# mountaindust/Parasitoids

Measured on AMD Instinct MI355X. Metric: grid-days/sec on 4096^2 fp64 domain, higher is better.
Workload: dtype f64; 1 GPU; C3 synthetic stack: N=4097 (nominal 4096^2), 30 Gaussian day kernels K=2049, reference torus P=5121, FFT size 5184 (fast mode), prob model, one replica stack per GPU; dom_len=4097, ndays=30, P=5121, fft_len=5184, kernels_direct=False, full_column_pipeline=True

## Files before the change

include/parasitoid_hip.h:

```cpp
#ifndef PARASITOID_HIP_H
#define PARASITOID_HIP_H
#include <stdint.h>

#ifdef __cplusplus
extern "C" {
#endif

#define PS_OK 0
#define PS_ERR_NO_DEVICE (-1)
#define PS_ERR_OOM (-2)
#define PS_ERR_BAD_SHAPE (-3)
#define PS_ERR_BAD_ARG (-4)
#define PS_ERR_UNSUPPORTED (-5)
#define PS_ERR_HIP (-6)
#define PS_ERR_HPROB_BOUNDS (-7)
#define PS_ERR_PMF_NEGATIVE (-8)
#define PS_ERR_FLIGHT_PROB (-9)
#define PS_ERR_STATE (-10)
#define PS_ERR_EMPTY (-11)

#define PS_MODE_EXACT 0
#define PS_MODE_FAST 1
#define PS_MODE_FOLD 2
#define PS_MODE_AUTO 3

typedef struct ps_solver ps_solver;
typedef struct ps_model ps_model;

typedef struct ps_day_stats {
  int64_t nnz;
  double sum;
  double delta;
  double padmax;
  int32_t flag;
  int32_t pad_;
} ps_day_stats;

int ps_version(void);
int ps_device_count(void);
const char* ps_last_error(void);
int ps_device_info(int device, char* name, int n, int* cus, int64_t* hbm_bytes);


int ps_solver_create(ps_solver** out, int device, int dom_len, int max_shape, int mode);
int ps_fast_size(int dom_len, int max_shape);
int ps_solver_retarget(ps_solver* s, int max_shape);
int ps_solver_destroy(ps_solver* s);
int ps_solver_info(ps_solver* s, int* dom_len, int* P, int* Pfft, int* H);
int ps_solver_sync(ps_solver* s);
int ps_solver_set_option(ps_solver* s, const char* key, double value);
int ps_solver_get_option(ps_solver* s, const char* key, double* value);
int ps_solver_kernels_direct(ps_solver* s);
int ps_solver_pipeline(ps_solver* s);
int ps_solver_auto_info(ps_solver* s, int* first_fold_day, int* fold_fft);
int ps_solver_auto_route(ps_solver* s, int first, int count, int32_t* owner);

int ps_solver_set_state_coo(ps_solver* s, const int32_t* row, const int32_t* col,
                            const double* val, int64_t nnz);

int ps_solver_fftconv2_coo(ps_solver* s, const int32_t* row, const int32_t* col,
                           const double* val, int64_t nnz, int kshape);

int ps_solver_get_cursol(ps_solver* s, double negval, double stat_scale, int renorm,
                         ps_day_stats* stats);

int ps_solver_back_solve(ps_solver* s, int nfilt, const int64_t* off, const int32_t* row,
                         const int32_t* col, const double* val, double negval,
                         double stat_scale, ps_day_stats* stats);


int ps_chain_set_kernels(ps_solver* s, int nk, const int64_t* off, const int32_t* kshape,
                         const int32_t* row, const int32_t* col, const double* val);
int ps_chain_run(ps_solver* s, int first, int count, double negval, double stat_scale,
                 int renorm);
int ps_chain_stats(ps_solver* s, int first, int count, ps_day_stats* out);

int ps_chain_run_release(ps_solver* s, int first, int count, double negval, int nfilt, int nuse,
                         const double* weights, int* certified);

int ps_chain_block_prefix(ps_solver* s, int first, int count, const void** total_dev, int64_t* total_bytes);
int ps_chain_block_finish(ps_solver* s, int first, int count, int nprev, const void* const* prev_totals,
                          double negval, double stat_scale, int renorm, int* flagged);
int ps_device_copy(void* dst, const void* src, int64_t bytes);

#define PS_REC_CHAIN 0
#define PS_REC_BACK 1
#define PS_REC_STATE 2
#define PS_REC_WSUM 3
int ps_record_stats(ps_solver* s, int kind, int idx, double negval, double stat_scale,
                    int renorm, ps_day_stats* out);
int ps_record_fetch_coo(ps_solver* s, int kind, int idx, double negval, double stat_scale,
                        double delta, double post_scale, int32_t* row, int32_t* col,
                        double* val, int64_t cap, int64_t* nnz_out);
int ps_record_fetch_csr(ps_solver* s, int kind, int idx, double negval, double stat_scale,
                        double delta, double post_scale, int32_t* indptr ,
                        int32_t* indices, double* data, int64_t cap, int64_t* nnz_out);
int ps_record_fetch_dense(ps_solver* s, int kind, int idx, double* out );
int ps_record_gather(ps_solver* s, int kind, int idx, int64_t n, const int32_t* rows,
                     const int32_t* cols, double scale, double negval, double* out);
int ps_record_gather_multi(ps_solver* s, int nrec, const int32_t* kind, const int32_t* idx, int64_t n,
                           const int32_t* rows, const int32_t* cols, double scale, double negval,
                           double* out);
int ps_weighted_sum(ps_solver* s, int n, const int32_t* kind, const int32_t* idx,
                    const double* w);

#define PS_PROF_NCLS 16
int ps_prof_enable(ps_solver* s, int on);
int ps_prof_read(ps_solver* s, int ncls, double* total_ms, int64_t* count);
int ps_prof_read_days(ps_solver* s, int ncls, int64_t* days);
int ps_prof_read_launches(ps_solver* s, int ncls, int64_t* launches);
int ps_prof_read_owner(ps_solver* s, int owner, int ncls, double* total_ms, int64_t* count, int64_t* launches,
                       int64_t* days);
int ps_solver_owner_fft(ps_solver* s, int owner);

int ps_solver_get_spectrum(ps_solver* s, double* out );
int ps_solver_set_spectrum(ps_solver* s, const double* in );

int ps_model_create(ps_model** out, int device);
int ps_model_destroy(ps_model* m);
int ps_model_set_option(ps_model* m, const char* key, double value);
int ps_model_set_wind(ps_model* m, const double* wind, const int32_t* day_keys, int ndays_wind,
                      int T, int test_run);
int ps_model_prob_mass(ps_model* m, int nd, const int32_t* day_idx, const double* start_time,
                       const double* hparams, const double* Dparams, const double* Dlparams,
                       double mu_r, int n_periods, double rad_dist, int rad_res,
                       int32_t* kshape, int64_t* nnz, int32_t* warned, int32_t* status);
int ps_model_fetch_coo(ps_model* m, int i, int32_t* row, int32_t* col, double* val, int64_t cap);
int ps_model_fetch_debug(ps_model* m, int i, double* hprob, int32_t* Hs, double* loss,
                         double* pmfsum);
int ps_model_hflight(ps_model* m, int day_i, const double* hparams, double* out);
int ps_model_mvn_cdf_values(ps_model* m, double cell, double mu_x, double mu_y, double sig_x,
                            double sig_y, double rho, int32_t* H, double* out, int64_t cap);
int ps_chain_set_kernels_from_model(ps_solver* s, ps_model* m, int first, int count);
int ps_solver_set_state_from_model(ps_solver* s, ps_model* m, int i);

int ps_model_export_device(ps_model* m, int first, int count, void* row_dev, void* col_dev, void* val_dev,
                           int64_t cap);
int ps_chain_set_kernels_device(ps_solver* s, int nk, const int64_t* off, const int32_t* kshape,
                                const void* row_dev, const void* col_dev, const void* val_dev);
int ps_solver_set_state_device(ps_solver* s, const void* row_dev, const void* col_dev, const void* val_dev,
                               int64_t nnz, int kshape);

typedef struct ps_summary ps_summary;
int ps_summary_create(int device, int N, int nslot, int nthr, const double* thr, ps_summary** out);
int ps_summary_add(ps_summary* a, ps_solver* s, int nslot, const int32_t* kind, const int32_t* idx,
                   const double* stat_scale, const double* post_scale, const int32_t* use_delta,
                   double negval, uint32_t weight);
int ps_summary_merge(ps_summary* dst, ps_summary* src);
int ps_summary_info(ps_summary* a, double* total_weight, int64_t* members);
int ps_summary_fetch(ps_summary* a, int slot, int what, double* out );
int ps_summary_reset(ps_summary* a);
int ps_summary_prof(ps_summary* a, int enable, double* total_ms, int64_t* launches);
void ps_summary_destroy(ps_summary* a);

typedef struct ps_linspread ps_linspread;
int ps_linspread_create(int device, int N, int nslot, int nparam, int nthr, const double* thr, ps_linspread** out);
int ps_linspread_set_center(ps_linspread* h, ps_solver* s, int nslot, const int32_t* kind, const int32_t* idx,
                            const double* stat_scale, const double* post_scale, const int32_t* use_delta,
                            double negval);
int ps_linspread_add(ps_linspread* h, ps_solver* s, int param, double coef, int nslot, const int32_t* kind,
                     const int32_t* idx, const double* stat_scale, const double* post_scale,
                     const int32_t* use_delta, double negval);
int ps_linspread_finalize(ps_linspread* h, int nparam, int rank, const double* F);
int ps_linspread_fetch(ps_linspread* h, int slot, int what, double* out );
int ps_linspread_info(ps_linspread* h, int* centered, int* finalized, int64_t* adds);
int ps_linspread_reset(ps_linspread* h);
int ps_linspread_prof(ps_linspread* h, int enable, double* add_ms, int64_t* add_launches, double* fin_ms,
                      int64_t* fin_launches);
void ps_linspread_destroy(ps_linspread* h);

typedef struct ps_hist ps_hist;
int ps_hist_create(int device, int N, int nslot, int nedge, const double* edges, ps_hist** out);
int ps_hist_add(ps_hist* h, ps_solver* s, int nslot, const int32_t* kind, const int32_t* idx,
                const double* stat_scale, const double* post_scale, const int32_t* use_delta, double negval,
                uint32_t weight);
int ps_hist_merge(ps_hist* dst, ps_hist* src);
int ps_hist_info(ps_hist* h, double* total_weight, int64_t* members, int* nedge);
int ps_hist_quantile(ps_hist* h, int slot, double p, double* value, double* lower, double* upper);
int ps_hist_exceed(ps_hist* h, int slot, int k, double* out );
int ps_hist_fetch_counts(ps_hist* h, int slot, int b, uint32_t* out );
int ps_hist_reset(ps_hist* h);
int ps_hist_prof(ps_hist* h, int enable, double* add_ms, int64_t* add_launches, double* q_ms,
                 int64_t* q_launches);
void ps_hist_destroy(ps_hist* h);

typedef struct ps_arrival ps_arrival;
int ps_arrival_create(int device, int N, int nslot, int nthr, const double* thr, ps_arrival** out);
int ps_arrival_add(ps_arrival* a, ps_solver* s, int nslot, const int32_t* kind, const int32_t* idx,
                   const double* stat_scale, const double* post_scale, const int32_t* use_delta, double negval,
                   uint32_t weight);
int ps_arrival_merge(ps_arrival* dst, ps_arrival* src);
int ps_arrival_info(ps_arrival* a, double* total_weight, int64_t* members);
int ps_arrival_prob(ps_arrival* a, int k, int slot, double* out );
int ps_arrival_quantile(ps_arrival* a, int k, double p, int32_t* out );
int ps_arrival_fetch_counts(ps_arrival* a, int k, int slot, uint32_t* out );
int ps_arrival_fetch_reached(ps_arrival* a, int64_t first, int64_t count, uint32_t* cells, uint32_t* weights);
int ps_arrival_reset(ps_arrival* a);
int ps_arrival_prof(ps_arrival* a, int enable, double* add_ms, int64_t* adds, double* map_ms, int64_t* maps);
void ps_arrival_destroy(ps_arrival* a);

#ifdef __cplusplus
}
#endif
#endif
```

parasitoids_amd/_lib.py:

```python
import ctypes as C
import os

import numpy as np

_HERE = os.path.dirname(os.path.abspath(__file__))
LIB_PATH = os.path.join(_HERE, 'libparasitoid_hip.so')

PS_OK = 0
PS_ERR_NO_DEVICE = -1
PS_ERR_OOM = -2
PS_ERR_BAD_SHAPE = -3
PS_ERR_BAD_ARG = -4
PS_ERR_UNSUPPORTED = -5
PS_ERR_HIP = -6
PS_ERR_HPROB_BOUNDS = -7
PS_ERR_PMF_NEGATIVE = -8
PS_ERR_FLIGHT_PROB = -9
PS_ERR_STATE = -10
PS_ERR_EMPTY = -11

MODE_EXACT = 0
MODE_FAST = 1
MODE_FOLD = 2
MODE_AUTO = 3

REC_CHAIN, REC_BACK, REC_STATE, REC_WSUM = 0, 1, 2, 3


class DayStats(C.Structure):
    _fields_ = [('nnz', C.c_int64), ('sum', C.c_double), ('delta', C.c_double),
                ('padmax', C.c_double), ('flag', C.c_int32), ('pad_', C.c_int32)]


class HipError(RuntimeError):
    def __init__(self, code, msg):
        super().__init__('libparasitoid_hip error %d: %s' % (code, msg))
        self.code = code


_I32P = C.POINTER(C.c_int32)
_I64P = C.POINTER(C.c_int64)
_F64P = C.POINTER(C.c_double)
_VP = C.c_void_p

SIGNATURES = {
    'ps_version': (C.c_int, []),
    'ps_device_count': (C.c_int, []),
    'ps_last_error': (C.c_char_p, []),
    'ps_device_info': (C.c_int, [C.c_int, C.c_char_p, C.c_int, _I32P, _I64P]),
    'ps_solver_create': (C.c_int, [C.POINTER(_VP), C.c_int, C.c_int, C.c_int, C.c_int]),
    'ps_solver_destroy': (C.c_int, [_VP]),
    'ps_solver_info': (C.c_int, [_VP, _I32P, _I32P, _I32P, _I32P]),
    'ps_solver_sync': (C.c_int, [_VP]),
    'ps_solver_set_option': (C.c_int, [_VP, C.c_char_p, C.c_double]),
    'ps_solver_get_option': (C.c_int, [_VP, C.c_char_p, _F64P]),
    'ps_solver_set_state_coo': (C.c_int, [_VP, _I32P, _I32P, _F64P, C.c_int64]),
    'ps_solver_fftconv2_coo': (C.c_int, [_VP, _I32P, _I32P, _F64P, C.c_int64, C.c_int]),
    'ps_solver_get_cursol': (C.c_int, [_VP, C.c_double, C.c_double, C.c_int, C.POINTER(DayStats)]),
    'ps_solver_back_solve': (C.c_int, [_VP, C.c_int, _I64P, _I32P, _I32P, _F64P, C.c_double,
                                       C.c_double, C.POINTER(DayStats)]),
    'ps_chain_set_kernels': (C.c_int, [_VP, C.c_int, _I64P, _I32P, _I32P, _I32P, _F64P]),
    'ps_chain_run': (C.c_int, [_VP, C.c_int, C.c_int, C.c_double, C.c_double, C.c_int]),
    'ps_chain_stats': (C.c_int, [_VP, C.c_int, C.c_int, C.POINTER(DayStats)]),
    'ps_chain_run_release': (C.c_int, [_VP, C.c_int, C.c_int, C.c_double, C.c_int, C.c_int, _F64P,
                                       C.POINTER(C.c_int)]),
    'ps_record_stats': (C.c_int, [_VP, C.c_int, C.c_int, C.c_double, C.c_double, C.c_int,
                                  C.POINTER(DayStats)]),
    'ps_solver_retarget': (C.c_int, [_VP, C.c_int]),
    'ps_fast_size': (C.c_int, [C.c_int, C.c_int]),
    'ps_solver_kernels_direct': (C.c_int, [_VP]),
    'ps_solver_pipeline': (C.c_int, [_VP]),
    'ps_solver_auto_info': (C.c_int, [_VP, _I32P, _I32P]),
    'ps_solver_auto_route': (C.c_int, [_VP, C.c_int, C.c_int, _I32P]),
    'ps_record_fetch_coo': (C.c_int, [_VP, C.c_int, C.c_int, C.c_double, C.c_double, C.c_double,
                                      C.c_double, _I32P, _I32P, _F64P, C.c_int64, _I64P]),
    'ps_record_fetch_csr': (C.c_int, [_VP, C.c_int, C.c_int, C.c_double, C.c_double, C.c_double,
                                      C.c_double, _I32P, _I32P, _F64P, C.c_int64, _I64P]),
    'ps_record_fetch_dense': (C.c_int, [_VP, C.c_int, C.c_int, _F64P]),
    'ps_record_gather': (C.c_int, [_VP, C.c_int, C.c_int, C.c_int64, _I32P, _I32P, C.c_double,
                                   C.c_double, _F64P]),
    'ps_record_gather_multi': (C.c_int, [_VP, C.c_int, _I32P, _I32P, C.c_int64, _I32P, _I32P, C.c_double,
                                          C.c_double, _F64P]),
    'ps_weighted_sum': (C.c_int, [_VP, C.c_int, _I32P, _I32P, _F64P]),
    'ps_prof_enable': (C.c_int, [_VP, C.c_int]),
    'ps_prof_read': (C.c_int, [_VP, C.c_int, _F64P, _I64P]),
    'ps_prof_read_days': (C.c_int, [_VP, C.c_int, _I64P]),
    'ps_prof_read_launches': (C.c_int, [_VP, C.c_int, _I64P]),
    'ps_chain_block_prefix': (C.c_int, [_VP, C.c_int, C.c_int, C.POINTER(C.c_void_p), C.POINTER(C.c_int64)]),
    'ps_chain_block_finish': (C.c_int, [_VP, C.c_int, C.c_int, C.c_int, C.POINTER(C.c_void_p), C.c_double, C.c_double,
                                        C.c_int, C.POINTER(C.c_int)]),
    'ps_device_copy': (C.c_int, [C.c_void_p, C.c_void_p, C.c_int64]),
    'ps_prof_read_owner': (C.c_int, [_VP, C.c_int, C.c_int, _F64P, _I64P, _I64P, _I64P]),
    'ps_solver_owner_fft': (C.c_int, [_VP, C.c_int]),
    'ps_solver_get_spectrum': (C.c_int, [_VP, _F64P]),
    'ps_solver_set_spectrum': (C.c_int, [_VP, _F64P]),
    'ps_model_create': (C.c_int, [C.POINTER(_VP), C.c_int]),
    'ps_model_destroy': (C.c_int, [_VP]),
    'ps_model_set_option': (C.c_int, [_VP, C.c_char_p, C.c_double]),
    'ps_model_set_wind': (C.c_int, [_VP, _F64P, _I32P, C.c_int, C.c_int, C.c_int]),
    'ps_model_prob_mass': (C.c_int, [_VP, C.c_int, _I32P, _F64P, _F64P, _F64P, _F64P, C.c_double,
                                     C.c_int, C.c_double, C.c_int, _I32P, _I64P, _I32P, _I32P]),
    'ps_model_fetch_coo': (C.c_int, [_VP, C.c_int, _I32P, _I32P, _F64P, C.c_int64]),
    'ps_model_fetch_debug': (C.c_int, [_VP, C.c_int, _F64P, _I32P, _F64P, _F64P]),
    'ps_model_hflight': (C.c_int, [_VP, C.c_int, _F64P, _F64P]),
    'ps_model_mvn_cdf_values': (C.c_int, [_VP, C.c_double, C.c_double, C.c_double, C.c_double,
                                          C.c_double, C.c_double, _I32P, _F64P, C.c_int64]),
    'ps_chain_set_kernels_from_model': (C.c_int, [_VP, _VP, C.c_int, C.c_int]),
    'ps_solver_set_state_from_model': (C.c_int, [_VP, _VP, C.c_int]),
    'ps_model_export_device': (C.c_int, [_VP, C.c_int, C.c_int, _VP, _VP, _VP, C.c_int64]),
    'ps_chain_set_kernels_device': (C.c_int, [_VP, C.c_int, _I64P, _I32P, _VP, _VP, _VP]),
    'ps_solver_set_state_device': (C.c_int, [_VP, _VP, _VP, _VP, C.c_int64, C.c_int]),
    'ps_summary_create': (C.c_int, [C.c_int, C.c_int, C.c_int, C.c_int, _F64P, C.POINTER(_VP)]),
    'ps_summary_add': (C.c_int, [_VP, _VP, C.c_int, _I32P, _I32P, _F64P, _F64P, _I32P, C.c_double,
                                 C.c_uint32]),
    'ps_summary_merge': (C.c_int, [_VP, _VP]),
    'ps_summary_info': (C.c_int, [_VP, _F64P, _I64P]),
    'ps_summary_fetch': (C.c_int, [_VP, C.c_int, C.c_int, _F64P]),
    'ps_summary_reset': (C.c_int, [_VP]),
    'ps_summary_prof': (C.c_int, [_VP, C.c_int, _F64P, _I64P]),
    'ps_summary_destroy': (None, [_VP]),
    'ps_linspread_create': (C.c_int, [C.c_int, C.c_int, C.c_int, C.c_int, C.c_int, _F64P, C.POINTER(_VP)]),
    'ps_linspread_set_center': (C.c_int, [_VP, _VP, C.c_int, _I32P, _I32P, _F64P, _F64P, _I32P, C.c_double]),
    'ps_linspread_add': (C.c_int, [_VP, _VP, C.c_int, C.c_double, C.c_int, _I32P, _I32P, _F64P, _F64P, _I32P,
                                   C.c_double]),
    'ps_linspread_finalize': (C.c_int, [_VP, C.c_int, C.c_int, _F64P]),
    'ps_linspread_fetch': (C.c_int, [_VP, C.c_int, C.c_int, _F64P]),
    'ps_linspread_info': (C.c_int, [_VP, _I32P, _I32P, _I64P]),
    'ps_linspread_reset': (C.c_int, [_VP]),
    'ps_linspread_prof': (C.c_int, [_VP, C.c_int, _F64P, _I64P, _F64P, _I64P]),
    'ps_linspread_destroy': (None, [_VP]),
    'ps_hist_create': (C.c_int, [C.c_int, C.c_int, C.c_int, C.c_int, _F64P, C.POINTER(_VP)]),
    'ps_hist_add': (C.c_int, [_VP, _VP, C.c_int, _I32P, _I32P, _F64P, _F64P, _I32P, C.c_double, C.c_uint32]),
    'ps_hist_merge': (C.c_int, [_VP, _VP]),
    'ps_hist_info': (C.c_int, [_VP, _F64P, _I64P, _I32P]),
    'ps_hist_quantile': (C.c_int, [_VP, C.c_int, C.c_double, _F64P, _F64P, _F64P]),
    'ps_hist_exceed': (C.c_int, [_VP, C.c_int, C.c_int, _F64P]),
    'ps_hist_fetch_counts': (C.c_int, [_VP, C.c_int, C.c_int, C.POINTER(C.c_uint32)]),
    'ps_hist_reset': (C.c_int, [_VP]),
    'ps_hist_prof': (C.c_int, [_VP, C.c_int, _F64P, _I64P, _F64P, _I64P]),
    'ps_hist_destroy': (None, [_VP]),
    'ps_arrival_create': (C.c_int, [C.c_int, C.c_int, C.c_int, C.c_int, _F64P, C.POINTER(_VP)]),
    'ps_arrival_add': (C.c_int, [_VP, _VP, C.c_int, _I32P, _I32P, _F64P, _F64P, _I32P, C.c_double, C.c_uint32]),
    'ps_arrival_merge': (C.c_int, [_VP, _VP]),
    'ps_arrival_info': (C.c_int, [_VP, _F64P, _I64P]),
    'ps_arrival_prob': (C.c_int, [_VP, C.c_int, C.c_int, _F64P]),
    'ps_arrival_quantile': (C.c_int, [_VP, C.c_int, C.c_double, _I32P]),
    'ps_arrival_fetch_counts': (C.c_int, [_VP, C.c_int, C.c_int, C.POINTER(C.c_uint32)]),
    'ps_arrival_fetch_reached': (C.c_int, [_VP, C.c_int64, C.c_int64, C.POINTER(C.c_uint32),
                                           C.POINTER(C.c_uint32)]),
    'ps_arrival_reset': (C.c_int, [_VP]),
    'ps_arrival_prof': (C.c_int, [_VP, C.c_int, _F64P, _I64P, _F64P, _I64P]),
    'ps_arrival_destroy': (None, [_VP]),
}

_lib = None


def load():
    global _lib
    if _lib is not None:
        return _lib
    if not os.path.exists(LIB_PATH):
        raise ImportError(
            'libparasitoid_hip.so not found at %s; build it with '
            '`python -c "import __graft_entry__ as g; g.build()"` or '
            '`make -C parasitoids_amd/csrc`' % LIB_PATH)
    try:
        lib = C.CDLL(LIB_PATH)
    except OSError as e:
        raise ImportError('cannot load %s: %s' % (LIB_PATH, e))
    for name, (res, args) in SIGNATURES.items():
        fn = getattr(lib, name)
        fn.restype = res
        fn.argtypes = args
    _lib = lib
    return lib


def check(rc):
    if rc != PS_OK:
        msg = load().ps_last_error()
        raise HipError(rc, msg.decode() if msg else '')


def require_device():
    lib = load()
    n = lib.ps_device_count()
    if n <= 0:
        msg = lib.ps_last_error()
        raise ImportError('no MI355X/HIP device available: %s' % (msg.decode() if msg else ''))
    return n


def default_device():
    return int(os.environ.get('PARASITOID_DEVICE', os.environ.get('LOCAL_RANK', '0')))


def i32(a):
    return np.ascontiguousarray(a, dtype=np.int32)


def f64(a):
    return np.ascontiguousarray(a, dtype=np.float64)


def p_i32(a):
    return a.ctypes.data_as(_I32P)


def p_i64(a):
    return a.ctypes.data_as(_I64P)


def p_f64(a):
    return a.ctypes.data_as(_F64P)
```

parasitoids_amd/csrc/chain_kernels.h:

```cpp
#pragma once
#include <hip/hip_runtime.h>
#include <stdint.h>

static __global__ void k_scatter_coo(const int* __restrict__ row, const int* __restrict__ col,
                              const double* __restrict__ val, int64_t nnz, double* dst, int ld,
                              int roff, int coff) {
  for (int64_t i = blockIdx.x * (int64_t)blockDim.x + threadIdx.x; i < nnz;
       i += (int64_t)gridDim.x * blockDim.x)
    atomicAdd(&dst[(int64_t)(row[i] + roff) * ld + col[i] + coff], val[i]);
}

static __global__ void k_zero_band(double* dst, int K, int r0, int r1) {
  double* base = dst + (int64_t)blockIdx.y * K * K + (int64_t)r0 * K;
  const int64_t n = (int64_t)(r1 - r0 + 1) * K;
  for (int64_t i = blockIdx.x * (int64_t)blockDim.x + threadIdx.x; i < n; i += (int64_t)gridDim.x * blockDim.x)
    base[i] = 0.0;
}

static __global__ void k_scatter_coo_batch(const int* __restrict__ row, const int* __restrict__ col,
                                           const double* __restrict__ val, const long long* __restrict__ koff,
                                           const int* __restrict__ kshape, int first, double* dst, int K) {
  const int d = first + blockIdx.y;
  const long long lo = koff[d], hi = koff[d + 1];
  const int off = K / 2 - kshape[d] / 2;
  double* out = dst + (int64_t)blockIdx.y * K * K;
  for (long long i = lo + blockIdx.x * (long long)blockDim.x + threadIdx.x; i < hi;
       i += (long long)gridDim.x * blockDim.x)
    atomicAdd(&out[(int64_t)(row[i] + off) * K + col[i] + off], val[i]);
}

struct DayStats {
  long long nnz;
  double sum;
  double delta;
  double padmax;
  int flag;
  int pad_;
};

static __global__ void k_day_finalize(const double* rowsum_, const long long* rowcnt_,
                               const unsigned long long* padmax_, int N, int renorm,
                               DayStats* out_) {
  const double* rowsum = rowsum_ + (int64_t)blockIdx.x * N;
  const long long* rowcnt = rowcnt_ + (int64_t)blockIdx.x * N;
  const unsigned long long* padmax = padmax_ + blockIdx.x;
  DayStats* out = out_ + blockIdx.x;
  __shared__ double ssum[256];
  __shared__ long long scnt[256];
  double s = 0.0;
  long long c = 0;
  for (int r = threadIdx.x; r < N; r += blockDim.x) {
    s += rowsum[r];
    c += rowcnt[r];
  }
  ssum[threadIdx.x] = s;
  scnt[threadIdx.x] = c;
  __syncthreads();
  for (int off = blockDim.x / 2; off > 0; off >>= 1) {
    if ((int)threadIdx.x < off) {
      ssum[threadIdx.x] += ssum[threadIdx.x + off];
      scnt[threadIdx.x] += scnt[threadIdx.x + off];
    }
    __syncthreads();
  }
  if (threadIdx.x == 0) {
    DayStats d;
    d.nnz = scnt[0];
    d.sum = ssum[0];
    d.delta = (renorm && scnt[0] > 0) ? (1.0 - ssum[0]) / (double)scnt[0] : 0.0;
    d.padmax = __longlong_as_double((long long)*padmax);
    d.flag = d.padmax > 1e-8 ? 1 : 0;
    d.pad_ = 0;
    *out = d;
  }
}

static __global__ void k_row_stats(const double* __restrict__ rec, int N, double scale, double negval,
                            double* rowsum, long long* rowcnt) {
  __shared__ double ssum[256];
  __shared__ int scnt[256];
  const int r = blockIdx.x;
  double s = 0.0;
  int c = 0;
  for (int i = threadIdx.x; i < N; i += blockDim.x) {
    const double t = rec[(int64_t)r * N + i] * scale;
    if (t != 0.0 && !(t < negval)) { s += t; ++c; }
  }
  ssum[threadIdx.x] = s;
  scnt[threadIdx.x] = c;
  __syncthreads();
  for (int off = blockDim.x / 2; off > 0; off >>= 1) {
    if ((int)threadIdx.x < off) {
      ssum[threadIdx.x] += ssum[threadIdx.x + off];
      scnt[threadIdx.x] += scnt[threadIdx.x + off];
    }
    __syncthreads();
  }
  if (threadIdx.x == 0) { rowsum[r] = ssum[0]; rowcnt[r] = scnt[0]; }
}

static __global__ void k_fold(const double* __restrict__ lin, int M, int P, int N, int m, double* torus,
                              double* rec, double negval, double stat_scale, double* rowsum,
                              long long* rowcnt, unsigned long long* padmax) {
  const int r = blockIdx.x;
  int yr[3], nr = 0;
  yr[nr++] = r;
  if (r < m) yr[nr++] = r + P;
  if (r >= P - m) yr[nr++] = r - P + M;
  __shared__ double ssum[256];
  __shared__ long long scnt[256];
  __shared__ double smax[256];
  double s = 0.0, pm = 0.0;
  long long cnt = 0;
  for (int c = threadIdx.x; c < P; c += blockDim.x) {
    int yc[3], nc = 0;
    yc[nc++] = c;
    if (c < m) yc[nc++] = c + P;
    if (c >= P - m) yc[nc++] = c - P + M;
    double v = 0.0;
    for (int i = 0; i < nr; ++i)
      for (int j = 0; j < nc; ++j) v += lin[(int64_t)yr[i] * M + yc[j]];
    torus[(int64_t)r * P + c] = v;
    if (r < N && c < N) {
      rec[(int64_t)r * N + c] = v;
      const double t = v * stat_scale;
      if (!(t < negval)) { s += t; ++cnt; }
    } else {
      pm = fmax(pm, v);
    }
  }
  ssum[threadIdx.x] = s;
  scnt[threadIdx.x] = cnt;
  smax[threadIdx.x] = pm;
  __syncthreads();
  for (int off = blockDim.x / 2; off > 0; off >>= 1) {
    if ((int)threadIdx.x < off) {
      ssum[threadIdx.x] += ssum[threadIdx.x + off];
      scnt[threadIdx.x] += scnt[threadIdx.x + off];
      smax[threadIdx.x] = fmax(smax[threadIdx.x], smax[threadIdx.x + off]);
    }
    __syncthreads();
  }
  if (threadIdx.x == 0) {
    if (r < N) { rowsum[r] = ssum[0]; rowcnt[r] = scnt[0]; }
    const double mx = smax[0];
    const unsigned long long bits = (unsigned long long)__double_as_longlong(mx);
    if (mx > 0.0 && bits > __hip_atomic_load(padmax, __ATOMIC_RELAXED, __HIP_MEMORY_SCOPE_AGENT))
      atomicMax(padmax, bits);
  }
}

static __global__ void k_truncate_if_flag(double* torus, int P, int N, const unsigned long long* padmax) {
  if (!(__longlong_as_double((long long)*padmax) > 1e-8)) return;
  const int r = blockIdx.x;
  for (int c = threadIdx.x; c < P; c += blockDim.x)
    if (r >= N || c >= N) torus[(int64_t)r * P + c] = 0.0;
}

static __global__ void k_scan_rows(const long long* rowcnt_, int N, long long* rowoff_) {
  const long long* rowcnt = rowcnt_ + (int64_t)blockIdx.x * N;
  long long* rowoff = rowoff_ + (int64_t)blockIdx.x * N;
  __shared__ long long part[1024];
  const int T = blockDim.x;
  const int per = (N + T - 1) / T;
  const int lo = threadIdx.x * per, hi = min(N, lo + per);
  long long s = 0;
  {
    int r = lo;
    for (; r + 8 <= hi; r += 8) {
      long long v[8];
#pragma unroll
      for (int u = 0; u < 8; ++u) v[u] = rowcnt[r + u];
#pragma unroll
      for (int u = 0; u < 8; ++u) s += v[u];
    }
    for (; r < hi; ++r) s += rowcnt[r];
  }
  part[threadIdx.x] = s;
  __syncthreads();
  for (int off = 1; off < T; off <<= 1) {
    const long long v = (int)threadIdx.x >= off ? part[threadIdx.x - off] : 0;
    __syncthreads();
    part[threadIdx.x] += v;
    __syncthreads();
  }
  long long acc = part[threadIdx.x] - s;
  int r = lo;
  for (; r + 8 <= hi; r += 8) {
    long long v[8];
#pragma unroll
    for (int u = 0; u < 8; ++u) v[u] = rowcnt[r + u];
#pragma unroll
    for (int u = 0; u < 8; ++u) { rowoff[r + u] = acc; acc += v[u]; }
  }
  for (; r < hi; ++r) { rowoff[r] = acc; acc += rowcnt[r]; }
}

static __global__ void k_compact_rows(const double* __restrict__ rec, int N, double scale, double negval,
                               double delta, double post_scale, const long long* rowoff,
                               int* orow, int* ocol, double* oval) {
  const int wave = (blockIdx.x * blockDim.x + threadIdx.x) >> 6;
  const int lane = threadIdx.x & 63;
  if (wave >= N) return;
  long long base = rowoff[wave];
  for (int c0 = 0; c0 < N; c0 += 64) {
    const int c = c0 + lane;
    double t = 0.0;
    bool keep = false;
    if (c < N) {
      t = rec[(int64_t)wave * N + c] * scale;
      keep = (t != 0.0) && !(t < negval);
    }
    const unsigned long long m = __ballot(keep);
    if (keep) {
      const int o = __popcll(m & ((1ull << lane) - 1ull));
      orow[base + o] = wave;
      ocol[base + o] = c;
      oval[base + o] = (t + delta) * post_scale;
    }
    base += __popcll(m);
  }
}

static __global__ void k_weighted_sum(const double* const* recs, const double* w, int nrec, int64_t n,
                               double* out) {
  for (int64_t i = blockIdx.x * (int64_t)blockDim.x + threadIdx.x; i < n;
       i += (int64_t)gridDim.x * blockDim.x) {
    double acc = 0.0;
    for (int d = 0; d < nrec; ++d) acc += recs[d][i] * w[d];
    out[i] = acc;
  }
}

static __global__ void k_expand_spectrum(const double2* __restrict__ half, int P, int H, int ld,
                                  double2* full) {
  const int64_t tot = (int64_t)P * P;
  for (int64_t idx = blockIdx.x * (int64_t)blockDim.x + threadIdx.x; idx < tot;
       idx += (int64_t)gridDim.x * blockDim.x) {
    const int r = (int)(idx / P), c = (int)(idx % P);
    double2 v;
    if (c < H) {
      v = half[(int64_t)r * ld + c];
    } else {
      const int rr = r ? P - r : 0, cc = P - c;
      v = half[(int64_t)rr * ld + cc];
      v.y = -v.y;
    }
    full[idx] = v;
  }
}

static __global__ void k_take_half_spectrum(const double2* __restrict__ full, int P, int H, int ld,
                                     double2* half) {
  const int64_t tot = (int64_t)P * H;
  for (int64_t idx = blockIdx.x * (int64_t)blockDim.x + threadIdx.x; idx < tot;
       idx += (int64_t)gridDim.x * blockDim.x) {
    const int r = (int)(idx / H), c = (int)(idx % H);
    half[(int64_t)r * ld + c] = full[(int64_t)r * P + c];
  }
}

static __global__ void k_gather_points_multi(const double* const* __restrict__ recs, int N, const int* rows,
                                             const int* cols, int64_t n, double scale, double negval, double* out) {
  const double* rec = recs[blockIdx.y];
  double* o = out + (int64_t)blockIdx.y * n;
  for (int64_t i = blockIdx.x * (int64_t)blockDim.x + threadIdx.x; i < n;
       i += (int64_t)gridDim.x * blockDim.x) {
    const double t = rec[(int64_t)rows[i] * N + cols[i]] * scale;
    o[i] = (t < negval) ? 0.0 : t;
  }
}

static __global__ void k_gather_points(const double* __restrict__ rec, int N, const int* rows,
                                const int* cols, int64_t n, double scale, double negval, double* out) {
  for (int64_t i = blockIdx.x * (int64_t)blockDim.x + threadIdx.x; i < n;
       i += (int64_t)gridDim.x * blockDim.x) {
    const double t = rec[(int64_t)rows[i] * N + cols[i]] * scale;
    out[i] = (t < negval) ? 0.0 : t;
  }
}

static __global__ void k_set_int2(int* dst, int a, int b) {
  if (threadIdx.x == 0 && blockIdx.x == 0) { dst[0] = a; dst[1] = b; }
}
```

parasitoids_amd/csrc/fft_kernels.h:

```cpp
#pragma once
#include "fft_core.h"

#define PS_UNROLL 5

struct SrcMap {
  int n1, off1, lo2, off2;
};
__device__ __forceinline__ bool pred_skip(const unsigned long long* pred) {
  return pred && !(__longlong_as_double((long long)*pred) > 1e-8);
}
__device__ __forceinline__ int src_map(const SrcMap& m, int i) {
  if (i < m.n1) return i + m.off1;
  if (i >= m.lo2) return i - m.lo2 + m.off2;
  return -1;
}

struct RowLive {
  int on;
  SrcMap map;
  const int* range;
};
__device__ __forceinline__ bool row_live(const RowLive& v, int r, int batch) {
  if (!v.on) return true;
  const int sr = src_map(v.map, r);
  if (sr < 0) return false;
  if (!v.range) return true;
  return sr >= v.range[2 * batch] && sr <= v.range[2 * batch + 1];
}

struct RowFwdArgs {
  const double* src;
  int64_t src_bstride;
  int src_ld;
  SrcMap rmap, cmap;
  cplx* dst;
  int64_t dst_bstride;
  int H, ld, P;
  int tstride;
  int rp;
  int skip_zero;
  const int* rowrange;
  int nblocks;
  const unsigned long long* pred;
  const unsigned long long* trunc_pred;
  int trunc_n;
  FftProg prog;
};

struct ColArgs {
  const cplx* src;
  const cplx* src2;
  cplx* prod_dst;
  cplx* dst;
  int64_t src_bstride, src2_bstride, prod_bstride, dst_bstride;
  int ld, ncols, wsh, n_outer;
  int in_base_mul, in_stride, out_base_mul, out_stride;
  int tw_mode;
  const cplx* tp_lo;
  const cplx* tp_hi;
  int tp_shift;
  RowLive live;
  int nblocks;
  const unsigned long long* pred;
  FftProg prog;
};

struct RowInvArgs {
  const cplx* src;
  int64_t src_bstride;
  int H, ld, P, N;
  int tstride;
  int pair_src;
  int rp;
  double scale;
  double* rec;
  int64_t rec_bstride;
  double negval, stat_scale;
  double* rowsum;
  long long* rowcnt;
  unsigned long long* padmax;
  double pad_floor;
  int64_t stat_bstride;
  int persistent;
  const int* pad_quiet;
  int nrec;
  double* rec_multi[32];
  FftProg prog;
};

__device__ __forceinline__ int tw_count(const FftProg& P) { return P.n_lo + P.n_hi + P.n_gen; }
__device__ __forceinline__ void load_tw(cplx* tlo, cplx* thi, const FftProg& P) {
  const int n = tw_count(P);
  for (int t = threadIdx.x; t < n; t += blockDim.x) tlo[t] = P.tw_lo[t];
}

template <int DIR, bool GEN, bool BIG>
__device__ __forceinline__ void run_stage_sel(cplx* data, const cplx* tlo, const cplx* thi,
                                              const FftProg& P, int s, int mode, int nb, int wsh,
                                              int bs) {
  const int tid = threadIdx.x, nthr = blockDim.x;
  switch (P.radix[s]) {
    case 2: run_stage_r<2, DIR>(data, tlo, thi, P, s, mode, nb, wsh, bs, tid, nthr); break;
    case 3: run_stage_r<3, DIR>(data, tlo, thi, P, s, mode, nb, wsh, bs, tid, nthr); break;
    case 4: run_stage_r<4, DIR>(data, tlo, thi, P, s, mode, nb, wsh, bs, tid, nthr); break;
    case 5: run_stage_r<5, DIR>(data, tlo, thi, P, s, mode, nb, wsh, bs, tid, nthr); break;
    case 7: run_stage_r<7, DIR>(data, tlo, thi, P, s, mode, nb, wsh, bs, tid, nthr); break;
    case 8: run_stage_r<8, DIR>(data, tlo, thi, P, s, mode, nb, wsh, bs, tid, nthr); break;
    case 9: run_stage_r<9, DIR>(data, tlo, thi, P, s, mode, nb, wsh, bs, tid, nthr); break;
    case 16: if (BIG) run_stage_r<16, DIR>(data, tlo, thi, P, s, mode, nb, wsh, bs, tid, nthr); break;
    case 18: if (BIG) run_stage_r<18, DIR>(data, tlo, thi, P, s, mode, nb, wsh, bs, tid, nthr); break;
    default:
      if (GEN) {
        if (DIR == PS_INV && P.m[s] > 1) {
          gen_pretwiddle<DIR>(data, tlo, thi, P, s, mode, nb, wsh, bs, tid, nthr);
          __syncthreads();
        }
        run_stage_generic<DIR>(data, tlo, thi, P, s, mode, nb, wsh, bs, tid, nthr);
      }
      break;
  }
}

template <int DIR, bool GEN, bool BIG = false>
__device__ __forceinline__ void lds_fft(cplx* data, const cplx* tlo, const cplx* thi,
                                        const FftProg& P, int mode, int nb, int wsh, int bs) {
  if (DIR == PS_FWD) {
    for (int s = 0; s < P.ns; ++s) {
      run_stage_sel<DIR, GEN, BIG>(data, tlo, thi, P, s, mode, nb, wsh, bs);
      __syncthreads();
    }
  } else {
    for (int s = P.ns - 1; s >= 0; --s) {
      run_stage_sel<DIR, GEN, BIG>(data, tlo, thi, P, s, mode, nb, wsh, bs);
      __syncthreads();
    }
  }
}

extern __shared__ __attribute__((aligned(16))) unsigned char ps_lds_raw[];

template <bool GEN, bool BIG>
__device__ __forceinline__ void row_fwd_block(const RowFwdArgs& a, const int bx) {
  const FftProg& P = a.prog;
  const int L = P.L;
  const int pitch = row_pitch(P);
  cplx* data = reinterpret_cast<cplx*>(ps_lds_raw);
  cplx* tlo = data + (size_t)a.rp * pitch;
  cplx* thi = tlo + P.n_lo;
  const double* src = a.src + (int64_t)blockIdx.y * a.src_bstride;
  cplx* dst = a.dst + (int64_t)blockIdx.y * a.dst_bstride;
  const int pair0 = bx * a.rp;
  const int nthr = blockDim.x;
  const int rlo = a.rowrange ? a.rowrange[2 * blockIdx.y] : 0;
  const int rhi = a.rowrange ? a.rowrange[2 * blockIdx.y + 1] : 0x7fffffff;
  auto srow = [&](int r) {
    const int sr = r < a.P ? src_map(a.rmap, r) : -1;
    return (sr < rlo || sr > rhi) ? -1 : sr;
  };
  bool any = false;
  for (int b = 0; b < a.rp; ++b) {
    const int ra = 2 * (pair0 + b), rb = ra + 1;
    if (srow(ra) >= 0) any = true;
    if (srow(rb) >= 0) any = true;
  }
  if (!any) {
    if (a.skip_zero) return;
    const cplx z = make_double2(0.0, 0.0);
    for (int b = 0; b < a.rp; ++b) {
      const int ra = 2 * (pair0 + b), rb = ra + 1;
      for (int k = threadIdx.x; k < a.H; k += nthr) {
        if (ra < a.P) dst[(int64_t)ra * a.ld + k] = z;
        if (rb < a.P) dst[(int64_t)rb * a.ld + k] = z;
      }
    }
    return;
  }
  load_tw(tlo, thi, P);
  for (int b = 0; b < a.rp; ++b) {
    const int ra = 2 * (pair0 + b), rb = ra + 1;
    const int sa = srow(ra);
    const int sb = srow(rb);
    const double* pa = src + (int64_t)sa * a.src_ld;
    const double* pb = src + (int64_t)sb * a.src_ld;
    for (int i0 = threadIdx.x; i0 < L; i0 += nthr * PS_UNROLL) {
      double va[PS_UNROLL], vb[PS_UNROLL];
#pragma unroll
      for (int u = 0; u < PS_UNROLL; ++u) {
        const int i = i0 + u * nthr;
        va[u] = 0.0;
        vb[u] = 0.0;
        if (i < L) {
          const int sc = src_map(a.cmap, i);
          if (sc >= 0) {
            if (sa >= 0) va[u] = pa[sc];
            if (sb >= 0) vb[u] = pb[sc];
          }
        }
      }
#pragma unroll
      for (int u = 0; u < PS_UNROLL; ++u) {
        const int i = i0 + u * nthr;
        if (i < L) data[b * pitch + row_phys(P, i)] = make_double2(va[u], vb[u]);
      }
    }
  }
  __syncthreads();
  lds_fft<PS_FWD, GEN, BIG>(data, tlo, thi, P, PS_MODE_ROW, a.rp, 0, pitch);
  for (int b = 0; b < a.rp; ++b) {
    const int ra = 2 * (pair0 + b), rb = ra + 1;
    if (ra >= a.P) break;
    const cplx* d = data + b * pitch;
    for (int k0 = threadIdx.x; k0 < a.H; k0 += nthr * PS_UNROLL) {
      unsigned pk[PS_UNROLL], pm[PS_UNROLL];
#pragma unroll
      for (int u = 0; u < PS_UNROLL; ++u) {
        const int k = k0 + u * nthr;
        pk[u] = 0;
        pm[u] = 0;
        if (k < a.H) {
          pk[u] = P.pos_phys[k];
          pm[u] = P.pos_phys[k ? L - k : 0];
        }
      }
#pragma unroll
      for (int u = 0; u < PS_UNROLL; ++u) {
        const int k = k0 + u * nthr;
        if (k < a.H) {
          const cplx zk = d[pk[u]];
          const cplx zm = d[pm[u]];
          const cplx A = make_double2(0.5 * (zk.x + zm.x), 0.5 * (zk.y - zm.y));
          const cplx B = make_double2(0.5 * (zk.y + zm.y), -0.5 * (zk.x - zm.x));
          dst[(int64_t)ra * a.ld + k] = A;
          if (rb < a.P) dst[(int64_t)rb * a.ld + k] = B;
        }
      }
    }
  }
}

template <bool GEN, bool BIG>
__global__ void __launch_bounds__(BIG ? 512 : 1024) k_row_fwd(RowFwdArgs a) {
  if (pred_skip(a.pred)) return;
  for (int bx = blockIdx.x; bx < a.nblocks; bx += gridDim.x) {
    row_fwd_block<GEN, BIG>(a, bx);
    if (bx + (int)gridDim.x < a.nblocks) __syncthreads();
  }
}

template <int DIR, bool GEN>
__device__ __forceinline__ void col_block(const ColArgs& a, const int bx) {
  const FftProg& P = a.prog;
  const int L = P.L;
  const int W = 1 << a.wsh;
  cplx* data = reinterpret_cast<cplx*>(ps_lds_raw);
  cplx* tlo = data + ((size_t)L << a.wsh);
  cplx* thi = tlo + P.n_lo;
  cplx* stw = tlo + tw_count(P);
  int* spos = reinterpret_cast<int*>(stw + L);
  const int ntiles = (a.ncols + W - 1) >> a.wsh;
  const int tile = bx % ntiles;
  const int o = bx / ntiles;
  const int c0 = tile << a.wsh;
  const int nthr = blockDim.x;
  const cplx* src = a.src + (int64_t)blockIdx.y * a.src_bstride;
  const cplx* src2 = a.src2 ? a.src2 + (int64_t)blockIdx.y * a.src2_bstride : nullptr;
  cplx* prod = a.prod_dst ? a.prod_dst + (int64_t)blockIdx.y * a.prod_bstride : nullptr;
  cplx* dst = a.dst + (int64_t)blockIdx.y * a.dst_bstride;
  const bool tw_on = a.tw_mode != 0 && o != 0;
  const int tot = L << a.wsh;
  const int in_base = o * a.in_base_mul, out_base = o * a.out_base_mul;
  cplx v[PS_UNROLL], v2[PS_UNROLL];
  auto load_batch = [&](int idx0) {
#pragma unroll
    for (int u = 0; u < PS_UNROLL; ++u) {
      const int idx = idx0 + u * nthr;
      const int row = idx >> a.wsh, col = c0 + (idx & (W - 1));
      v[u] = make_double2(0.0, 0.0);
      v2[u] = make_double2(1.0, 0.0);
      const int grow = in_base + row * a.in_stride;
      if (idx < tot && col < a.ncols && row_live(a.live, grow, blockIdx.y)) {
        const int64_t g = (int64_t)grow * a.ld + col;
        v[u] = src[g];
        if (src2) v2[u] = src2[g];
      }
    }
  };
  auto store_batch = [&](int idx0) {
#pragma unroll
    for (int u = 0; u < PS_UNROLL; ++u) {
      const int idx = idx0 + u * nthr;
      if (idx >= tot) continue;
      const int row = idx >> a.wsh, c = idx & (W - 1);
      cplx x = v[u];
      if (src2) {
        x = cmul(x, v2[u]);
        if (prod && c0 + c < a.ncols) prod[(int64_t)(in_base + row * a.in_stride) * a.ld + c0 + c] = x;
      }
      if (a.tw_mode == 2 && tw_on) x = cmulc(x, stw[row]);
      const int lrow = DIR == PS_INV ? spos[row] : row;
      data[(lrow << a.wsh) + c] = x;
    }
  };
  load_batch(threadIdx.x);
  load_tw(tlo, thi, P);
  for (int r = threadIdx.x; r < L; r += nthr) {
    spos[r] = (int)P.pos[r];
    if (tw_on) stw[r] = tw_lookup(a.tp_lo, a.tp_hi, a.tp_shift, o * r);
  }
  __syncthreads();
  store_batch(threadIdx.x);
  for (int idx0 = threadIdx.x + nthr * PS_UNROLL; idx0 < tot; idx0 += nthr * PS_UNROLL) {
    load_batch(idx0);
    store_batch(idx0);
  }
  __syncthreads();
  lds_fft<DIR, GEN>(data, tlo, thi, P, PS_MODE_COL, W, a.wsh, 0);
  for (int idx = threadIdx.x; idx < tot; idx += nthr) {
    const int row = idx >> a.wsh, c = idx & (W - 1);
    const int col = c0 + c;
    if (col >= a.ncols) continue;
    const int lrow = DIR == PS_FWD ? spos[row] : row;
    cplx x = data[(lrow << a.wsh) + c];
    if (a.tw_mode == 1 && tw_on) x = cmul(x, stw[row]);
    dst[(int64_t)(out_base + row * a.out_stride) * a.ld + col] = x;
  }
}

template <int DIR, bool GEN>
__global__ void __launch_bounds__(256, 4) k_col(ColArgs a) {
  if (pred_skip(a.pred)) return;
  for (int bx = blockIdx.x; bx < a.nblocks; bx += gridDim.x) {
    col_block<DIR, GEN>(a, bx);
    if (bx + (int)gridDim.x < a.nblocks) __syncthreads();
  }
}

struct ColFusedArgs {
  const cplx* src;
  cplx* state;
  cplx* dst;
  int64_t src_bstride;
  int64_t dst_dstride;
  int ld, ncols, wsh, L1, L2, store_prod;
  RowLive live;
  RowLive live2;
  int direct;
  int no_conj;
  const cplx* tp_lo;
  const cplx* tp_hi;
  int tp_shift;
// ... 629 lines not shown
```

parasitoids_amd/csrc/fft_rs_kernels.h:

```cpp
#pragma once
#include "fft_kernels.h"
#include "fft_rs.h"
#include <type_traits>


template <int R1, int R2, int R3>
struct RsInvLds {
  using S = Rs<R1, R2, R3>;
  static constexpr int XW = (S::XWORDS + 15) & ~15;
  static constexpr int RED = 16 * (S::NTHR / 64);
  static constexpr size_t bytes(int np) { return (size_t)np * (XW + RED) * sizeof(double); }
};

template <int R1, int R2, int R3, int NP>
__global__ void __launch_bounds__((Rs<R1, R2, R3>::NTHR * NP)) k_row_inv_rs(RowInvArgs a) {
  using S = Rs<R1, R2, R3>;
  using Y = RsInvLds<R1, R2, R3>;
  constexpr int L = S::L;
  constexpr int NW = S::NTHR / 64;
  const int half = threadIdx.x / S::NTHR;
  int unit = (int)blockIdx.x;
  if (a.tstride) {
    constexpr int KL = NP >= 4 ? 1 : 4 / NP;
    const int xcd = unit & 7, q = unit >> 3;
// ... 468 lines not shown

template <int R1, int R2, int R3>
struct Rs2Lds {
  using S = Rs<R1, R2, R3>;
  using Y = RsInvLds<R1, R2, R3>;
  static constexpr int NW = S::NTHR / 64;
  static constexpr int RED = 8 * NW;
  static constexpr int HS = (S::L / 2 + 1 + 63) & ~63;
  static constexpr size_t bytes = (size_t)(Y::XW + 2 * RED) * sizeof(double) + 2 * (size_t)HS * sizeof(cplx);
  static constexpr bool ok = 2 * S::NTHR <= 1024 && S::RMAX <= 18 && bytes <= (size_t)160 * 1024;
};

template <int R1, int R2, int R3>
__global__ void __launch_bounds__((2 * Rs<R1, R2, R3>::NTHR)) k_row_inv_rs2(RowInvArgs a, int npairs, int units) {
  using S = Rs<R1, R2, R3>;
  using Y = RsInvLds<R1, R2, R3>;
  using Z = Rs2Lds<R1, R2, R3>;
  constexpr int L = S::L;
  constexpr int NW = S::NTHR / 64;
  constexpr int NCH = Z::HS / 64;
  constexpr int H = L / 2 + 1;
  double* ex = reinterpret_cast<double*>(ps_lds_raw);
  const int role = __builtin_amdgcn_readfirstlane((int)threadIdx.x / S::NTHR);
  const int j0 = threadIdx.x - role * S::NTHR, lane = j0 & 63, wave = __builtin_amdgcn_readfirstlane(j0 >> 6);
  double* red = ex + Y::XW + role * Z::RED;
  double* ered = red + 5 * NW;
  cplx* st = reinterpret_cast<cplx*>(ex + Y::XW + 2 * Z::RED);
  const FftProg& P = a.prog;
  const cplx w2c = tw_lookup(P.tw_lo, P.tw_hi, P.tw_shift, S::tw2(j0));
  const cplx w3c = tw_lookup(P.tw_lo, P.tw_hi, P.tw_shift, j0 < S::T3 ? S::tw3(j0) : 0);
  const int G2 = 2 * (int)gridDim.x;

  auto next_unit = [&](int v) {
    while (v < units && a.pad_quiet) {
      const int vb = v / npairs, vp = v - vb * npairs;
      if (2 * vp < a.N || !a.pad_quiet[vb]) break;
      v += G2;
    }
    return v;
  };
  auto count_units = [&](int r) {
    int n = 0;
    for (int v = next_unit(2 * (int)blockIdx.x + r); v < units; v = next_unit(v + G2)) ++n;
    return n;
  };
  const int n0 = count_units(0), n1 = count_units(1);
  const int HP = max(2 * n0, n1 > 0 ? 2 * n1 + 1 : 0);

  cplx x[S::RMAX];
  int cur = next_unit(2 * (int)blockIdx.x + role);
  bool loaded = false;
  bool done = false;

  auto prefetch = [&](int u) {
    const int b = u / npairs, pair = u - b * npairs;
    const cplx* src = a.src + (int64_t)b * a.src_bstride;
    const int ra = 2 * pair, rb = (ra + 1 < a.P) ? ra + 1 : ra;
    const cplx* pa = src + (int64_t)ra * a.ld;
    const int ksh = a.pair_src ? 1 : 0;
    const int bo = a.pair_src ? 1 : (rb - ra) * a.ld;
    int ln = lane;
    asm volatile("" : "+v"(ln));
    const int bofs = (ln >> 5) ? bo : 0;
    ln &= 31;
#pragma unroll
    for (int t = 0; t < (2 * NCH + NW - 1) / NW; ++t) {
      const int c = wave + t * NW;
      if (c < 2 * NCH) {
        int k = c * 32 + ln;
        k = k < H ? k : H - 1;
        const cplx* g = pa + ((k << ksh) + bofs);
        cplx* d = st + c * 64;
        __builtin_amdgcn_global_load_lds(g, (ps_lds_ptr)d, 16, 0, 0);
      }
    }
  };

  int eb = 0, era = 0;
  double e_sa = 0.0, e_sb = 0.0, e_pmax = 0.0;
  int e_ca = 0, e_cb = 0;
  bool pend = false;
  int pend_b = 0, pend_ra = 0;
  auto epi_piece = [&](int j, auto q0c, auto q1c) {
    constexpr int Q0 = decltype(q0c)::value, Q1 = decltype(q1c)::value;
    const int ra = era, rb = era + 1;
    double* rec = a.nrec > 0 ? a.rec_multi[eb] : a.rec + (int64_t)eb * a.rec_bstride;
    if (j < S::T3) {
      double* reca = rec + (int64_t)ra * a.N;
      double* recb = rec + (int64_t)rb * a.N;
      const bool dom_a = ra < a.N, dom_b = rb < a.N;
      const unsigned uj = (unsigned)j, uN = (unsigned)a.N;
      const bool dom_ab = dom_a && dom_b;
      const bool hb = rb < a.P;
#pragma unroll
      for (int q = Q0; q < Q1; ++q) {
        const unsigned i = uj + (unsigned)(q * S::T3);
        const double va = x[q].x * a.scale, vb = x[q].y * a.scale;
        const double ta = va * a.stat_scale, tb = vb * a.stat_scale;
        if (dom_ab && (unsigned)((q + 1) * S::T3) <= uN) {
          reca[i] = va;
          recb[i] = vb;
          const bool ka = !(ta < a.negval), kb = !(tb < a.negval);
          e_sa += ka ? ta : 0.0;
          e_sb += kb ? tb : 0.0;
          e_ca += __popcll(__ballot(ka));
          e_cb += __popcll(__ballot(kb));
        } else {
          const bool in = i < uN;
          const bool ina = in && dom_a, inb = in && dom_b;
          const bool ka = ina && !(ta < a.negval), kb = inb && !(tb < a.negval);
          e_sa += ka ? ta : 0.0;
          e_sb += kb ? tb : 0.0;
          e_ca += __popcll(__ballot(ka));
          e_cb += __popcll(__ballot(kb));
          e_pmax = fmax(e_pmax, ina ? 0.0 : va);
          e_pmax = fmax(e_pmax, (inb || !hb) ? 0.0 : vb);
          if (ina) reca[i] = va;
          if (inb) recb[i] = vb;
        }
      }
    }
  };
  auto finalize = [&]() {
    double ta = 0, tb = 0, na = 0, nbb = 0, m = 0;
    for (int w = 0; w < NW; ++w) {
      ta += red[w * 4 + 0];
      tb += red[w * 4 + 1];
      na += red[w * 4 + 2];
      nbb += red[w * 4 + 3];
      m = fmax(m, red[4 * NW + w]);
    }
    const int frb = pend_ra + 1;
    double* rowsum = a.rowsum + (int64_t)pend_b * a.stat_bstride;
    long long* rowcnt = a.rowcnt + (int64_t)pend_b * a.stat_bstride;
    if (pend_ra < a.N) { rowsum[pend_ra] = ta; rowcnt[pend_ra] = (long long)na; }
    if (frb < a.N) { rowsum[frb] = tb; rowcnt[frb] = (long long)nbb; }
    unsigned long long* pm = a.padmax + pend_b;
    const unsigned long long bits = (unsigned long long)__double_as_longlong(m);
    if (m > a.pad_floor && bits > __hip_atomic_load(pm, __ATOMIC_RELAXED, __HIP_MEMORY_SCOPE_AGENT))
      atomicMax(pm, bits);
  };
  auto T_half = [&]() {
    int j = j0;
    cplx w2 = w2c, w3 = w3c;
    asm volatile("" : "+v"(j), "+v"(w2.x), "+v"(w2.y), "+v"(w3.x), "+v"(w3.y));
    bool act = loaded;
    const int pair = cur % npairs;
    const bool pad_only = 2 * pair >= a.N;
    const bool hasb = 2 * pair + 1 < a.P;
    PS_BAR_LDS();
    if (pend && j0 == S::NTHR - 1) finalize();
    pend = false;
    double energy = 0.0;
    if (act && j < S::T1) {
#pragma unroll
      for (int q = 0; q < R1; ++q) {
        const bool direct = (q < R1 / 2) || (q == R1 / 2 && j == 0);
        const int i = j + q * S::T1;
        const int k = direct ? i : L - i;
        const int slot = k + (k & ~31);
        const cplx A = st[slot];
        cplx B = st[slot + 32];
        if (!hasb) B = make_double2(0.0, 0.0);
        if (direct) energy += A.x * A.x + A.y * A.y + B.x * B.x + B.y * B.y;
        x[q] = direct ? make_double2(A.x - B.y, A.y + B.x) : make_double2(A.x + B.y, B.x - A.y);
      }
    }
    if (act && pad_only) {
      energy = ps_wave_sum(energy);
      if (lane == 63) ered[wave] = energy;
    }
    PS_BAR_LDS();
    if (act && pad_only) {
      double e = 0.0;
      for (int w = 0; w < NW; ++w) e += ered[w];
      if (sqrt(2.0 * (double)a.P * e) * a.scale < a.pad_floor) act = false;
    }
    if (act && j < S::T1) {
      bfly<R1, PS_INV>(x);
      rs_put<R1, 0>(ex, S::x1_w(j), 1, x);
    }
    PS_BAR_LDS();
    if (act && j < S::T2) rs_get<R2, 0>(ex, S::x_r(j), S::X1_RS, x);
    PS_BAR_LDS();
    if (act && j < S::T1) rs_put<R1, 1>(ex, S::x1_w(j), 1, x);
    PS_BAR_LDS();
    if (act && j < S::T2) rs_get<R2, 1>(ex, S::x_r(j), S::X1_RS, x);
    asm volatile("" : "+v"(w2.x), "+v"(w2.y));
    if (act && j < S::T2) rs_stage<R2, PS_INV>(x, w2, true);
    PS_BAR_LDS();
    if (act && j < S::T2) rs_put<R2, 0>(ex, S::x2_w(j), 17, x);
    PS_BAR_LDS();
    if (act && j < S::T3) rs_get<R3, 0>(ex, S::x_r(j), S::X2_RS, x);
    PS_BAR_LDS();
    if (act && j < S::T2) rs_put<R2, 1>(ex, S::x2_w(j), 17, x);
    PS_BAR_LDS();
    if (act && j < S::T3) rs_get<R3, 1>(ex, S::x_r(j), S::X2_RS, x);
    asm volatile("" : "+v"(w3.x), "+v"(w3.y));
    if (act && j < S::T3) rs_stage<R3, PS_INV>(x, w3, true);
    if (loaded) {
      loaded = false;
      if (act) done = true;
      else cur = next_unit(cur + G2);
    }
  };
#define PS_EPI_PIECE(k) \
  if (epi) epi_piece(j, std::integral_constant<int, ((k) * R3) / 6>(), std::integral_constant<int, (((k) + 1) * R3) / 6>())
  auto S_half = [&]() {
    int j = j0;
    asm volatile("" : "+v"(j));
    const bool epi = done;
    if (epi) {
      eb = cur / npairs;
      era = 2 * (cur - eb * npairs);
      e_sa = e_sb = e_pmax = 0.0;
      e_ca = e_cb = 0;
      done = false;
      cur = next_unit(cur + G2);
    }
    PS_BAR_LDS();
    PS_BAR_LDS();
    loaded = false;
    if (cur < units) {
      prefetch(cur);
      loaded = true;
    }
    PS_BAR_LDS();
    PS_EPI_PIECE(0);
    PS_BAR_LDS();
    PS_EPI_PIECE(1);
    PS_BAR_LDS();
    PS_EPI_PIECE(2);
    PS_BAR_LDS();
    PS_EPI_PIECE(3);
    PS_BAR_LDS();
    PS_EPI_PIECE(4);
    PS_BAR_LDS();
    PS_EPI_PIECE(5);
    PS_BAR_LDS();
    if (epi) {
      const double sa = ps_wave_sum(e_sa), sb = ps_wave_sum(e_sb);
      const int ca = __builtin_amdgcn_readfirstlane(e_ca), cb = __builtin_amdgcn_readfirstlane(e_cb);
      const double pmax = ps_wave_max0(e_pmax);
      if (lane == 63) {
        red[wave * 4 + 0] = sa;
        red[wave * 4 + 1] = sb;
        red[wave * 4 + 2] = (double)ca;
        red[wave * 4 + 3] = (double)cb;
        red[4 * NW + wave] = pmax;
      }
      pend = true;
      pend_b = eb;
      pend_ra = era;
    }
    PS_WAIT_VM0();
  };
#undef PS_EPI_PIECE
  auto idle_half = [&]() {
#pragma unroll
    for (int i = 0; i < 9; ++i) PS_BAR_LDS();
  };

  if (role == 0) {
    if (cur < units) {
      prefetch(cur);
      PS_WAIT_VM0();
      loaded = true;
    }
    for (int k = 0; k < n0; ++k) {
      T_half();
      S_half();
    }
    for (int h = 2 * n0; h < HP; ++h) idle_half();
  } else {
    for (int k = 0; k < n1; ++k) {
      S_half();
      T_half();
    }
    int h = 2 * n1;
    if (n1 > 0) {
      S_half();
      ++h;
    }
    for (; h < HP; ++h) idle_half();
  }
  PS_BAR_LDS();
  if (pend && j0 == S::NTHR - 1) finalize();
}


template <int R1, int R2, int R3, int NP>
__global__ void __launch_bounds__((Rs<R1, R2, R3>::NTHR * NP)) k_row_fwd_rs(RowFwdArgs a) {
  using S = Rs<R1, R2, R3>;
  using Y = RsInvLds<R1, R2, R3>;
  constexpr int L = S::L;
  if (pred_skip(a.pred)) return;
  const int half = threadIdx.x / S::NTHR;
  int unit = (int)blockIdx.x;
  if (a.tstride) {
    constexpr int KL = NP >= 4 ? 1 : 4 / NP;
    const int xcd = unit & 7, q = unit >> 3;
    unit = ((q / KL) * 8 + xcd) * KL + (q % KL);
  }
  const int pair = ((int)gridDim.x - 1 - unit) * NP + half;
  const int ra = 2 * pair, rb = ra + 1;
  if (ra >= a.P || pair < 0) return;
  double* ex = reinterpret_cast<double*>(ps_lds_raw) + half * (Y::XW + Y::RED);
  const int j = threadIdx.x - half * S::NTHR;
  const double* src = a.src + (int64_t)blockIdx.y * a.src_bstride;
  cplx* dst = a.dst + (int64_t)blockIdx.y * a.dst_bstride;
  const int rlo = a.rowrange ? a.rowrange[2 * blockIdx.y] : 0;
  const int rhi = a.rowrange ? a.rowrange[2 * blockIdx.y + 1] : 0x7fffffff;
  SrcMap rmap = a.rmap, cmap = a.cmap;
  const bool trunc = a.trunc_pred && !pred_skip(a.trunc_pred);
  if (trunc) {
    rmap.n1 = rmap.n1 < a.trunc_n ? rmap.n1 : a.trunc_n;
    cmap.n1 = cmap.n1 < a.trunc_n ? cmap.n1 : a.trunc_n;
  }
  auto srow = [&](int r) {
    const int sr = r < a.P ? src_map(rmap, r) : -1;
    return (sr < rlo || sr > rhi) ? -1 : sr;
  };
  const int sa = srow(ra), sb = srow(rb);
  const int64_t kst = a.tstride ? (int64_t)a.tstride : 1;
  cplx* da = dst + (a.tstride ? (int64_t)ra : (int64_t)ra * a.ld);
  cplx* db = dst + (a.tstride ? (int64_t)rb : (int64_t)rb * a.ld);
  const bool hasb = rb < a.P;
  if (sa < 0 && sb < 0) {
    const bool cut = trunc && ((ra < a.P && src_map(a.rmap, ra) >= 0) || (rb < a.P && src_map(a.rmap, rb) >= 0));
    if (a.skip_zero && !cut) return;
    const cplx z = make_double2(0.0, 0.0);
    for (int k = j; k < a.H; k += S::NTHR) {
      da[k * kst] = z;
      if (hasb) db[k * kst] = z;
    }
    return;
  }
  const FftProg& P = a.prog;
  const cplx w2 = tw_lookup(P.tw_lo, P.tw_hi, P.tw_shift, S::tw2(j));
  const cplx w3 = tw_lookup(P.tw_lo, P.tw_hi, P.tw_shift, j < S::T3 ? S::tw3(j) : 0);
  cplx x[S::RMAX];
  if (j < S::T1) {
    const double* pa = src + (int64_t)(sa >= 0 ? sa : 0) * a.src_ld;
    const double* pb = src + (int64_t)(sb >= 0 ? sb : 0) * a.src_ld;
#pragma unroll
    for (int q = 0; q < R1; ++q) {
      const int sc = src_map(cmap, j + q * S::T1);
      const bool ok = sc >= 0;
      const int c = ok ? sc : 0;
      const double va = pa[c], vb = pb[c];
      x[q] = make_double2((ok && sa >= 0) ? va : 0.0, (ok && sb >= 0) ? vb : 0.0);
    }
    bfly<R1, PS_FWD>(x);
  }
  rs_tail<S, R1, R2, R3, PS_FWD>(x, ex, j, w2, w3);
  cplx zm[R3 / 2 + 1];
  constexpr int NQ = R3 / 2 + 1;
  __syncthreads();
  if (j < S::T3) {
#pragma unroll
    for (int q = 0; q < R3; ++q) ex[j + q * S::T3] = x[q].x;
  }
  __syncthreads();
  if (j < S::T3) {
#pragma unroll
    for (int q = 0; q < NQ; ++q) {
      const int k = j + q * S::T3;
      zm[q].x = ex[k ? L - k : 0];
    }
  }
  __syncthreads();
  if (j < S::T3) {
#pragma unroll
    for (int q = 0; q < R3; ++q) ex[j + q * S::T3] = x[q].y;
  }
  __syncthreads();
  if (j < S::T3) {
#pragma unroll
    for (int q = 0; q < NQ; ++q) {
      const int k = j + q * S::T3;
      zm[q].y = ex[k ? L - k : 0];
      if (k <= L / 2) {
        const cplx zk = x[q];
        da[k * kst] = make_double2(0.5 * (zk.x + zm[q].x), 0.5 * (zk.y - zm[q].y));
        if (hasb) db[k * kst] = make_double2(0.5 * (zk.y + zm[q].y), -0.5 * (zk.x - zm[q].x));
      }
    }
  }
}
```

parasitoids_amd/csrc/ps_config.h:

```cpp
#pragma once
#include <cstdlib>
#include <cstring>

#define PS_OPTION_TABLE(X)                                                                          \
                                               \
  X("PS_NO_RS", no_rs, 0, FLAG, C)                                                                  \
  X("PS_NO_RS_FWD", no_rs_fwd, 0, FLAG, C)                                                          \
  X("PS_NO_BIG_RADIX", no_big_radix, 0, FLAG, C)                                                    \
  X("PS_NO_TPIPE", no_tpipe, 0, FLAG, C)                                                            \
  X("PS_NO_FOLD_TPIPE", no_fold_tpipe, 0, FLAG, C)                                                  \
  X("PS_COL_SINGLE_MAX", col_single_max, 1200, INT, C)                                              \
  X("PS_COL_L1", col_l1, 0, INT, C)                                                                 \
  X("PS_CHUNK_DAYS", chunk_days, 0, INT, C)                                                         \
  X("PS_FAST_SIZE", fast_size, 0, INT, C)                                                           \
  X("PS_RS_AREA", rs_area, 0.0, NUM, C)                                                             \
                                                                                 \
  X("PS_COL_WSH", col_wsh, -1, INT, R)                                                              \
  X("PS_COL_THREADS", col_threads, 256, INT, R)                                                     \
  X("PS_FUSED_WSH", fused_wsh, -1, INT, R)                                                          \
  X("PS_FUSED_THREADS", fused_threads, 0, INT, R)                                                   \
  X("PS_FUSED_G", fused_g, 2, INT, R)                                                               \
  X("PS_MULTI_WSH", multi_wsh, -1, INT, R)                                                          \
  X("PS_DUAL_WSH", dual_wsh, -1, INT, R)                                                            \
  X("PS_FUSED_DAYS", fused_days, 8, INT, R)                                                         \
  X("PS_DIRECT_DAYS", direct_days, 4, INT, R)                                                       \
  X("PS_DIRECT_MAX_TERMS", direct_max_terms, 8, INT, R)                                             \
  X("PS_TPIPE_DAYS", tpipe_days, 32, INT, R)                                                        \
  X("PS_DUAL_MIN_DAYS", dual_min_days, 6, INT, R)                                                   \
                                                   \
  X("PS_TINV", tinv, 0, INT, R)                                                                     \
  X("PS_RSP", rsp, -1, INT, R)                                                                      \
  X("PS_ROW2", row2, -1, INT, R)                                                                    \
  X("PS_TPIPE", tpipe, -1, INT, R)                                                                  \
  X("PS_NO_PAIR_ROWS", no_pair_rows, 0, FLAG, R)                                                    \
  X("PS_TPIPE_SPLIT", tpipe_split, 0, INT, R)                                                       \
  X("PS_NO_CONJ", no_conj, 0, FLAG, R)                                                              \
  X("PS_NO_DUAL", no_dual, 0, FLAG, R)                                                              \
  X("PS_NO_DIRECT", no_direct, 0, FLAG, R)                                                          \
  X("PS_NO_ROW_BATCH", no_row_batch, 0, FLAG, R)                                                    \
  X("PS_NO_PAD_QUIET", no_pad_quiet, 0, FLAG, R)                                                    \
  X("PS_NO_TAIL_SPLIT", no_tail_split, 0, FLAG, R)                                                  \
  X("PS_NO_DEFER_REFFT", no_defer_refft, 0, FLAG, R)                                                \
  X("PS_NO_FILTER_CACHE", no_filter_cache, 0, FLAG, R)                                              \
  X("PS_NO_FOLD_FUSE", no_fold_fuse, 0, FLAG, R)                                                    \
  X("PS_NO_FOLD_ALT", no_fold_alt, 0, FLAG, R)                                                      \
  X("PS_NO_FOLD_ROWS", no_fold_rows, 0, FLAG, R)                                                    \
                                                                                 \
  X("PS_NO_SPECULATION", no_speculation, 0, FLAG, R)                                                \
  X("PS_SPEC_DEPTH", spec_depth, 2, INT, R)                                                         \
  X("PS_NO_FLAG_HISTORY", no_flag_history, 0, FLAG, R)                                              \
  X("PS_NO_WINDOW_HINT", no_window_hint, 0, FLAG, R)                                                \
  X("PS_FIRST_WINDOW", first_window, -1, INT, R)                                                    \
  X("PS_KT_SPLIT", kt_split, -1, INT, R)                                                            \
  X("PS_NO_LAZY_KT", no_lazy_kt, 0, FLAG, R)                                                        \
  X("PS_NO_WIDE", no_wide, 0, FLAG, R)                                                              \
  X("PS_NO_ROUTE_HISTORY", no_route_history, 0, FLAG, R)                                            \
  X("PS_WIDE_MIN_N", wide_min_n, 1500, INT, R)                                                      \
  X("PS_AUTO_WINDOW", auto_window, 4, INT, R)                                                       \
                                                                  \
  X("PS_PM_SEG", pm_seg, 8, INT, R)                                                                 \
  X("PS_PM_SYNC", pm_sync, 0, FLAG, R)                                                              \
  X("PS_PM_NO_UNROLL", pm_no_unroll, 0, FLAG, R)

struct ps_config {
#define PS_CFG_FIELD_FLAG int
#define PS_CFG_FIELD_INT int
#define PS_CFG_FIELD_NUM double
#define X(key, field, dflt, kind, when) PS_CFG_FIELD_##kind field = dflt;
  PS_OPTION_TABLE(X)
#undef X
};

inline void ps_config_from_env(ps_config* c) {
  *c = ps_config();
#define PS_CFG_ENV_FLAG(field) c->field = (e[0] == '\0' || std::strcmp(e, "0") != 0) ? 1 : 0
#define PS_CFG_ENV_INT(field) c->field = std::atoi(e)
#define PS_CFG_ENV_NUM(field) c->field = std::atof(e)
#define X(key, field, dflt, kind, when) \
  if (const char* e = std::getenv(key)) { PS_CFG_ENV_##kind(field); }
  PS_OPTION_TABLE(X)
#undef X
}

inline int ps_config_set(ps_config* c, const char* key, double value, bool live) {
  if (!key) return -1;
#define PS_CFG_SET_FLAG(field) c->field = value != 0.0 ? 1 : 0
#define PS_CFG_SET_INT(field) c->field = (int)value
#define PS_CFG_SET_NUM(field) c->field = value
#define PS_CFG_WHEN_C true
#define PS_CFG_WHEN_R false
#define X(k, field, dflt, kind, when)         \
  if (std::strcmp(key, k) == 0) {             \
    if (live && PS_CFG_WHEN_##when) return -2; \
    PS_CFG_SET_##kind(field);                 \
    return 0;                                 \
  }
  PS_OPTION_TABLE(X)
#undef X
  return -1;
}

inline int ps_config_get(const ps_config* c, const char* key, double* value) {
  if (!key || !value) return -1;
#define X(k, field, dflt, kind, when) \
  if (std::strcmp(key, k) == 0) {     \
    *value = (double)c->field;        \
    return 0;                         \
  }
  PS_OPTION_TABLE(X)
#undef X
  return -1;
}
```

parasitoids_amd/csrc/ps_rs_rows.hip:

```cpp
#include "rs_cfg.h"
#include "rs_launch.h"
#include <algorithm>
#include <cstdlib>

bool rs_lookup(int L, int* r2, int* r3) {
#define X(A, B) if (L == 16 * A * B) { *r2 = A; *r3 = B; return true; }
  PS_RS_SIZES(X)
#undef X
  return false;
}

int rs_next_size(int n) {
  int best = 0;
#define X(A, B) if (16 * A * B >= n && (best == 0 || 16 * A * B < best)) best = 16 * A * B;
  PS_RS_SIZES(X)
#undef X
  return best;
}

bool rs_info(int r2, int r3, RsInfo* out) {
#define X(A, B)                                                                       \
  if (r2 == A && r3 == B) {                                                           \
    using C = RsCfg<A, B>;                                                            \
    *out = RsInfo{C::NP, C::S::NTHR, C::LDS, C::LDSC1, C::LDSC, C::CHAIN, RsPLds<16, A, B>::fits};            \
    return true;                                                                      \
  }
  PS_RS_SIZES(X)
#undef X
  return false;
}

int rs_rows_set_attrs() {
#define X(A, B)                                                                                              \
  {                                                                                                          \
    using C = RsCfg<A, B>;                                                                                   \
    constexpr int np = C::NP;                                                                                \
    using Z = RsPLds<16, A, B>;                                                                              \
    if constexpr (Z::fits) {                                                                                 \
      auto kp = k_row_inv_rsp<16, A, B>;                                                                     \
      if (hipFuncSetAttribute((const void*)kp, hipFuncAttributeMaxDynamicSharedMemorySize, (int)Z::bytes) != hipSuccess) return -1; \
    }                                                                                                        \
    using Z2 = Rs2Lds<16, A, B>;                                                                             \
    if constexpr (Z2::ok) {                                                                                  \
      auto k2 = k_row_inv_rs2<16, A, B>;                                                                     \
      if (Z2::bytes > 48 * 1024 &&                                                                           \
          hipFuncSetAttribute((const void*)k2, hipFuncAttributeMaxDynamicSharedMemorySize, (int)Z2::bytes) != hipSuccess) return -1; \
    }                                                                                                        \
    if (C::LDSC1 > 48 * 1024) {                                                                              \
      auto kr = k_row_inv_fold<16, A, B>;                                                                    \
      if (hipFuncSetAttribute((const void*)kr, hipFuncAttributeMaxDynamicSharedMemorySize, (int)C::LDSC1) != hipSuccess) return -1; \
    }                                                                                                        \
    if (C::LDS > 48 * 1024) {                                                                                \
      auto ki = k_row_inv_rs<16, A, B, np>;                                                                  \
      auto kf = k_row_fwd_rs<16, A, B, np>;                                                                  \
      if (hipFuncSetAttribute((const void*)ki, hipFuncAttributeMaxDynamicSharedMemorySize, (int)C::LDS) != hipSuccess) return -1; \
      if (hipFuncSetAttribute((const void*)kf, hipFuncAttributeMaxDynamicSharedMemorySize, (int)C::LDS) != hipSuccess) return -1; \
    }                                                                                                        \
  }
  PS_RS_SIZES(X)
#undef X
  return 0;
}

static int device_cus();
static int grid_x(int npairs, int np, int tstride) {
  int gx = (npairs + np - 1) / np;
  if (tstride) {
    const int m = 8 * (np >= 4 ? 1 : 4 / np);
    gx = (gx + m - 1) / m * m;
  }
  return gx;
}

int rs_launch_row_fwd(int r2, int r3, const RowFwdArgs& a, int npairs, int batch, hipStream_t st) {
#define X(A, B)                                                                                              \
  if (r2 == A && r3 == B) {                                                                                  \
    using C = RsCfg<A, B>;                                                                                   \
    constexpr int np = C::NP;                                                                                \
                                                 \
    constexpr int np2 = (np >= 2 && C::S::L <= 2560) ? np / 2 : np;                                          \
    if constexpr (np2 != np) {                                                                               \
      const int live = a.rmap.n1 + (a.P > a.rmap.lo2 ? a.P - a.rmap.lo2 : 0);                                \
      if ((((live + 1) / 2 + np - 1) / np) * batch < device_cus()) {                                         \
        auto k2 = k_row_fwd_rs<16, A, B, np2>;                                                               \
        using Y2 = RsInvLds<16, A, B>;                                                                       \
        constexpr size_t lds2 = Y2::bytes(np2);                                                              \
        hipLaunchKernelGGL(k2, dim3(grid_x(npairs, np2, a.tstride), batch), dim3(C::S::NTHR * np2), lds2, st, a); \
        return 1;                                                                                            \
      }                                                                                                      \
    }                                                                                                        \
    auto kern = k_row_fwd_rs<16, A, B, np>;                                                                  \
    hipLaunchKernelGGL(kern, dim3(grid_x(npairs, np, a.tstride), batch), dim3(C::S::NTHR * np), C::LDS, st, a); \
    return 1;                                                                                                \
  }
  PS_RS_SIZES(X)
#undef X
  return 0;
}

int rs_launch_row_fold(int r2, int r3, const RowFoldArgs& a, int units, hipStream_t st) {
#define X(A, B)                                                                                              \
  if (r2 == A && r3 == B) {                                                                                  \
    using C = RsCfg<A, B>;                                                                                   \
    auto kern = k_row_inv_fold<16, A, B>;                                                                    \
    hipLaunchKernelGGL(kern, dim3(units), dim3(C::S::NTHR), C::LDSC1, st, a);                                \
    return 1;                                                                                                \
  }
  PS_RS_SIZES(X)
#undef X
  return 0;
}

static int device_cus() {
  static int n = 0;
  if (n == 0) {
    int dev = 0;
    hipDeviceProp_t prop;
    if (hipGetDevice(&dev) != hipSuccess || hipGetDeviceProperties(&prop, dev) != hipSuccess) return 256;
    n = prop.multiProcessorCount > 0 ? prop.multiProcessorCount : 256;
  }
  return n;
}

int rs_launch_row_inv(int r2, int r3, const RowInvArgs& a, int npairs, int batch, hipStream_t st) {
#define X(A, B)                                                                                              \
  if (r2 == A && r3 == B) {                                                                                  \
    using C = RsCfg<A, B>;                                                                                   \
    using Z = RsPLds<16, A, B>;                                                                              \
    using Z2 = Rs2Lds<16, A, B>;                                                                             \
    if constexpr (Z2::ok) {                                                                                  \
      if (a.persistent == 2 && a.tstride == 0) {         \
        const int units = npairs * batch;                                                                    \
        const int wgs = std::min(device_cus(), (units + 1) / 2);                                             \
        auto k2 = k_row_inv_rs2<16, A, B>;                                                                   \
        hipLaunchKernelGGL(k2, dim3(wgs), dim3(2 * C::S::NTHR), Z2::bytes, st, a, npairs, units);            \
        return 1;                                                                                            \
      }                                                                                                      \
    }                                                                                                        \
    if constexpr (Z::fits) {                                                                                 \
      if (a.persistent && a.tstride == 0) {                                                                  \
        const int units = npairs * batch;                                                                    \
                 \
        constexpr int W = C::S::NTHR / 64;                                                                   \
        constexpr int kw = 8 / W < 1 ? 1 : 8 / W, kl = (int)((size_t)160 * 1024 / Z::bytes);                 \
        constexpr int per_cu = kw < kl ? kw : kl;                                                            \
        const int slots = device_cus() * per_cu;                                                             \
        const int wgs = units < slots ? units : slots;                                                       \
        auto kp = k_row_inv_rsp<16, A, B>;                                                                   \
        hipLaunchKernelGGL(kp, dim3(wgs), dim3(C::S::NTHR), Z::bytes, st, a, npairs, units); \
        return 1;                                                                                            \
      }                                                                                                      \
    }                                                                                                        \
    constexpr int np = C::NP;                                                                                \
    auto kern = k_row_inv_rs<16, A, B, np>;                                                                  \
    hipLaunchKernelGGL(kern, dim3(grid_x(npairs, np, a.tstride), batch), dim3(C::S::NTHR * np), C::LDS, st, a); \
    return 1;                                                                                                \
  }
  PS_RS_SIZES(X)
#undef X
  return 0;
}
```

parasitoids_amd/csrc/ps_solver.hip:

```cpp
#include <deque>

#include "chain_kernels.h"
#include "fft_kernels.h"
#include "fft_colfull_kernels.h"
#include "rs_launch.h"
#include "ps_common.h"
#include "ps_config.h"

thread_local std::string ps_tls_error;

extern "C" const char* ps_last_error(void) { return ps_tls_error.c_str(); }
extern "C" int ps_version(void) { return 100; }

extern "C" int ps_device_count(void) {
  int n = 0;
  hipError_t e = hipGetDeviceCount(&n);
  if (e != hipSuccess) return ps_fail(PS_ERR_NO_DEVICE, "hipGetDeviceCount: %s", hipGetErrorString(e));
  return n;
}

extern "C" int ps_device_info(int device, char* name, int n, int* cus, int64_t* hbm_bytes) {
  hipDeviceProp_t p;
  PS_HIP(hipGetDeviceProperties(&p, device));
  if (name && n > 0) snprintf(name, n, "%s (%s)", p.name, p.gcnArchName);
  if (cus) *cus = p.multiProcessorCount;
  if (hbm_bytes) *hbm_bytes = (int64_t)p.totalGlobalMem;
  return PS_OK;
}

int ps_use_device(int device) {
  int n = 0;
  hipError_t e = hipGetDeviceCount(&n);
  if (e != hipSuccess || n <= 0)
    return ps_fail(PS_ERR_NO_DEVICE, "no HIP device available (%s)", hipGetErrorString(e));
  if (device < 0 || device >= n) return ps_fail(PS_ERR_NO_DEVICE, "device %d out of range (%d devices)", device, n);
  PS_HIP(hipSetDevice(device));
  return PS_OK;
}

static const int kMaxLds = 160 * 1024;

#include <map>
#include <mutex>
#include <unordered_map>
namespace {
struct DevPool {
  std::mutex mu;
  std::map<int, std::multimap<size_t, void*>> free_;
  std::unordered_map<void*, std::pair<int, size_t>> live;
  size_t cached = 0;
  size_t limit() {
    static const size_t gb = getenv("PS_POOL_GB") ? (size_t)atoi(getenv("PS_POOL_GB")) : 16;
    return gb << 30;
  }
  void flush_locked() {
    for (auto& dv : free_)
      for (auto& kv : dv.second) (void)hipFree(kv.second);
    free_.clear();
    cached = 0;
  }
};
DevPool& pool() {
  static DevPool* p = new DevPool();
  return *p;
}
size_t round_size(size_t b) {
  const size_t g = b >= (1u << 20) ? (size_t)1 << 20 : 256;
  return (b + g - 1) / g * g;
}
}

static hipError_t poison(void* p, size_t n) {
  static const bool on = getenv("PS_POISON") != nullptr;
  if (!on) return hipSuccess;
  hipError_t e = hipMemset(p, 0xFF, n);
  if (e == hipSuccess) e = hipDeviceSynchronize();
  return e;
}

hipError_t ps_dev_malloc(void** out, size_t bytes) {
  DevPool& P = pool();
  int dev = 0;
  (void)hipGetDevice(&dev);
  const size_t want = round_size(bytes ? bytes : 1);
  std::lock_guard<std::mutex> lk(P.mu);
  auto& fr = P.free_[dev];
  auto it = fr.lower_bound(want);
  if (it != fr.end() && it->first <= want + want / 4 + (1u << 20)) {
    *out = it->second;
    P.live[*out] = {dev, it->first};
    P.cached -= it->first;
    const size_t got = it->first;
    fr.erase(it);
    return poison(*out, got);
  }
  hipError_t e = hipMalloc(out, want);
  if (e != hipSuccess) {
    (void)hipGetLastError();
    P.flush_locked();
    e = hipMalloc(out, want);
  }
  if (e == hipSuccess) {
    P.live[*out] = {dev, want};
    e = poison(*out, want);
  }
  return e;
}

void ps_dev_free(void* p) {
  if (!p) return;
  DevPool& P = pool();
  std::lock_guard<std::mutex> lk(P.mu);
  auto it = P.live.find(p);
  if (it == P.live.end()) {
    (void)hipFree(p);
    return;
  }
  const int dev = it->second.first;
  const size_t sz = it->second.second;
  P.live.erase(it);
  if (P.cached + sz > P.limit()) {
    (void)hipFree(p);
    return;
  }
  P.free_[dev].emplace(sz, p);
  P.cached += sz;
}

void ps_dev_quiesce() { (void)hipDeviceSynchronize(); }
static const int kPredGrid = 512;
static const double kCleanEps = 1e-15;
#define PS_PROF_NCLS 16
enum { PS_PROF_ROW_FWD = 0, PS_PROF_COL_FWD_A = 1, PS_PROF_COL_FWD_B = 2, PS_PROF_COL_INV_A = 3,
       PS_PROF_COL_INV_B = 4, PS_PROF_ROW_INV = 5, PS_PROF_REFFT = 6, PS_PROF_COL_INV_A2 = 7,
       PS_PROF_COL_INV_A4 = 8, PS_PROF_COL_INV_A8 = 9, PS_PROF_ROW_INV2 = 10, PS_PROF_ROW_INV4 = 11,
       PS_PROF_ROW_INV8 = 12,
       PS_PROF_COL_INV_AN = 13,
       PS_PROF_ROW_INVN = 14,
       PS_PROF_COL_TAIL = 15 };
#define PS_MAX_GROUP_DAYS 32

struct ColPass {
  DevPlan* plan;
  int n_outer, in_base_mul, in_stride, out_base_mul, out_stride, tw_mode;
  bool second = false;
};

struct ps_solver {
  int device = 0;
  hipStream_t stream = nullptr;
  int N = 0, M = 0, Pref = 0, Pf = 0, H = 0, ld = 0, mode = 0;
  DevPlan row_plan, col_plan1, col_plan2;
  bool split = false;
  bool tpipe = false;
  bool tpipe_ok = false;
  bool tinv = false;
  ps_config cfg;
  bool spec_valid = false;
  bool row_big = false;
  int num_cu = 256;
  bool speculate = true;
  int fused_days = 8;
  int spec_window = 1;
  hipEvent_t spec_ev[2] = {nullptr, nullptr};
  hipStream_t stream2 = nullptr;
  hipEvent_t kt_ev = nullptr, kt_ev0 = nullptr;
  int kt_from = -1;
  int kt_lazy_from = -1, kt_lazy_c0 = 0, kt_lazy_cn = 0, kt_lazy_direct = 0;
  unsigned long long* hflags = nullptr;
  int hflags_n = 0;
  unsigned long long* hhist = nullptr;
  int hhist_n = 0, hist_first = -1, hist_count = 0;
  hipEvent_t hist_ev = nullptr;
  int rs_r2 = 0, rs_r3 = 0;
  int L1 = 0, L2 = 0;
  DevBuf<cplx> tp_lo, tp_hi;
  int tp_shift = 0;
  std::vector<ColPass> fwd_passes, inv_passes;
  DevBuf<cplx> Ahat, Chat, T1, T2, Bhat;
  int chunk_days = 1;
  DevBuf<int> srange;
  bool srange_valid = false;
  DevBuf<int> krow, kcol;
  DevBuf<double> kval;
  std::vector<int64_t> koff;
  std::vector<int> kshape;
  int nk = 0, Kmax = 0;
  bool kernels_on_device = false;
  DevBuf<double> kdense;
  DevBuf<long long> dkoff;
  DevBuf<int> dkshape;
  int bhat_first = -1, bhat_count = 0;
  std::vector<double*> recs[4];
  DevBuf<double> rowsum;
  DevBuf<long long> rowcnt;
  DevBuf<long long> rowoff;
  DevBuf<unsigned long long> padmax;
  DevBuf<DayStats> dstats;
  int nstat = 0;
  int last_renorm = 0;
  RowLive kt_live{0, {0, 0, 0, 0}, nullptr};
  bool kt_direct = false;
  DevBuf<int> krange;
  std::vector<int> hkrange;
  DevBuf<int> orow, ocol;
  DevBuf<double> oval;
  DevBuf<const double*> wptr;
  DevBuf<double> wval;
  bool have_state = false;
  bool auto_exact = false;
  double pad_floor = 0.5e-8;
  ps_solver* child = nullptr;
  ps_solver* wide = nullptr;
  ps_solver* narrow = nullptr;
  bool narrow_kernels = false;
  bool borrowed = false;
  bool child_kernels = false, wide_kernels = false;
  std::vector<signed char> owner;
  std::vector<signed char> route_hist;
  int route_first = -1, route_end = -1;
  int auto_first_regime = 2;
  int auto_first = -1;
  int auto_hint = -1;
  int noflag_hint = 0;
  long long auto_runs = 0;
  struct FiltKey { uint64_t h1, h2; int64_t n; };
  std::vector<FiltKey> filt_keys;
  DevBuf<cplx> Fhat;
  long long filt_hits = 0, filt_misses = 0;
  DevBuf<double> torus, lin, fold_rowsum;
  DevBuf<long long> fold_rowcnt;
  DevBuf<unsigned long long> fold_padmax;
  DevBuf<double> pad_energy;
  DevBuf<int> pad_quiet;
  DevBuf<cplx> tail_hat;
  DevBuf<cplx> Trow;
  DevBuf<cplx> blk;
  int blk_first = -1, blk_count = 0;
  DevBuf<unsigned long long> one_flag;
  const unsigned long long* refft_pending = nullptr;
  int ncu = 0;
  bool prof_on = false;
  struct ProfRec { int cls; hipEvent_t a, b; int days; };
  std::vector<ProfRec> prof_pending;
  std::vector<hipEvent_t> prof_pool;
  double prof_ms[PS_PROF_NCLS] = {0};
  long long prof_cnt[PS_PROF_NCLS] = {0};
  long long prof_seen[PS_PROF_NCLS] = {0};
  long long prof_days[PS_PROF_NCLS] = {0};
  int prof_every = 1;
};

static hipEvent_t prof_event(ps_solver* s) {
  if (!s->prof_pool.empty()) {
    hipEvent_t e = s->prof_pool.back();
    s->prof_pool.pop_back();
    return e;
  }
  hipEvent_t e = nullptr;
  (void)hipEventCreateWithFlags(&e, hipEventDisableSystemFence);
  return e;
}
struct ProfScope {
  ps_solver* s;
  ps_solver::ProfRec r;
  bool on;
  ProfScope(ps_solver* s_, int cls, int days = 1) : s(s_), on(false) {
    r.days = days;
    if (!s->prof_on) return;
    on = cls >= PS_PROF_COL_INV_A2 || (s->prof_seen[cls]++ % s->prof_every) == 0;
    if (!on) return;
    r.cls = cls;
    r.a = prof_event(s);
    r.b = prof_event(s);
    (void)hipEventRecord(r.a, s->stream);
  }
  ~ProfScope() {
    if (!on) return;
    (void)hipEventRecord(r.b, s->stream);
    s->prof_pending.push_back(r);
  }
};

static int row_threads(int L, bool big = false) { return L <= 1024 ? 256 : ((L <= 2560 || big) ? 512 : 1024); }
static int row_pairs(const FftProg& P) {
  int rp = 2048 / std::max(1, P.L);
  rp = std::max(1, std::min(8, rp));
  return rp;
}
static int col_wsh(const ps_solver* s, int L) {
  int w = 4096 / std::max(1, L);
  int sh = 2;
  while ((1 << (sh + 1)) <= w && sh < 5) ++sh;
  if (s->cfg.col_wsh >= 0) sh = s->cfg.col_wsh;
  return sh;
}
static int col_threads(const ps_solver* s) { return s->cfg.col_threads; }

static int set_lds_attr() {
  static bool done = false;
  if (done) return PS_OK;
  const void* ks[] = {(const void*)k_row_fwd<false, false>, (const void*)k_row_fwd<true, false>,
                      (const void*)k_row_fwd<false, true>,
                      (const void*)k_row_inv<false, false>, (const void*)k_row_inv<true, false>,
                      (const void*)k_row_inv<false, true>,
                      (const void*)k_col<PS_FWD, false>, (const void*)k_col<PS_FWD, true>,
                      (const void*)k_col<PS_INV, false>, (const void*)k_col<PS_INV, true>,
                      (const void*)k_col_fused<false>, (const void*)k_col_fused<true>,
                      (const void*)k_col_fused_dual<false>, (const void*)k_col_fused_dual<true>,
#define PS_MULTI_K(ND) \
  (const void*)k_col_fused_multi<false, ND, 1>, (const void*)k_col_fused_multi<true, ND, 1>, \
  (const void*)k_col_fused_multi<false, ND, 2>, (const void*)k_col_fused_multi<true, ND, 2>
                      PS_MULTI_K(1), PS_MULTI_K(2), PS_MULTI_K(4), PS_MULTI_K(8)};
#undef PS_MULTI_K
  for (const void* k : ks) PS_HIP(hipFuncSetAttribute(k, hipFuncAttributeMaxDynamicSharedMemorySize, kMaxLds));
  if (rs_rows_set_attrs() != 0 || rs_colfull_set_attrs() != 0 || rs_coldual_set_attrs() != 0) return ps_fail(PS_ERR_HIP, "hipFuncSetAttribute failed for a register-resident kernel");
  done = true;
  return PS_OK;
}

static int launch_row_fwd(ps_solver* s, const double* src, int64_t src_bstride, int src_ld,
                          SrcMap rmap, SrcMap cmap, cplx* dst, int batch,
                          const unsigned long long* pred, int skip_zero = 0, const int* rowrange = nullptr,
                          const unsigned long long* trunc_pred = nullptr, int trunc_n = 0) {
  RowFwdArgs a;
  if (trunc_pred && s->rs_r2 == 0) return ps_fail(PS_ERR_STATE, "row pass: only the register-resident kernels truncate on the fly");
  a.trunc_pred = trunc_pred; a.trunc_n = trunc_n;
  a.src = src; a.src_bstride = src_bstride; a.src_ld = src_ld;
  a.rmap = rmap; a.cmap = cmap;
  a.dst = dst; a.dst_bstride = (int64_t)s->Pf * s->ld;
  a.H = s->H; a.ld = s->ld; a.P = s->Pf;
  a.tstride = s->tpipe ? s->Pf : 0;
  a.prog = s->row_plan.prog;
  a.rp = row_pairs(a.prog);
  a.pred = pred;
  a.skip_zero = skip_zero;
  a.rowrange = rowrange;
  const int npairs = (s->Pf + 1) / 2;
  a.nblocks = (npairs + a.rp - 1) / a.rp;
  dim3 grid(pred ? std::min(a.nblocks, kPredGrid) : a.nblocks, batch);
  const int thr = row_threads(a.prog.L, s->row_big);
  const size_t lds = ((size_t)a.rp * row_pitch(a.prog) + a.prog.n_lo + a.prog.n_hi + a.prog.n_gen) * sizeof(cplx);
  if (lds > (size_t)kMaxLds) return ps_fail(PS_ERR_UNSUPPORTED, "row pass needs %zu B LDS", lds);
  ProfScope prof(s, pred ? PS_PROF_REFFT : PS_PROF_ROW_FWD);
  if (s->rs_r2 != 0 && !s->cfg.no_rs_fwd) {
    if (!rs_launch_row_fwd(s->rs_r2, s->rs_r3, a, npairs, batch, s->stream))
      return ps_fail(PS_ERR_STATE, "no register-resident row kernel for 16 x %d x %d", s->rs_r2, s->rs_r3);
  } else if (s->row_plan.generic)
    hipLaunchKernelGGL((k_row_fwd<true, false>), grid, dim3(thr), lds, s->stream, a);
  else if (s->row_big)
    hipLaunchKernelGGL((k_row_fwd<false, true>), grid, dim3(thr), lds, s->stream, a);
  else
    hipLaunchKernelGGL((k_row_fwd<false, false>), grid, dim3(thr), lds, s->stream, a);
  PS_HIP(hipGetLastError());
  return PS_OK;
}

template <int DIR>
static int launch_col(ps_solver* s, const ColPass& cp, const cplx* src, const cplx* src2,
                      cplx* prod, cplx* dst, int batch, int64_t src2_bstride,
                      const unsigned long long* pred, RowLive live = RowLive{0, {0, 0, 0, 0}, nullptr}) {
  ColArgs a;
  a.src = src; a.src2 = src2; a.prod_dst = prod; a.dst = dst;
  const int64_t bs = (int64_t)s->Pf * s->ld;
  a.src_bstride = bs; a.src2_bstride = src2_bstride; a.prod_bstride = bs; a.dst_bstride = bs;
  a.ld = s->ld; a.ncols = s->H;
  a.prog = cp.plan->prog;
  a.wsh = col_wsh(s, a.prog.L);
  a.n_outer = cp.n_outer;
  a.in_base_mul = cp.in_base_mul; a.in_stride = cp.in_stride;
  a.out_base_mul = cp.out_base_mul; a.out_stride = cp.out_stride;
  a.tw_mode = cp.tw_mode;
  a.tp_lo = s->tp_lo.p; a.tp_hi = s->tp_hi.p; a.tp_shift = s->tp_shift;
  a.pred = pred;
  a.live = live;
  const int W = 1 << a.wsh;
  const int ntiles = (s->H + W - 1) / W;
  dim3 grid((unsigned)(ntiles * cp.n_outer), batch);
  size_t lds = (((size_t)a.prog.L << a.wsh) + a.prog.n_lo + a.prog.n_hi + a.prog.n_gen + a.prog.L) * sizeof(cplx) + (size_t)a.prog.L * sizeof(int);
  while (lds > (size_t)kMaxLds && a.wsh > 0) {
    --a.wsh;
    lds = (((size_t)a.prog.L << a.wsh) + a.prog.n_lo + a.prog.n_hi + a.prog.n_gen + a.prog.L) * sizeof(cplx) + (size_t)a.prog.L * sizeof(int);
  }
  if (lds > (size_t)kMaxLds) return ps_fail(PS_ERR_UNSUPPORTED, "column pass needs %zu B LDS", lds);
  {
    const int W2 = 1 << a.wsh;
    a.nblocks = ((s->H + W2 - 1) / W2) * cp.n_outer;
    grid.x = (unsigned)(pred ? std::min(a.nblocks, kPredGrid) : a.nblocks);
  }
  ProfScope prof(s, pred ? PS_PROF_REFFT
                          : (DIR == PS_FWD ? PS_PROF_COL_FWD_A : PS_PROF_COL_INV_A) + (cp.second ? 1 : 0));
  if (cp.plan->generic)
    hipLaunchKernelGGL((k_col<DIR, true>), grid, dim3(col_threads(s)), lds, s->stream, a);
  else
    hipLaunchKernelGGL((k_col<DIR, false>), grid, dim3(col_threads(s)), lds, s->stream, a);
  PS_HIP(hipGetLastError());
  return PS_OK;
}

static bool row_inv_persistent(const ps_solver* s) {
  const int knob = s->cfg.rsp;
  RsInfo info;
  if (s->rs_r2 == 0 || !rs_info(s->rs_r2, s->rs_r3, &info) || !info.rsp || knob == 0) return false;
  return knob == 1 || (s->tpipe && s->Pf >= 1536);
}

static int inter_layout(const ps_solver* s) {
  if (!s->tpipe) return 0;
  if (s->tinv) return 1;
  return (s->mode != PS_MODE_FOLD && !s->cfg.no_pair_rows && s->Pf % 2 == 0) ? 2 : 0;
}

static int launch_row_inv(ps_solver* s, const cplx* src, double* rec, int stat_slot, int batch,
                          double negval, double stat_scale, bool full_field = false,
                          double* const* recs_multi = nullptr, const int* pad_quiet = nullptr) {
  RowInvArgs a;
  a.pad_quiet = pad_quiet;
  a.persistent = (row_inv_persistent(s) && !(s->tpipe && s->tinv && !full_field)) ? 1 : 0;
  if (a.persistent && (s->cfg.row2 > 0 || (s->cfg.row2 < 0 && s->Pf >= 4096))) a.persistent = 2;
  a.nrec = 0;
  for (int i = 0; i < PS_MAX_GROUP_DAYS; ++i) a.rec_multi[i] = nullptr;
  if (recs_multi) {
    if (!a.persistent || batch > PS_MAX_GROUP_DAYS) return ps_fail(PS_ERR_STATE, "row pass: a record table needs the persistent kernel and at most %d entries", PS_MAX_GROUP_DAYS);
    a.nrec = batch;
    for (int i = 0; i < batch; ++i) a.rec_multi[i] = recs_multi[i];
  }
  a.src = src; a.src_bstride = (int64_t)s->Pf * s->ld;
  a.H = s->H; a.ld = s->ld; a.P = s->Pf; a.N = s->N;
  a.tstride = (s->tpipe && s->tinv && !full_field) ? s->Pf : 0;
  a.pair_src = (!full_field && inter_layout(s) == 2) ? 1 : 0;
  a.prog = s->row_plan.prog;
  a.rp = row_pairs(a.prog);
  a.scale = 1.0 / ((double)s->Pf * (double)s->Pf);
  a.rec = rec; a.rec_bstride = (int64_t)s->N * s->N;
  a.negval = negval; a.stat_scale = stat_scale;
  a.rowsum = s->rowsum.p + (int64_t)stat_slot * s->N;
  a.rowcnt = s->rowcnt.p + (int64_t)stat_slot * s->N;
  a.padmax = s->padmax.p + stat_slot;
  a.pad_floor = s->pad_floor;
  a.stat_bstride = s->N;
  if (full_field) {
    a.N = s->Pf;
    a.rec_bstride = (int64_t)s->Pf * s->Pf;
    a.rowsum = s->fold_rowsum.p; a.rowcnt = s->fold_rowcnt.p; a.padmax = s->fold_padmax.p;
    a.stat_bstride = s->Pf;
  }
  const int npairs = (s->Pf + 1) / 2;
  dim3 grid((npairs + a.rp - 1) / a.rp, batch);
  const int thr = row_threads(a.prog.L, s->row_big);
  const size_t lds = ((size_t)a.rp * row_pitch(a.prog) + a.prog.n_lo + a.prog.n_hi + a.prog.n_gen) * sizeof(cplx) +
                     4 * (thr / 64) * sizeof(double);
  if (lds > (size_t)kMaxLds) return ps_fail(PS_ERR_UNSUPPORTED, "row pass needs %zu B LDS", lds);
  ProfScope prof(s, !recs_multi ? PS_PROF_ROW_INV : batch == 2 ? PS_PROF_ROW_INV2 : batch == 4 ? PS_PROF_ROW_INV4
                                : batch == 8 ? PS_PROF_ROW_INV8 : batch == 1 ? PS_PROF_ROW_INV : PS_PROF_ROW_INVN,
                 recs_multi ? batch : 1);
  if (s->rs_r2 != 0) {
    if (!rs_launch_row_inv(s->rs_r2, s->rs_r3, a, npairs, batch, s->stream))
      return ps_fail(PS_ERR_STATE, "no register-resident row kernel for 16 x %d x %d", s->rs_r2, s->rs_r3);
  } else if (s->row_plan.generic)
    hipLaunchKernelGGL((k_row_inv<true, false>), grid, dim3(thr), lds, s->stream, a);
  else if (s->row_big)
    hipLaunchKernelGGL((k_row_inv<false, true>), grid, dim3(thr), lds, s->stream, a);
  else
    hipLaunchKernelGGL((k_row_inv<false, false>), grid, dim3(thr), lds, s->stream, a);
  PS_HIP(hipGetLastError());
  return PS_OK;
}

static bool colfull_dual(const ps_solver* s, int nd) {
  const int dual_min = s->cfg.dual_min_days;
  return dual_min > 0 && nd >= dual_min && rs_dual_ok(s->rs_r2, s->rs_r3);
}

static SrcMap map_plain(int n, int P);
struct ColAlt { const cplx* src; const unsigned long long* pred; RowLive live; };

static int launch_colfull(ps_solver* s, int mode, const cplx* src, cplx* state, int store_prod, cplx* dst, int batch,
                          RowLive live, const unsigned long long* pred, int nd = 1, double* pad_energy = nullptr,
                          int col0 = 0, int ncols = -1, int64_t state_bstride = -1, bool timed = true,
                          const ColAlt* alt = nullptr) {
  ColFullArgs a;
  a.pad_energy = nullptr;
  a.alt_src = nullptr; a.alt_pred = nullptr; a.alt_live = RowLive{0, {0, 0, 0, 0}, nullptr};
  if (alt) {
    if (!(mode == 0 && nd == 1 && batch == 1 && !pred) || s->refft_pending)
      return ps_fail(PS_ERR_STATE, "full-column pass: an alternative state source needs a plain single-day pass");
    a.alt_src = alt->src; a.alt_pred = alt->pred; a.alt_live = alt->live;
  }
  if (s->refft_pending) {
    if (!(mode == 0 && nd == 1 && batch == 1 && !pred && state == s->Ahat.p))
      return ps_fail(PS_ERR_STATE, "full-column pass: a flagged day's re-transform is still pending");
    a.alt_src = s->Trow.p; a.alt_pred = s->refft_pending;
    a.alt_live = RowLive{1, map_plain(s->N, s->Pf), nullptr};
  }
  a.pad_row0 = 2 * ((s->N + 1) / 2);
  a.ncols_total = s->H;
  a.col0 = col0;
  const int64_t spec = (int64_t)s->Pf * s->ld;
  a.src = src; a.src_bstride = spec;
  a.state = state; a.state_bstride = state_bstride >= 0 ? state_bstride : spec;
  a.dst = dst; a.dst_bstride = spec;
  a.ld = s->ld; a.ncols = ncols >= 0 ? ncols : s->H; a.mode = mode; a.store_prod = store_prod;
  a.nd = nd; a.src_dstride = spec; a.dst_dstride = spec;
  colfull_set_layout(a, s->tinv ? 1 : inter_layout(s), s->Pf);
  a.live = live;
  a.pred = pred;
  a.prog = s->row_plan.prog;
  const int groups = (a.ncols - col0 + 7) / 8;
  const int lines8 = (groups + 7) / 8;
  if (mode == 2) a.pad_energy = pad_energy;
  const bool prof_was = s->prof_on;
  if (!timed) s->prof_on = false;
  ProfScope prof(s, pred ? PS_PROF_REFFT
                          : (mode == 1 ? PS_PROF_COL_FWD_A
                                       : (nd == 2 ? PS_PROF_COL_INV_A2 : nd == 4 ? PS_PROF_COL_INV_A4
                                          : nd == 8 ? PS_PROF_COL_INV_A8 : nd == 1 ? PS_PROF_COL_INV_A : PS_PROF_COL_INV_AN)),
                 nd);
  s->prof_on = prof_was;
  if (mode == 0 && !pred && store_prod && colfull_dual(s, nd)) {
    a.pad_energy = pad_energy;
    if (!rs_launch_coldual(s->rs_r2, s->rs_r3, a, lines8, batch, s->stream))
      return ps_fail(PS_ERR_STATE, "two-role full-column pass: size 16 x %d x %d is not served", s->rs_r2, s->rs_r3);
    PS_HIP(hipGetLastError());
    return PS_OK;
  }
  if (!rs_launch_colfull(s->rs_r2, s->rs_r3, a, lines8, batch, s->stream))
    return ps_fail(PS_ERR_UNSUPPORTED, "full-column pass: size 16 x %d x %d cannot run this (chained days need the state column in LDS)",
                   s->rs_r2, s->rs_r3);
  PS_HIP(hipGetLastError());
  return PS_OK;
}

static bool colfull_chains(const ps_solver* s) {
  RsInfo info;
  return rs_info(s->rs_r2, s->rs_r3, &info) && info.chain;
}

static int fwd2d(ps_solver* s, const double* src, int64_t src_bstride, int src_ld, SrcMap rmap,
                 SrcMap cmap, cplx* out, int batch, const unsigned long long* pred, const int* rowrange = nullptr) {
  PS_TRY(launch_row_fwd(s, src, src_bstride, src_ld, rmap, cmap, s->T1.p, batch, pred, 1, rowrange));
  if (s->tpipe) return launch_colfull(s, 1, s->T1.p, out, 0, nullptr, batch, RowLive{1, rmap, rowrange}, pred);
  if (s->fwd_passes.size() == 1) {
    PS_TRY(launch_col<PS_FWD>(s, s->fwd_passes[0], s->T1.p, nullptr, nullptr, out, batch, 0, pred, RowLive{1, rmap, rowrange}));
  } else {
    PS_TRY(launch_col<PS_FWD>(s, s->fwd_passes[0], s->T1.p, nullptr, nullptr, s->T2.p, batch, 0, pred, RowLive{1, rmap, rowrange}));
    PS_TRY(launch_col<PS_FWD>(s, s->fwd_passes[1], s->T2.p, nullptr, nullptr, out, batch, 0, pred));
  }
  return PS_OK;
}

static int inv2d(ps_solver* s, const cplx* A, const cplx* B, cplx* prod, double* rec,
                 int stat_slot, double negval, double stat_scale) {
  if (s->tpipe) {
    if (B || prod) return ps_fail(PS_ERR_STATE, "inv2d: product form is not used by the full-column pipeline");
    PS_TRY(launch_colfull(s, 2, nullptr, const_cast<cplx*>(A), 0, s->T1.p, 1, RowLive{0, {0, 0, 0, 0}, nullptr}, nullptr));
    return launch_row_inv(s, s->T1.p, rec, stat_slot, 1, negval, stat_scale);
  }
  if (s->inv_passes.size() == 1) {
    PS_TRY(launch_col<PS_INV>(s, s->inv_passes[0], A, B, prod, s->T1.p, 1, 0, nullptr));
    PS_TRY(launch_row_inv(s, s->T1.p, rec, stat_slot, 1, negval, stat_scale));
  } else {
    PS_TRY(launch_col<PS_INV>(s, s->inv_passes[0], A, B, prod, s->T1.p, 1, 0, nullptr));
    PS_TRY(launch_col<PS_INV>(s, s->inv_passes[1], s->T1.p, nullptr, nullptr, s->T2.p, 1, 0, nullptr));
    PS_TRY(launch_row_inv(s, s->T2.p, rec, stat_slot, 1, negval, stat_scale));
  }
  return PS_OK;
}

static int fwd2d_partial(ps_solver* s, const double* src, int64_t src_bstride, int src_ld,
                         SrcMap rmap, SrcMap cmap, cplx* out, int batch, const int* rowrange = nullptr,
                         bool direct = false) {
  const RowLive live{1, rmap, rowrange};
  s->kt_live = RowLive{0, {0, 0, 0, 0}, nullptr};
  s->kt_direct = s->split && direct && !s->tpipe;
  if (s->tpipe) {
    s->kt_live = live;
    return launch_row_fwd(s, src, src_bstride, src_ld, rmap, cmap, out, batch, nullptr, 1, rowrange);
  }
  if (!s->split || direct) {
    s->kt_live = live;
    return launch_row_fwd(s, src, src_bstride, src_ld, rmap, cmap, out, batch, nullptr, 1, rowrange);
  }
  PS_TRY(launch_row_fwd(s, src, src_bstride, src_ld, rmap, cmap, s->T1.p, batch, nullptr, 1, rowrange));
  return launch_col<PS_FWD>(s, s->fwd_passes[0], s->T1.p, nullptr, nullptr, out, batch, 0, nullptr, live);
}

static void fused_direct_args(ps_solver* s, ColFusedArgs& a) {
  a.direct = s->kt_direct ? 1 : 0;
  a.no_conj = s->cfg.no_conj;
  a.tp_lo = s->tp_lo.p; a.tp_hi = s->tp_hi.p; a.tp_shift = s->tp_shift;
  a.mgL2 = ps_magic((uint32_t)a.L2);
}
static size_t fused_direct_lds(const ColFusedArgs& a) { return a.direct ? ((size_t)a.L1 + a.L2 + 1) * sizeof(cplx) + 64 : 0; }

static int launch_col_fused(ps_solver* s, const cplx* kt, cplx* state, int store_prod, cplx* dst,
                            const int* rowrange) {
  ColFusedArgs a;
  DevPlan* plan = s->split ? &s->col_plan2 : &s->col_plan1;
  a.src = kt; a.state = state; a.dst = dst;
  a.src_bstride = 0;
  a.ld = s->ld; a.ncols = s->H;
  a.L1 = s->split ? s->L1 : 1;
  a.L2 = s->split ? s->L2 : s->Pf;
  a.store_prod = store_prod;
  a.live = s->kt_live;
  a.live.range = rowrange;
  a.prog = plan->prog;
  a.dst_dstride = 0;
  a.live2 = RowLive{0, {0, 0, 0, 0}, nullptr};
  fused_direct_args(s, a);
  a.wsh = std::min(col_wsh(s, a.prog.L), 4);
  if (s->cfg.fused_wsh >= 0) a.wsh = s->cfg.fused_wsh;
  auto need = [&](int wsh) {
    return (((size_t)a.prog.L << wsh) + a.prog.n_lo + a.prog.n_hi + a.prog.n_gen) * sizeof(cplx) +
           (size_t)(a.prog.L + 4) * sizeof(int) + fused_direct_lds(a);
  };
  while (need(a.wsh) > (size_t)kMaxLds && a.wsh > 0) --a.wsh;
  if (need(a.wsh) > (size_t)kMaxLds) return ps_fail(PS_ERR_UNSUPPORTED, "column pass needs %zu B LDS", need(a.wsh));
  const int W = 1 << a.wsh;
  const int ntiles = (s->H + W - 1) / W;
  dim3 grid((unsigned)((a.direct ? (ntiles + 7) / 8 * 8 : ntiles) * a.L1), 1);
  ProfScope prof(s, PS_PROF_COL_INV_A);
  const int fthr = s->cfg.fused_threads > 0 ? s->cfg.fused_threads : col_threads(s);
  if (plan->generic)
    hipLaunchKernelGGL(k_col_fused<true>, grid, dim3(fthr), need(a.wsh), s->stream, a);
  else
    hipLaunchKernelGGL(k_col_fused<false>, grid, dim3(fthr), need(a.wsh), s->stream, a);
  PS_HIP(hipGetLastError());
  return PS_OK;
}

static int launch_col_fused_multi(ps_solver* s, const cplx* kt, int nd, cplx* state, cplx* dst,
                                  const int* rowrange, int* done) {
  ColFusedArgs a;
  DevPlan* plan = s->split ? &s->col_plan2 : &s->col_plan1;
  const int64_t spec = (int64_t)s->Pf * s->ld;
  a.src = kt; a.state = state; a.dst = dst;
  a.src_bstride = spec;
  a.dst_dstride = spec;
  a.ld = s->ld; a.ncols = s->H;
  a.L1 = s->split ? s->L1 : 1;
  a.L2 = s->split ? s->L2 : s->Pf;
  a.store_prod = 1;
  a.live = s->kt_live;
  a.live.range = rowrange;
  a.live2 = RowLive{0, {0, 0, 0, 0}, nullptr};
  a.prog = plan->prog;
  fused_direct_args(s, a);
  const int ndsh = nd == 1 ? 0 : nd == 2 ? 1 : (nd == 4 ? 2 : 3);
  const int gopt = s->cfg.fused_g;
  const int G = (a.direct && gopt == 2 && a.L1 % 2 == 0) ? 2 : 1;
  const int gsh = G == 2 ? 1 : 0;
  a.wsh = std::min(col_wsh(s, a.prog.L), nd >= 4 ? 3 : 4);
  if (s->cfg.multi_wsh >= 0) a.wsh = s->cfg.multi_wsh;
  auto need = [&](int wsh) {
    return (((size_t)a.prog.L << (wsh + ndsh + gsh)) + a.prog.n_lo + a.prog.n_hi + a.prog.n_gen) * sizeof(cplx) +
           (size_t)(a.prog.L + 4) * sizeof(int) + G * fused_direct_lds(a) +
           (a.direct ? (size_t)a.L2 * nd * sizeof(unsigned) : 0);
  };
  const size_t lds_cap = (size_t)kMaxLds / 2;
  while (need(a.wsh) > lds_cap && a.wsh > 2) --a.wsh;
  *done = 0;
  if (need(a.wsh) > lds_cap) return PS_OK;
  const int W = 1 << a.wsh;
  const int ntiles = (s->H + W - 1) / W;
  dim3 grid((unsigned)((a.direct ? (ntiles + 7) / 8 * 8 : ntiles) * (a.L1 / G)), 1);
  ProfScope prof(s, nd == 1 ? PS_PROF_COL_INV_A : nd == 2 ? PS_PROF_COL_INV_A2 : nd == 4 ? PS_PROF_COL_INV_A4 : PS_PROF_COL_INV_A8);
  const int fenv = s->cfg.fused_threads;
  const int fthr = fenv > 0 ? fenv : (G == 2 && nd > 1 ? 512 : col_threads(s));
#define PS_MULTI_LAUNCH(ND, GG)                                                                                          \
  if (plan->generic) hipLaunchKernelGGL((k_col_fused_multi<true, ND, GG>), grid, dim3(fthr), need(a.wsh), s->stream, a); \
  else hipLaunchKernelGGL((k_col_fused_multi<false, ND, GG>), grid, dim3(fthr), need(a.wsh), s->stream, a)
  if (G == 2) {
    if (nd == 1) { PS_MULTI_LAUNCH(1, 2); }
    else if (nd == 2) { PS_MULTI_LAUNCH(2, 2); }
    else if (nd == 4) { PS_MULTI_LAUNCH(4, 2); }
    else { PS_MULTI_LAUNCH(8, 2); }
  } else {
    if (nd == 1) { PS_MULTI_LAUNCH(1, 1); }
    else if (nd == 2) { PS_MULTI_LAUNCH(2, 1); }
    else if (nd == 4) { PS_MULTI_LAUNCH(4, 1); }
    else { PS_MULTI_LAUNCH(8, 1); }
  }
#undef PS_MULTI_LAUNCH
  PS_HIP(hipGetLastError());
  *done = 1;
  return PS_OK;
}

static int launch_col_fused_dual(ps_solver* s, const cplx* kt, const cplx* state_part, RowLive state_live,
                                 cplx* dst, const int* rowrange, int* done) {
  ColFusedArgs a;
  DevPlan* plan = s->split ? &s->col_plan2 : &s->col_plan1;
  a.src = kt; a.state = const_cast<cplx*>(state_part); a.dst = dst;
  a.src_bstride = 0;
  a.ld = s->ld; a.ncols = s->H;
  a.L1 = s->split ? s->L1 : 1;
  a.L2 = s->split ? s->L2 : s->Pf;
  a.store_prod = 0;
  a.live = s->kt_live;
  a.live.range = rowrange;
  a.live2 = state_live;
  a.prog = plan->prog;
  a.dst_dstride = 0;
  fused_direct_args(s, a);
  a.wsh = std::min(col_wsh(s, a.prog.L), 4);
  if (s->cfg.dual_wsh >= 0) a.wsh = s->cfg.dual_wsh;
  auto need = [&](int wsh) {
    return (((size_t)a.prog.L << (wsh + 1)) + a.prog.n_lo + a.prog.n_hi + a.prog.n_gen) * sizeof(cplx);
  };
  while (need(a.wsh) > (size_t)kMaxLds && a.wsh > 2) --a.wsh;
  *done = 0;
  if (need(a.wsh) > (size_t)kMaxLds || s->cfg.no_dual) return PS_OK;
  const int W = 1 << a.wsh;
  const int ntiles = (s->H + W - 1) / W;
  dim3 grid((unsigned)((a.direct ? (ntiles + 7) / 8 * 8 : ntiles) * a.L1), 1);
  ProfScope prof(s, PS_PROF_COL_INV_A);
  const int fthr = s->cfg.fused_threads > 0 ? s->cfg.fused_threads : col_threads(s);
  if (plan->generic)
    hipLaunchKernelGGL(k_col_fused_dual<true>, grid, dim3(fthr), need(a.wsh), s->stream, a);
  else
    hipLaunchKernelGGL(k_col_fused_dual<false>, grid, dim3(fthr), need(a.wsh), s->stream, a);
  PS_HIP(hipGetLastError());
  *done = 1;
  return PS_OK;
}

static int conv_inv(ps_solver* s, const cplx* kt, cplx* state, int store_prod, double* rec,
                    int stat_slot, double negval, double stat_scale, const int* rowrange = nullptr) {
  if (s->tpipe) {
    RowLive live = s->kt_live;
    live.range = rowrange;
    const int split2 = s->cfg.tpipe_split;
    if (split2 && store_prod) {
      PS_TRY(launch_colfull(s, 3, kt, state, 1, nullptr, 1, live, nullptr));
      PS_TRY(launch_colfull(s, 2, nullptr, state, 0, s->T1.p, 1, RowLive{0, {0, 0, 0, 0}, nullptr}, nullptr));
    } else {
      PS_TRY(launch_colfull(s, 0, kt, state, store_prod, s->T1.p, 1, live, nullptr));
    }
    return launch_row_inv(s, s->T1.p, rec, stat_slot, 1, negval, stat_scale);
  }
  int done = 0;
  if (s->kt_direct && store_prod) PS_TRY(launch_col_fused_multi(s, kt, 1, state, s->T1.p, rowrange, &done));
  if (!done) PS_TRY(launch_col_fused(s, kt, state, store_prod, s->T1.p, rowrange));
  if (!s->split) return launch_row_inv(s, s->T1.p, rec, stat_slot, 1, negval, stat_scale);
  PS_TRY(launch_col<PS_INV>(s, s->inv_passes[1], s->T1.p, nullptr, nullptr, s->T2.p, 1, 0, nullptr));
  return launch_row_inv(s, s->T2.p, rec, stat_slot, 1, negval, stat_scale);
}

static int conv_inv_multi(ps_solver* s, const cplx* kt, int nd, cplx* state, double* const* recs, int d0,
                          double negval, double stat_scale, const int* rowrange, int* done) {
  const size_t spec = (size_t)s->Pf * s->ld;
  PS_TRY(s->T1.ensure(spec * nd));
  if (s->tpipe) {
    *done = 0;
    if (!colfull_chains(s)) return PS_OK;
    RowLive live = s->kt_live;
    live.range = rowrange;
    const bool batched_rows = row_inv_persistent(s) && !s->tinv && nd <= PS_MAX_GROUP_DAYS && !s->cfg.no_row_batch;
    const bool quiet = batched_rows && colfull_dual(s, nd) && s->N + 1 < s->Pf && !s->cfg.no_pad_quiet;
    if (quiet) {
      PS_TRY(s->pad_energy.ensure((size_t)nd * s->H));
      PS_TRY(s->pad_quiet.ensure(PS_MAX_GROUP_DAYS));
    }
    int hmain = s->H;
    if (!s->ncu) {
      int v = 0;
      if (hipDeviceGetAttribute(&v, hipDeviceAttributeMultiprocessorCount, s->device) == hipSuccess) s->ncu = v;
    }
    if (colfull_dual(s, nd) && s->ncu > 0 && s->H > s->ncu && !s->tinv && !s->cfg.no_tail_split) {
      const int rem = s->H % s->ncu;
      if (rem > 0 && rem * 3 <= s->ncu) hmain = s->H - rem;
    }
    PS_TRY(launch_colfull(s, 0, kt, state, 1, s->T1.p, 1, live, nullptr, nd, quiet ? s->pad_energy.p : nullptr, 0, hmain));
    if (hmain < s->H) {
      const int rem = s->H - hmain;
      PS_TRY(s->tail_hat.ensure((size_t)nd * rem * s->Pf));
      cplx* th = s->tail_hat.p - (int64_t)hmain * s->Pf;
      {
        ProfScope prof(s, PS_PROF_COL_TAIL, nd);
        PS_TRY(launch_colfull(s, 1, kt, th, 0, nullptr, nd, live, nullptr, 1, nullptr, hmain, s->H, (int64_t)rem * s->Pf, false));
        hipLaunchKernelGGL(k_prefix_cols, dim3((s->Pf + 255) / 256, rem), dim3(256), 0, s->stream,
                           state + (int64_t)hmain * s->Pf, s->tail_hat.p, s->Pf, rem, nd);
        PS_HIP(hipGetLastError());
        PS_TRY(launch_colfull(s, 2, nullptr, th, 0, s->T1.p, nd, RowLive{0, {0, 0, 0, 0}, nullptr}, nullptr, 1,
                              quiet ? s->pad_energy.p : nullptr, hmain, s->H, (int64_t)rem * s->Pf, false));
      }
    }
    if (quiet) {
      hipLaunchKernelGGL(k_pad_quiet, dim3(nd), dim3(256), 0, s->stream, s->pad_energy.p, s->H, (double)s->Pf,
                         1.0 / ((double)s->Pf * (double)s->Pf), s->pad_floor, s->pad_quiet.p);
      PS_HIP(hipGetLastError());
    }
    if (batched_rows) {
      PS_TRY(launch_row_inv(s, s->T1.p, nullptr, d0, nd, negval, stat_scale, false, recs, quiet ? s->pad_quiet.p : nullptr));
    } else {
      for (int i = 0; i < nd; ++i)
        PS_TRY(launch_row_inv(s, s->T1.p + i * spec, recs[i], d0 + i, 1, negval, stat_scale));
    }
    *done = 1;
    return PS_OK;
  }
  PS_TRY(launch_col_fused_multi(s, kt, nd, state, s->T1.p, rowrange, done));
  if (!*done) return PS_OK;
  for (int i = 0; i < nd; ++i) {
    cplx* t = s->T1.p + i * spec;
    if (s->split) {
      PS_TRY(launch_col<PS_INV>(s, s->inv_passes[1], t, nullptr, nullptr, s->T2.p, 1, 0, nullptr));
      t = s->T2.p;
    }
    PS_TRY(launch_row_inv(s, t, recs[i], d0 + i, 1, negval, stat_scale));
  }
  return PS_OK;
}

static SrcMap map_plain(int n, int P) { return SrcMap{n, 0, P, 0}; }
static SrcMap map_wrap(int m, int P) { return SrcMap{m + 1, m, P - m, 0}; }

static int ensure_record(ps_solver* s, int kind, int idx) {
  auto& v = s->recs[kind];
  if ((int)v.size() <= idx) v.resize(idx + 1, nullptr);
  if (!v[idx]) {
    hipError_t e = ps_dev_malloc((void**)&v[idx], (size_t)s->N * s->N * sizeof(double));
    if (e != hipSuccess) return ps_fail(PS_ERR_OOM, "record allocation failed: %s", hipGetErrorString(e));
  }
  return PS_OK;
}

static int ensure_stats(ps_solver* s, int n) {
  if (n <= s->nstat) return PS_OK;
  PS_TRY(s->rowsum.ensure((size_t)(n + 1) * s->N));
  PS_TRY(s->rowcnt.ensure((size_t)(n + 1) * s->N));
  PS_TRY(s->padmax.ensure(n + 1));
  PS_TRY(s->dstats.ensure(n + 1));
  s->nstat = n;
  return PS_OK;
}

static int finalize_days(ps_solver* s, int slot, int count, int renorm) {
  if (count <= 0) return PS_OK;
  hipLaunchKernelGGL(k_day_finalize, dim3(count), dim3(256), 0, s->stream,
                     s->rowsum.p + (int64_t)slot * s->N, s->rowcnt.p + (int64_t)slot * s->N,
                     s->padmax.p + slot, s->N, renorm, s->dstats.p + slot);
  PS_HIP(hipGetLastError());
  return PS_OK;
}

static int refft_if_flag(ps_solver* s, const double* rec, cplx* hat, int slot) {
  return fwd2d(s, rec, 0, s->N, map_plain(s->N, s->Pf), map_plain(s->N, s->Pf), hat, 1,
               s->padmax.p + slot);
}

static int refft_rows_if_flag(ps_solver* s, const double* rec, int slot) {
  PS_TRY(s->Trow.ensure((size_t)s->Pf * s->ld));
  const SrcMap m = map_plain(s->N, s->Pf);
  PS_TRY(launch_row_fwd(s, rec, 0, s->N, m, m, s->Trow.p, 1, s->padmax.p + slot, 1, nullptr));
  s->refft_pending = s->padmax.p + slot;
  return PS_OK;
}
static int resolve_refft(ps_solver* s) {
  if (!s->refft_pending) return PS_OK;
  const unsigned long long* pred = s->refft_pending;
  s->refft_pending = nullptr;
  return launch_colfull(s, 1, s->Trow.p, s->Ahat.p, 0, nullptr, 1, RowLive{1, map_plain(s->N, s->Pf), nullptr}, pred);
}

static int fast_size(const ps_config& cfg, int Pref) {
  if (cfg.fast_size >= Pref) return cfg.fast_size;
  int Pf = ps_next_fast_len(Pref);
  if (!cfg.no_rs) {
    const int L = rs_next_size(Pref);
    const double area = cfg.rs_area > 0.0 ? cfg.rs_area : (Pf < 2048 ? 1.2 : 1.08);
    if (L > 0 && ((double)L * L <= area * (double)Pf * Pf || Pf > 9700)) Pf = L;
  }
  return Pf;
}

extern "C" int ps_fast_size(int dom_len, int max_shape) {
  if (dom_len < 1 || max_shape < 1) return 0;
  ps_config cfg;
  ps_config_from_env(&cfg);
  return fast_size(cfg, dom_len + max_shape / 2);
}

static int solver_create(ps_solver** out, int device, int dom_len, int max_shape, int mode, const ps_config& cfg);

extern "C" int ps_solver_create(ps_solver** out, int device, int dom_len, int max_shape, int mode) {
  ps_config cfg;
  ps_config_from_env(&cfg);
  return solver_create(out, device, dom_len, max_shape, mode, cfg);
}

static int solver_create(ps_solver** out, int device, int dom_len, int max_shape, int mode, const ps_config& cfg) {
  if (!out) return ps_fail(PS_ERR_BAD_ARG, "null output handle");
  *out = nullptr;
  if (dom_len < 1 || max_shape < 1) return ps_fail(PS_ERR_BAD_SHAPE, "dom_len=%d max_shape=%d", dom_len, max_shape);
  if (mode != PS_MODE_EXACT && mode != PS_MODE_FAST && mode != PS_MODE_FOLD && mode != PS_MODE_AUTO)
    return ps_fail(PS_ERR_BAD_ARG, "mode %d", mode);
  const bool auto_exact = mode == PS_MODE_AUTO;
  if (auto_exact) mode = PS_MODE_FAST;
  PS_TRY(ps_use_device(device));
  PS_TRY(set_lds_attr());
  ps_solver* s = new ps_solver();
  s->cfg = cfg;
  s->tinv = cfg.tinv != 0;
  s->fused_days = cfg.fused_days;
  s->device = device;
  s->N = dom_len;
  s->M = max_shape / 2;
  s->Pref = dom_len + s->M;
  s->mode = mode;
  s->auto_exact = auto_exact;
  if (auto_exact) s->pad_floor = 0.5 * kCleanEps;
  s->Pf = mode == PS_MODE_FAST ? fast_size(cfg, s->Pref) : s->Pref;
  if (mode == PS_MODE_FOLD) s->Pf = fast_size(cfg, s->Pref + 2 * s->M);
  s->H = s->Pf / 2 + 1;
  s->ld = (s->H + 7) & ~7;
  auto fail = [&](int rc) {
    ps_solver_destroy(s);
    return rc;
  };
  {
    HostFftPlan small, big;
    const bool ok_s = ps_build_plan(s->Pf, true, &small), ok_b = ps_build_plan(s->Pf, true, &big, true);
    if (ok_s && ok_b && small.max_prime <= 9 && s->Pf > 1024 && big.prog.ns < small.prog.ns &&
        !cfg.no_big_radix) {
      s->row_plan.host = big;
      s->row_big = true;
    }
  }
  if (!s->row_big && !ps_build_plan(s->Pf, true, &s->row_plan.host))
    return fail(ps_fail(PS_ERR_UNSUPPORTED, "cannot plan a length-%d FFT (prime factor > %d); use PS_MODE_FAST",
                        s->Pf, PS_MAX_GENERIC_RADIX));
  {
    int r2 = 0, r3 = 0;
    const bool rs = !cfg.no_rs && rs_lookup(s->Pf, &r2, &r3);
    if (!rs && (size_t)(row_pitch(s->row_plan.host.prog) + 512) * sizeof(cplx) > (size_t)kMaxLds)
      return fail(ps_fail(PS_ERR_UNSUPPORTED, "pad size %d exceeds the LDS-resident row limit", s->Pf));
  }
  int rc = s->row_plan.upload();
  if (rc) return fail(rc);
  if (cfg.no_rs || !rs_lookup(s->Pf, &s->rs_r2, &s->rs_r3)) s->rs_r2 = s->rs_r3 = 0;
  s->tpipe_ok = (mode == PS_MODE_FAST || mode == PS_MODE_FOLD) && s->rs_r2 != 0 && !cfg.no_rs &&
                !cfg.no_rs_fwd && !cfg.no_tpipe;
  if (mode == PS_MODE_FOLD && cfg.no_fold_tpipe) s->tpipe_ok = false;
  s->tpipe = s->tpipe_ok;
  {
    int ncu = 0;
    if (hipDeviceGetAttribute(&ncu, hipDeviceAttributeMultiprocessorCount, device) == hipSuccess && ncu > 0) s->num_cu = ncu;
  }
  {
    s->L1 = ps_choose_col_split(s->Pf, cfg.col_single_max);
  }
  if (cfg.col_l1 > 1 && cfg.col_l1 < s->Pf && s->Pf % cfg.col_l1 == 0) s->L1 = cfg.col_l1;
  s->split = s->L1 != s->Pf;
  if (s->split) {
    s->L2 = s->Pf / s->L1;
    if (!ps_build_plan(s->L1, false, &s->col_plan1.host) || !ps_build_plan(s->L2, false, &s->col_plan2.host))
      return fail(ps_fail(PS_ERR_UNSUPPORTED, "cannot plan column FFT %d = %d x %d", s->Pf, s->L1, s->L2));
    if ((rc = s->col_plan1.upload())) return fail(rc);
    if ((rc = s->col_plan2.upload())) return fail(rc);
    s->fwd_passes = {ColPass{&s->col_plan1, s->L2, 1, s->L2, 1, s->L2, 1},
                     ColPass{&s->col_plan2, s->L1, s->L2, 1, 1, s->L1, 0, true}};
    s->inv_passes = {ColPass{&s->col_plan2, s->L1, 1, s->L1, s->L2, 1, 0},
                     ColPass{&s->col_plan1, s->L2, 1, s->L2, 1, s->L2, 2, true}};
  } else {
    s->L2 = 1;
    if (!ps_build_plan(s->Pf, false, &s->col_plan1.host))
      return fail(ps_fail(PS_ERR_UNSUPPORTED, "cannot plan column FFT %d", s->Pf));
    if ((rc = s->col_plan1.upload())) return fail(rc);
    s->fwd_passes = {ColPass{&s->col_plan1, 1, 0, 1, 0, 1, 0}};
    s->inv_passes = {ColPass{&s->col_plan1, 1, 0, 1, 0, 1, 0}};
  }
  {
    HostTwiddle tw;
    ps_build_twiddle(s->Pf, &tw);
    s->tp_shift = tw.shift;
    if ((rc = s->tp_lo.ensure(tw.lo.size()))) return fail(rc);
    if ((rc = s->tp_hi.ensure(tw.hi.size()))) return fail(rc);
    hipError_t e1 = hipMemcpy(s->tp_lo.p, tw.lo.data(), tw.lo.size() * sizeof(cplx), hipMemcpyHostToDevice);
    hipError_t e2 = hipMemcpy(s->tp_hi.p, tw.hi.data(), tw.hi.size() * sizeof(cplx), hipMemcpyHostToDevice);
    if (e1 != hipSuccess || e2 != hipSuccess) return fail(ps_fail(PS_ERR_HIP, "twiddle upload failed"));
  }
  hipError_t e = hipStreamCreateWithFlags(&s->stream, hipStreamNonBlocking);
  if (e != hipSuccess) return fail(ps_fail(PS_ERR_HIP, "hipStreamCreate: %s", hipGetErrorString(e)));
  const size_t spec = (size_t)s->Pf * s->ld;
  size_t budget = (size_t)3 << 30;
  {
    size_t mfree = 0, mtotal = 0;
    if (hipMemGetInfo(&mfree, &mtotal) == hipSuccess && mtotal / 16 > budget) budget = mtotal / 16;
  }
  s->chunk_days = (int)std::max<size_t>(1, std::min<size_t>(64, budget / (spec * sizeof(cplx))));
  if (cfg.chunk_days > 0) s->chunk_days = cfg.chunk_days;
  if ((rc = s->Ahat.ensure(spec))) return fail(rc);
  if ((rc = s->rowoff.ensure(s->N))) return fail(rc);
  if ((rc = ensure_stats(s, 4))) return fail(rc);
  *out = s;
  return PS_OK;
}

extern "C" int ps_solver_destroy(ps_solver* s) {
  if (!s) return PS_OK;
  (void)hipSetDevice(s->device);
  if (s->stream) (void)hipStreamSynchronize(s->stream);
  if (s->child) {
    ps_solver_destroy(s->child);
    s->child = nullptr;
  }
  if (s->wide) {
    ps_solver_destroy(s->wide);
    s->wide = nullptr;
  }
  if (s->narrow) {
    ps_solver_destroy(s->narrow);
    s->narrow = nullptr;
  }
  if (s->borrowed) {
    s->stream = nullptr;
    for (auto& p : s->recs[PS_REC_CHAIN]) p = nullptr;
  }
  if (s->stream2) {
    (void)hipStreamSynchronize(s->stream2);
    (void)hipStreamDestroy(s->stream2);
  }
  if (s->kt_ev) (void)hipEventDestroy(s->kt_ev);
  if (s->kt_ev0) (void)hipEventDestroy(s->kt_ev0);
  if (s->stream) (void)hipStreamDestroy(s->stream);
  ps_dev_quiesce();
  s->row_plan.release(); s->col_plan1.release(); s->col_plan2.release();
  s->tp_lo.release(); s->tp_hi.release();
  s->Ahat.release(); s->Chat.release(); s->T1.release(); s->T2.release(); s->Bhat.release(); s->Fhat.release();
  s->Trow.release(); s->blk.release(); s->one_flag.release(); s->tail_hat.release(); s->pad_energy.release(); s->pad_quiet.release();
  s->srange.release();
  s->krow.release(); s->kcol.release(); s->kval.release(); s->kdense.release(); s->krange.release();
  for (auto& v : s->recs)
    for (double* p : v)
      if (p) ps_dev_free(p);
  s->rowsum.release(); s->rowcnt.release(); s->rowoff.release(); s->padmax.release();
  s->dstats.release();
  s->orow.release(); s->ocol.release(); s->oval.release(); s->wptr.release(); s->wval.release();
  for (auto& r : s->prof_pending) { (void)hipEventDestroy(r.a); (void)hipEventDestroy(r.b); }
  for (auto e : s->prof_pool) (void)hipEventDestroy(e);
  for (auto e : s->spec_ev) if (e) (void)hipEventDestroy(e);
  if (s->hflags) (void)hipHostFree(s->hflags);
  if (s->hhist) (void)hipHostFree(s->hhist);
  if (s->hist_ev) (void)hipEventDestroy(s->hist_ev);
  s->dkoff.release(); s->dkshape.release();
  s->torus.release(); s->lin.release(); s->fold_rowsum.release(); s->fold_rowcnt.release(); s->fold_padmax.release();
  delete s;
  return PS_OK;
}

extern "C" int ps_solver_retarget(ps_solver* s, int max_shape) {
  if (!s || max_shape < 1) return ps_fail(PS_ERR_BAD_ARG, "retarget: bad arguments");
  if (s->auto_exact) {
    const int m = max_shape / 2;
    if (s->N + m > s->Pf)
      return ps_fail(PS_ERR_BAD_SHAPE, "retarget: max_shape %d needs an FFT size >= %d, the solver has %d", max_shape,
                     s->N + m, s->Pf);
    PS_HIP(hipSetDevice(s->device));
    PS_HIP(hipStreamSynchronize(s->stream));
    if (s->child && ps_solver_retarget(s->child, max_shape) != PS_OK) {
      ps_solver_destroy(s->child);
      s->child = nullptr;
    }
    if (s->wide) {
      ps_solver_destroy(s->wide);
      s->wide = nullptr;
    }
    if (s->narrow) {
      ps_solver_destroy(s->narrow);
      s->narrow = nullptr;
    }
    s->narrow_kernels = false;
    s->child_kernels = false;
    s->wide_kernels = false;
    s->route_first = s->route_end = -1;
    s->M = m;
    s->Pref = s->N + m;
    s->have_state = false;
    s->bhat_first = -1;
    s->bhat_count = 0;
    return PS_OK;
  }
  if (s->mode != PS_MODE_FOLD) return ps_fail(PS_ERR_UNSUPPORTED, "retarget: only PS_MODE_FOLD solvers can change their torus");
  const int m = max_shape / 2;
  if (s->N + 3 * m > s->Pf)
    return ps_fail(PS_ERR_BAD_SHAPE, "retarget: max_shape %d needs an FFT size >= %d, the solver has %d", max_shape,
                   s->N + 3 * m, s->Pf);
  PS_HIP(hipSetDevice(s->device));
  PS_HIP(hipStreamSynchronize(s->stream));
  s->M = m;
  s->Pref = s->N + m;
  s->have_state = false;
  s->bhat_first = -1;
  s->bhat_count = 0;
  return PS_OK;
}

extern "C" int ps_solver_info(ps_solver* s, int* dom_len, int* P, int* Pfft, int* H) {
  if (!s) return ps_fail(PS_ERR_BAD_ARG, "null solver");
  if (dom_len) *dom_len = s->N;
  if (P) *P = s->Pref;
  if (Pfft) *Pfft = s->Pf;
  if (H) *H = s->H;
  return PS_OK;
}

extern "C" int ps_solver_sync(ps_solver* s) {
  if (!s) return ps_fail(PS_ERR_BAD_ARG, "null solver");
  PS_HIP(hipSetDevice(s->device));
  PS_HIP(hipStreamSynchronize(s->stream));
  return PS_OK;
}

static int ensure_temps(ps_solver* s, int batch) {
  const size_t spec = (size_t)s->Pf * s->ld;
  PS_TRY(s->T1.ensure(spec * batch));
  if (s->split) PS_TRY(s->T2.ensure(spec * batch));
  return PS_OK;
}

static int check_coo(const int32_t* row, const int32_t* col, int64_t nnz, int lim, const char* what) {
  for (int64_t i = 0; i < nnz; ++i)
    if (row[i] < 0 || row[i] >= lim || col[i] < 0 || col[i] >= lim)
      return ps_fail(PS_ERR_BAD_SHAPE, "%s: entry %lld (%d,%d) outside %d x %d", what, (long long)i, row[i],
                     col[i], lim, lim);
  return PS_OK;
}

static int scatter_from_device(ps_solver* s, const int* row, const int* col, const double* val,
                               int64_t nnz, double* dst, int ld, int off) {
  if (nnz <= 0) return PS_OK;
  const int thr = 256;
  const int blocks = (int)std::min<int64_t>((nnz + thr - 1) / thr, 4096);
  hipLaunchKernelGGL(k_scatter_coo, dim3(blocks), dim3(thr), 0, s->stream, row, col, val, nnz, dst, ld, off, off);
  PS_HIP(hipGetLastError());
  return PS_OK;
}

static int upload_coo(ps_solver* s, const int32_t* row, const int32_t* col, const double* val, int64_t nnz) {
  PS_TRY(s->orow.ensure(std::max<int64_t>(nnz, 1)));
  PS_TRY(s->ocol.ensure(std::max<int64_t>(nnz, 1)));
  PS_TRY(s->oval.ensure(std::max<int64_t>(nnz, 1)));
  if (nnz > 0) {
    PS_HIP(hipMemcpyAsync(s->orow.p, row, nnz * 4, hipMemcpyHostToDevice, s->stream));
    PS_HIP(hipMemcpyAsync(s->ocol.p, col, nnz * 4, hipMemcpyHostToDevice, s->stream));
    PS_HIP(hipMemcpyAsync(s->oval.p, val, nnz * 8, hipMemcpyHostToDevice, s->stream));
    PS_HIP(hipStreamSynchronize(s->stream));
  }
  return PS_OK;
}

int ps_solver_set_state_device_coo(ps_solver* s, const int* row, const int* col, const double* val,
                                   int64_t nnz, int off) {
  PS_TRY(ensure_record(s, PS_REC_STATE, 0));
  PS_TRY(ensure_temps(s, 1));
  s->srange_valid = false;
  double* rec = s->recs[PS_REC_STATE][0];
  PS_HIP(hipMemsetAsync(rec, 0, (size_t)s->N * s->N * sizeof(double), s->stream));
  PS_TRY(scatter_from_device(s, row, col, val, nnz, rec, s->N, off));
  if (s->mode == PS_MODE_FOLD) {
    PS_TRY(s->torus.ensure((size_t)s->Pref * s->Pref));
    PS_HIP(hipMemsetAsync(s->torus.p, 0, (size_t)s->Pref * s->Pref * sizeof(double), s->stream));
    PS_HIP(hipMemcpy2DAsync(s->torus.p, (size_t)s->Pref * sizeof(double), rec, (size_t)s->N * sizeof(double),
                            (size_t)s->N * sizeof(double), (size_t)s->N, hipMemcpyDeviceToDevice, s->stream));
    s->have_state = true;
    return PS_OK;
  }
  s->spec_valid = false;
  s->have_state = true;
  return PS_OK;
}

static int ensure_spectrum(ps_solver* s) {
  if (s->spec_valid || s->mode == PS_MODE_FOLD) return PS_OK;
  if (s->recs[PS_REC_STATE].empty() || !s->recs[PS_REC_STATE][0]) return ps_fail(PS_ERR_STATE, "no state record");
  PS_TRY(ensure_temps(s, 1));
  PS_TRY(fwd2d(s, s->recs[PS_REC_STATE][0], 0, s->N, map_plain(s->N, s->Pf), map_plain(s->N, s->Pf), s->Ahat.p, 1, nullptr,
               s->srange_valid ? s->srange.p : nullptr));
  s->spec_valid = true;
  return PS_OK;
}

static void set_pipeline(ps_solver* s, bool tpipe) {
  if (!s->tpipe_ok) tpipe = false;
  if (s->tpipe == tpipe) return;
  s->tpipe = tpipe;
  s->bhat_first = -1;
  s->bhat_count = 0;
  s->filt_keys.clear();
}

extern "C" int ps_solver_set_state_coo(ps_solver* s, const int32_t* row, const int32_t* col,
                                       const double* val, int64_t nnz) {
  if (!s || nnz < 0 || (nnz > 0 && (!row || !col || !val))) return ps_fail(PS_ERR_BAD_ARG, "set_state_coo: bad arguments");
  PS_HIP(hipSetDevice(s->device));
  PS_TRY(check_coo(row, col, nnz, s->N, "state"));
  PS_TRY(upload_coo(s, row, col, val, nnz));
  PS_TRY(ps_solver_set_state_device_coo(s, s->orow.p, s->ocol.p, s->oval.p, nnz, 0));
  int range[2] = {1, 0};
  for (int64_t i = 0; i < nnz; ++i) {
    if (range[0] > range[1]) range[0] = range[1] = row[i];
    range[0] = std::min(range[0], (int)row[i]);
    range[1] = std::max(range[1], (int)row[i]);
  }
  PS_TRY(s->srange.ensure(2));
  hipLaunchKernelGGL(k_set_int2, dim3(1), dim3(64), 0, s->stream, s->srange.p, range[0], range[1]);
  PS_HIP(hipGetLastError());
  s->srange_valid = true;
  return PS_OK;
}

static bool direct_possible(const ps_solver* s) {
  return s->split && s->mode != PS_MODE_FOLD && !s->cfg.no_direct &&
         s->L1 <= 255 && s->L2 <= 255;
}
static bool day_is_compact(const ps_solver* s, int d) {
  const int max_terms = s->cfg.direct_max_terms;
  const int M = s->Kmax / 2;
  const int lo = s->hkrange[2 * d], hi = s->hkrange[2 * d + 1];
  if (lo > hi) return true;
  const int below = std::max(0, std::min(hi, M - 1) - lo + 1), above = std::max(0, hi - std::max(lo, M) + 1);
  const int terms = (below + s->L2 - 1) / s->L2 + (above + s->L2 - 1) / s->L2;
  return terms <= max_terms;
}

static int transform_kernels(ps_solver* s, int first, int count, int slot0, int total, int direct_chunk) {
  const int K = s->Kmax, M = K / 2;
  const size_t spec = (size_t)s->Pf * s->ld;
  if (total < 0) total = count;
  PS_TRY(s->kdense.ensure((size_t)total * K * K));
  PS_TRY(s->Bhat.ensure(spec * total));
  PS_TRY(ensure_temps(s, total));
  double* kd = s->kdense.p + (size_t)slot0 * K * K;
  int blo = K, bhi = -1;
  int64_t maxn = 0;
  for (int d = first; d < first + count; ++d) {
    if (s->hkrange[2 * d] <= s->hkrange[2 * d + 1]) {
      blo = std::min(blo, s->hkrange[2 * d]);
      bhi = std::max(bhi, s->hkrange[2 * d + 1]);
    }
    maxn = std::max<int64_t>(maxn, s->koff[d + 1] - s->koff[d]);
  }
  if (bhi >= blo) {
    blo = std::max(blo, 0);
    bhi = std::min(bhi, K - 1);
    const int64_t n = (int64_t)(bhi - blo + 1) * K;
    const int blocks = (int)std::min<int64_t>((n + 255) / 256, 2048);
    hipLaunchKernelGGL(k_zero_band, dim3(blocks, count), dim3(256), 0, s->stream, kd, K, blo, bhi);
    PS_HIP(hipGetLastError());
  }
  if (maxn > 0) {
    const int thr = 256;
    const int blocks = (int)std::min<int64_t>((maxn + thr - 1) / thr, 1024);
    hipLaunchKernelGGL(k_scatter_coo_batch, dim3(blocks, count), dim3(thr), 0, s->stream, s->krow.p, s->kcol.p,
                       s->kval.p, s->dkoff.p, s->dkshape.p, first, kd, K);
    PS_HIP(hipGetLastError());
  }
  bool direct = direct_possible(s);
  if (direct_chunk >= 0) direct = direct && direct_chunk != 0;
  else for (int d = first; d < first + count && direct; ++d) direct = day_is_compact(s, d);
  PS_TRY(fwd2d_partial(s, kd, (int64_t)K * K, K, map_wrap(M, s->Pf), map_wrap(M, s->Pf), s->Bhat.p + (size_t)slot0 * spec, count,
                       s->krange.p + 2 * first, direct));
  s->bhat_first = first - slot0;
  s->bhat_count = slot0 + count;
  return PS_OK;
}

static int transform_kernels(ps_solver* s, int first, int count, int slot0 = 0, int total = -1, int direct_chunk = -1);
static int kernels_ready(ps_solver* s, int d) {
  if (s->kt_lazy_from >= 0 && d >= s->kt_lazy_from) {
    const int from = s->kt_lazy_from, done = from - s->kt_lazy_c0;
    s->kt_lazy_from = -1;
    PS_TRY(transform_kernels(s, from, s->kt_lazy_cn - done, done, s->kt_lazy_cn, s->kt_lazy_direct));
  }
  if (s->kt_from >= 0 && d >= s->kt_from) {
    PS_HIP(hipStreamWaitEvent(s->stream, s->kt_ev, 0));
    s->kt_from = -1;
  }
  return PS_OK;
}

static int drain_kernel_readers(ps_solver* s) {
  if (s->stream2) PS_HIP(hipStreamSynchronize(s->stream2));
  PS_HIP(hipStreamSynchronize(s->stream));
  return PS_OK;
}

static int set_kernels_common(ps_solver* s, int nk, const int64_t* off, const int32_t* kshape,
                              const int32_t* rows) {
  s->koff.assign(off, off + nk + 1);
  s->kshape.assign(kshape, kshape + nk);
  s->nk = nk;
  s->Kmax = 1;
  for (int d = 0; d < nk; ++d) {
    if (kshape[d] < 1 || kshape[d] % 2 == 0)
      return ps_fail(PS_ERR_BAD_SHAPE, "kernel %d has even/invalid shape %d (CalcSol.py:58)", d, kshape[d]);
    if (kshape[d] / 2 > s->M)
      return ps_fail(PS_ERR_BAD_SHAPE, "kernel %d shape %d exceeds max_shape %d", d, kshape[d], 2 * s->M + 1);
    s->Kmax = std::max(s->Kmax, kshape[d]);
  }
  if (2 * (s->Kmax / 2) + 1 > s->Pf) return ps_fail(PS_ERR_BAD_SHAPE, "kernel larger than the pad");
  s->hkrange.assign(2 * (size_t)std::max(nk, 1), 0);
  const int M = s->Kmax / 2;
  for (int d = 0; d < nk; ++d) {
    const int o = M - kshape[d] / 2;
    int lo = 0, hi = kshape[d] - 1;
    if (rows && off[d + 1] > off[d]) {
      lo = kshape[d];
      hi = -1;
      for (int64_t i = off[d]; i < off[d + 1]; ++i) {
        lo = std::min(lo, (int)rows[i]);
        hi = std::max(hi, (int)rows[i]);
      }
    } else if (rows) {
      lo = 1;
      hi = 0;
    }
    s->hkrange[2 * d] = lo + o;
    s->hkrange[2 * d + 1] = hi + o;
  }
  PS_TRY(s->krange.ensure(s->hkrange.size()));
  PS_TRY(s->dkoff.ensure((size_t)nk + 1));
  PS_TRY(s->dkshape.ensure((size_t)std::max(nk, 1)));
  {
    std::vector<long long> o64(off, off + nk + 1);
    PS_HIP(hipMemcpy(s->dkoff.p, o64.data(), o64.size() * sizeof(long long), hipMemcpyHostToDevice));
    if (nk > 0) PS_HIP(hipMemcpy(s->dkshape.p, kshape, (size_t)nk * sizeof(int), hipMemcpyHostToDevice));
  }
  PS_HIP(hipMemcpyAsync(s->krange.p, s->hkrange.data(), s->hkrange.size() * sizeof(int), hipMemcpyHostToDevice, s->stream));
  PS_HIP(hipStreamSynchronize(s->stream));
  s->bhat_first = -1;
  s->bhat_count = 0;
  s->kernels_on_device = true;
  s->child_kernels = false;
  s->wide_kernels = false;
  s->narrow_kernels = false;
  return PS_OK;
}

extern "C" int ps_chain_set_kernels(ps_solver* s, int nk, const int64_t* off, const int32_t* kshape,
                                    const int32_t* row, const int32_t* col, const double* val) {
  if (!s || nk < 0 || !off || (nk > 0 && !kshape)) return ps_fail(PS_ERR_BAD_ARG, "set_kernels: bad arguments");
  PS_HIP(hipSetDevice(s->device));
  const int64_t tot = off[nk];
  for (int d = 0; d < nk; ++d) {
    if (off[d + 1] < off[d]) return ps_fail(PS_ERR_BAD_ARG, "offsets not monotone");
    PS_TRY(check_coo(row + off[d], col + off[d], off[d + 1] - off[d], kshape[d], "kernel"));
  }
  PS_TRY(drain_kernel_readers(s));
  PS_TRY(s->krow.ensure(std::max<int64_t>(tot, 1)));
  PS_TRY(s->kcol.ensure(std::max<int64_t>(tot, 1)));
  PS_TRY(s->kval.ensure(std::max<int64_t>(tot, 1)));
  if (tot > 0) {
    PS_HIP(hipMemcpyAsync(s->krow.p, row, tot * 4, hipMemcpyHostToDevice, s->stream));
    PS_HIP(hipMemcpyAsync(s->kcol.p, col, tot * 4, hipMemcpyHostToDevice, s->stream));
    PS_HIP(hipMemcpyAsync(s->kval.p, val, tot * 8, hipMemcpyHostToDevice, s->stream));
    PS_HIP(hipStreamSynchronize(s->stream));
  }
  return set_kernels_common(s, nk, off, kshape, row);
}

int ps_chain_adopt_device_kernels(ps_solver* s, int nk, const int64_t* off, const int32_t* kshape,
                                  const int* row, const int* col, const double* val) {
  const int64_t tot = off[nk];
  PS_TRY(drain_kernel_readers(s));
  PS_TRY(s->krow.ensure(std::max<int64_t>(tot, 1)));
  PS_TRY(s->kcol.ensure(std::max<int64_t>(tot, 1)));
  PS_TRY(s->kval.ensure(std::max<int64_t>(tot, 1)));
  if (tot > 0) {
    PS_HIP(hipMemcpyAsync(s->krow.p, row, tot * 4, hipMemcpyDeviceToDevice, s->stream));
    PS_HIP(hipMemcpyAsync(s->kcol.p, col, tot * 4, hipMemcpyDeviceToDevice, s->stream));
    PS_HIP(hipMemcpyAsync(s->kval.p, val, tot * 8, hipMemcpyDeviceToDevice, s->stream));
  }
  return set_kernels_common(s, nk, off, kshape, nullptr);
}

static int auto_attach(ps_solver* s, ps_solver** slot, int mode, int max_shape, bool* kernels_ok, int end) {
  if (!*slot) {
    ps_solver* c = nullptr;
    PS_TRY(solver_create(&c, s->device, s->N, max_shape, mode, s->cfg));
    (void)hipStreamSynchronize(c->stream);
    (void)hipStreamDestroy(c->stream);
    c->stream = s->stream;
    c->borrowed = true;
    c->speculate = false;
    c->pad_floor = 0.5 * kCleanEps;
    c->prof_on = s->prof_on;
    c->prof_every = s->prof_every;
    *slot = c;
    *kernels_ok = false;
  }
  ps_solver* c = *slot;
  if (!*kernels_ok) {
    PS_TRY(ps_chain_adopt_device_kernels(c, s->nk, s->koff.data(), s->kshape.data(), s->krow.p, s->kcol.p, s->kval.p));
    c->hkrange = s->hkrange;
    PS_HIP(hipMemcpyAsync(c->krange.p, c->hkrange.data(), c->hkrange.size() * sizeof(int), hipMemcpyHostToDevice, c->stream));
    PS_HIP(hipStreamSynchronize(c->stream));
    *kernels_ok = true;
  }
  PS_TRY(ensure_stats(c, std::max(4, end)));
  return PS_OK;
}

static const double* auto_prev_field(ps_solver* s, int first, int d) {
  if (d > 0 && d - 1 < (int)s->recs[PS_REC_CHAIN].size() && s->recs[PS_REC_CHAIN][d - 1] && (d > first || first > 0))
    return s->recs[PS_REC_CHAIN][d - 1];
  if (d == first && first == 0 && !s->recs[PS_REC_STATE].empty()) return s->recs[PS_REC_STATE][0];
  return nullptr;
}

static int auto_alias_records(ps_solver* s, ps_solver* c, int lo, int hi) {
  auto& cr = c->recs[PS_REC_CHAIN];
  if ((int)cr.size() < hi) cr.resize(hi, nullptr);
  for (int d = lo; d < hi; ++d) {
    PS_TRY(ensure_record(s, PS_REC_CHAIN, d));
    cr[d] = s->recs[PS_REC_CHAIN][d];
  }
  return PS_OK;
}

static int auto_read_padmax(ps_solver* s, ps_solver* c, int d, int w, double* out) {
  if (s->hflags_n < d + w) {
    if (s->hflags) (void)hipHostFree(s->hflags);
    s->hflags = nullptr;
    s->hflags_n = 0;
    PS_HIP(hipHostMalloc((void**)&s->hflags, (size_t)(d + w + 64) * sizeof(unsigned long long), hipHostMallocDefault));
    s->hflags_n = d + w + 64;
  }
  PS_HIP(hipMemcpyAsync(s->hflags + d, c->padmax.p + d, (size_t)w * sizeof(unsigned long long), hipMemcpyDeviceToHost, s->stream));
  PS_HIP(hipStreamSynchronize(s->stream));
  for (int i = 0; i < w; ++i) __builtin_memcpy(&out[i], &s->hflags[d + i], sizeof(double));
  return PS_OK;
}

static int auto_handover(ps_solver* s, int first, int f, int end, double negval, double stat_scale, int renorm,
                         double m_front) {
  const int wide_min_n = s->cfg.wide_min_n;
  const bool no_wide = s->cfg.no_wide || s->N < wide_min_n;
  const int kWin = std::min(64, std::max(1, s->cfg.auto_window));
  std::vector<signed char> hist;
  if (!s->cfg.no_route_history && s->route_first == first && s->route_end == end) hist = s->route_hist;
  if ((int)s->owner.size() < end) s->owner.resize(end, 0);
  for (int d = first; d < f; ++d) s->owner[d] = 0;
  enum { WIDE = 1, CHILD = 2, NARROW = 3 };
  std::vector<signed char> hint((size_t)end, 0);
  auto hist_owner = [&](int q) { return q >= 0 && q < (int)hist.size() && q < end ? (int)hist[q] : -1; };
  auto stretch = [&](int q, int who) {
    int e = q;
    while (e < end && e - q < 64 && hist_owner(e) == who) ++e;
    return e - q;
  };
  int regime = (no_wide || !(m_front > 1e-8)) ? CHILD : WIDE;
  s->auto_first_regime = regime;
  bool wide_live = false, child_live = false, narrow_live = false;
  int no_narrow_day = -1;
  int d = f;
  while (d < end) {
    const double* prev = auto_prev_field(s, first, d);
    if (regime == NARROW && hist_owner(d) != NARROW) {
      regime = WIDE;
      narrow_live = false;
    }
    if (regime == WIDE && hist_owner(d) == NARROW && d != no_narrow_day) {
      regime = NARROW;
      wide_live = false;
    }
    if (regime == WIDE && hist_owner(d) == CHILD) {
      regime = CHILD;
      wide_live = false;
      continue;
    }
    if (regime == NARROW) {
      PS_TRY(auto_attach(s, &s->narrow, PS_MODE_FAST, 2 * s->M + 1, &s->narrow_kernels, end));
      ps_solver* c = s->narrow;
      if (!narrow_live) {
        if (!prev) return ps_fail(PS_ERR_STATE, "auto mode: no field to continue day %d from", d);
        PS_TRY(ensure_record(c, PS_REC_STATE, 0));
        PS_HIP(hipMemcpyAsync(c->recs[PS_REC_STATE][0], prev, (size_t)s->N * s->N * sizeof(double), hipMemcpyDeviceToDevice, c->stream));
        c->spec_valid = false;
        c->srange_valid = false;
        c->have_state = true;
        narrow_live = true;
        wide_live = child_live = false;
      }
      const int w = std::min(std::max(1, stretch(d, NARROW)), end - d);
      PS_TRY(auto_alias_records(s, c, d, d + w));
      PS_TRY(ps_chain_run(c, d, w, negval, stat_scale, renorm));
      double m[64];
      PS_TRY(auto_read_padmax(s, c, d, std::min(w, 64), m));
      int x = -1;
      for (int i = 0; i < w && x < 0; ++i)
        if (m[i] >= kCleanEps && !(m[i] > 4e-8)) x = d + i;
      const int keep = x < 0 ? d + w : x;
      for (int q = d; q < keep; ++q) s->owner[q] = hint[q] = NARROW;
      d = keep;
      if (x >= 0) {
        regime = WIDE;
        narrow_live = false;
        no_narrow_day = x;
      }
      continue;
    }
    if (regime == WIDE) {
      PS_TRY(auto_attach(s, &s->wide, PS_MODE_FAST, 4 * s->M + 1, &s->wide_kernels, end));
      ps_solver* c = s->wide;
      if (!wide_live) {
        if (!prev) return ps_fail(PS_ERR_STATE, "auto mode: no field to continue day %d from", d);
        PS_TRY(ensure_record(c, PS_REC_STATE, 0));
        PS_HIP(hipMemcpyAsync(c->recs[PS_REC_STATE][0], prev, (size_t)s->N * s->N * sizeof(double), hipMemcpyDeviceToDevice, c->stream));
        c->spec_valid = false;
        c->srange_valid = false;
        c->have_state = true;
        wide_live = true;
        child_live = narrow_live = false;
      }
      const int hw = stretch(d, WIDE);
      const int w = std::min(hw > 0 ? hw : kWin, end - d);
      PS_TRY(auto_alias_records(s, c, d, d + w));
      PS_TRY(ps_chain_run(c, d, w, negval, stat_scale, renorm));
      double m[64];
      PS_TRY(auto_read_padmax(s, c, d, std::min(w, 64), m));
      int x = -1;
      for (int i = 0; i < w && x < 0; ++i)
        if (m[i] >= kCleanEps && !(m[i] > 1e-8)) x = d + i;
      const int keep = x < 0 ? d + w : x;
      for (int q = d; q < keep; ++q) {
        s->owner[q] = WIDE;
        const double mq = m[q - d];
        hint[q] = (mq > 4e-8 || mq < 0.25 * kCleanEps) ? NARROW : WIDE;
      }
      d = keep;
      if (x >= 0) {
        regime = CHILD;
        wide_live = false;
      }
    } else {
      PS_TRY(auto_attach(s, &s->child, PS_MODE_FOLD, 2 * s->M + 1, &s->child_kernels, end));
      ps_solver* c = s->child;
      if (!child_live) {
        if (!prev) return ps_fail(PS_ERR_STATE, "auto mode: no field to continue day %d from", d);
        PS_TRY(c->torus.ensure((size_t)c->Pref * c->Pref));
        PS_HIP(hipMemsetAsync(c->torus.p, 0, (size_t)c->Pref * c->Pref * sizeof(double), c->stream));
        PS_HIP(hipMemcpy2DAsync(c->torus.p, (size_t)c->Pref * sizeof(double), prev, (size_t)s->N * sizeof(double),
                                (size_t)s->N * sizeof(double), (size_t)s->N, hipMemcpyDeviceToDevice, c->stream));
        c->have_state = true;
        child_live = true;
        wide_live = narrow_live = false;
      }
      const int hc = stretch(d, CHILD);
      const int w = no_wide ? end - d : std::min(hc > 0 ? hc : kWin, end - d);
      PS_TRY(auto_alias_records(s, c, d, d + w));
      PS_TRY(ps_chain_run(c, d, w, negval, stat_scale, renorm));
      int g = -1;
      if (!no_wide) {
        double m[64];
        PS_TRY(auto_read_padmax(s, c, d, std::min(w, 64), m));
        for (int i = 0; i < w && g < 0; ++i)
          if (m[i] > 1e-8 && hist_owner(d + i + 1) != CHILD) g = d + i;
      }
      const int keep = g < 0 ? d + w : g + 1;
      for (int q = d; q < keep; ++q) s->owner[q] = hint[q] = CHILD;
      d = keep;
      if (g >= 0) {
        regime = WIDE;
        child_live = false;
      }
    }
  }
  s->auto_first = f;
  s->auto_hint = f - first;
  s->route_hist.assign(hint.begin(), hint.end());
  s->route_first = first;
  s->route_end = end;
  s->have_state = false;
  return PS_OK;
}

static int chain_run_body(ps_solver* s, int first, int count, double negval, double stat_scale, int renorm);

extern "C" int ps_chain_run(ps_solver* s, int first, int count, double negval, double stat_scale,
                            int renorm) {
  const int rc = chain_run_body(s, first, count, negval, stat_scale, renorm);
  if (s && s->kt_from >= 0) {
    (void)hipStreamWaitEvent(s->stream, s->kt_ev, 0);
    s->kt_from = -1;
  }
  if (s) s->kt_lazy_from = -1;
  if (s && s->refft_pending) {
    if (rc == PS_OK) return resolve_refft(s);
    s->refft_pending = nullptr;
  }
  return rc;
}

static int chain_run_body(ps_solver* s, int first, int count, double negval, double stat_scale, int renorm) {
  if (!s) return ps_fail(PS_ERR_BAD_ARG, "null solver");
  if (!s->have_state)
    return ps_fail(PS_ERR_STATE, s->auto_exact && s->auto_first >= 0
                                     ? "auto mode: set the state before every chain run (the previous run handed days over to the "
                                       "exact-torus helpers, the front solver's spectrum is void)"
                                     : "chain_run before set_state");
  if (!s->kernels_on_device || first < 0 || count < 0 || first + count > s->nk)
    return ps_fail(PS_ERR_STATE, "chain_run: days [%d,%d) not uploaded (nk=%d)", first, first + count, s->nk);
  PS_HIP(hipSetDevice(s->device));
  PS_TRY(ensure_stats(s, std::max(4, s->nk)));
  for (int d = first; d < first + count; ++d) PS_TRY(ensure_record(s, PS_REC_CHAIN, d));
  PS_HIP(hipMemsetAsync(s->padmax.p + first, 0, (size_t)count * sizeof(unsigned long long), s->stream));
  s->last_renorm = renorm;
  if (s->mode == PS_MODE_FOLD) {
    const size_t spec = (size_t)s->Pf * s->ld;
    PS_TRY(s->Ahat.ensure(spec));
    PS_TRY(s->fold_rowsum.ensure((size_t)s->Pf));
    PS_TRY(s->fold_rowcnt.ensure((size_t)s->Pf));
    PS_TRY(s->fold_padmax.ensure(1));
    PS_TRY(ensure_temps(s, 1));
    PS_TRY(s->T2.ensure(spec));
    const bool fuse = s->tpipe && s->rs_r2 != 0 && !s->cfg.no_fold_fuse;
    const bool fuse_alt = fuse && rs_colfull_alt_ok(s->rs_r2, s->rs_r3) && !s->cfg.no_fold_alt;
    const bool fold_rows = fuse && s->Pref >= 2 * s->M && !s->cfg.no_fold_rows;
    if (!fold_rows) PS_TRY(s->lin.ensure((size_t)s->Pf * s->Pf));
    if (fuse_alt && !s->one_flag.p) {
      PS_TRY(s->one_flag.ensure(1));
      const double one = 1.0;
      PS_HIP(hipMemcpyAsync(s->one_flag.p, &one, sizeof(double), hipMemcpyHostToDevice, s->stream));
      PS_HIP(hipStreamSynchronize(s->stream));
    }
    for (int c0 = first; c0 < first + count; c0 += s->chunk_days) {
      const int cn = std::min(s->chunk_days, first + count - c0);
      PS_TRY(transform_kernels(s, c0, cn));
      for (int d = c0; d < c0 + cn; ++d) {
        const cplx* B = s->Bhat.p + (size_t)(d - s->bhat_first) * s->Pf * s->ld;
        const SrcMap tmap = map_plain(s->Pref, s->Pf);
        if (fuse) {
          PS_TRY(launch_row_fwd(s, s->torus.p, 0, s->Pref, tmap, tmap, s->T1.p, 1, nullptr, 1, nullptr,
                                d > first ? s->padmax.p + d - 1 : nullptr, s->N));
          RowLive klive = s->kt_live;
          klive.range = s->krange.p + 2 * d;
          if (fuse_alt) {
            const ColAlt alt{s->T1.p, s->one_flag.p, RowLive{1, tmap, nullptr}};
            PS_TRY(launch_colfull(s, 0, B, s->Ahat.p, 0, s->T2.p, 1, klive, nullptr, 1, nullptr, 0, -1, -1, true, &alt));
          } else {
            PS_TRY(launch_colfull(s, 1, s->T1.p, s->Ahat.p, 0, nullptr, 1, RowLive{1, tmap, nullptr}, nullptr));
            PS_TRY(launch_colfull(s, 0, B, s->Ahat.p, 0, s->T2.p, 1, klive, nullptr));
          }
          if (fold_rows) {
            RowFoldArgs fa;
            fa.src = s->T2.p; fa.ld = s->ld; fa.M = s->Pf; fa.P = s->Pref; fa.N = s->N; fa.m = s->M;
            fa.scale = 1.0 / ((double)s->Pf * (double)s->Pf); fa.negval = negval; fa.stat_scale = stat_scale;
            fa.torus = s->torus.p; fa.rec = s->recs[PS_REC_CHAIN][d];
            fa.rowsum = s->rowsum.p + (int64_t)d * s->N; fa.rowcnt = s->rowcnt.p + (int64_t)d * s->N;
            fa.padmax = s->padmax.p + d;
            fa.prog = s->row_plan.prog;
            const int units = 2 * s->M + (s->Pref - 2 * s->M + 1) / 2;
            ProfScope prof(s, PS_PROF_ROW_INV);
            if (!rs_launch_row_fold(s->rs_r2, s->rs_r3, fa, units, s->stream))
              return ps_fail(PS_ERR_STATE, "no fold row kernel for 16 x %d x %d", s->rs_r2, s->rs_r3);
            PS_HIP(hipGetLastError());
          } else {
            PS_TRY(launch_row_inv(s, s->T2.p, s->lin.p, d, 1, negval, stat_scale, true));
            hipLaunchKernelGGL(k_fold, dim3(s->Pref), dim3(256), 0, s->stream, s->lin.p, s->Pf, s->Pref, s->N, s->M,
                               s->torus.p, s->recs[PS_REC_CHAIN][d], negval, stat_scale,
                               s->rowsum.p + (int64_t)d * s->N, s->rowcnt.p + (int64_t)d * s->N, s->padmax.p + d);
            PS_HIP(hipGetLastError());
          }
          if (d == first + count - 1) {
            hipLaunchKernelGGL(k_truncate_if_flag, dim3(s->Pref), dim3(256), 0, s->stream, s->torus.p, s->Pref, s->N,
                               s->padmax.p + d);
            PS_HIP(hipGetLastError());
          }
          continue;
        }
        if (s->tpipe) {
          PS_TRY(launch_row_fwd(s, s->torus.p, 0, s->Pref, tmap, tmap, s->T1.p, 1, nullptr, 1));
          PS_TRY(launch_colfull(s, 1, s->T1.p, s->Ahat.p, 0, nullptr, 1, RowLive{1, tmap, nullptr}, nullptr));
          RowLive klive = s->kt_live;
          klive.range = s->krange.p + 2 * d;
          PS_TRY(launch_colfull(s, 0, B, s->Ahat.p, 0, s->T2.p, 1, klive, nullptr));
          PS_TRY(launch_row_inv(s, s->T2.p, s->lin.p, d, 1, negval, stat_scale, true));
          hipLaunchKernelGGL(k_fold, dim3(s->Pref), dim3(256), 0, s->stream, s->lin.p, s->Pf, s->Pref, s->N, s->M,
                             s->torus.p, s->recs[PS_REC_CHAIN][d], negval, stat_scale,
                             s->rowsum.p + (int64_t)d * s->N, s->rowcnt.p + (int64_t)d * s->N, s->padmax.p + d);
          PS_HIP(hipGetLastError());
          hipLaunchKernelGGL(k_truncate_if_flag, dim3(s->Pref), dim3(256), 0, s->stream, s->torus.p, s->Pref, s->N,
                             s->padmax.p + d);
          PS_HIP(hipGetLastError());
          continue;
        }
        PS_TRY(launch_row_fwd(s, s->torus.p, 0, s->Pref, tmap, tmap, s->T1.p, 1, nullptr, 1));
        const cplx* part = s->T1.p;
        cplx* fused_out = s->T2.p;
        RowLive part_live{1, tmap, nullptr};
        if (s->split) {
          PS_TRY(launch_col<PS_FWD>(s, s->fwd_passes[0], s->T1.p, nullptr, nullptr, s->T2.p, 1, 0, nullptr, part_live));
          part = s->T2.p;
          fused_out = s->T1.p;
          part_live = RowLive{0, {0, 0, 0, 0}, nullptr};
        }
        int dual = 0;
        PS_TRY(launch_col_fused_dual(s, B, part, part_live, fused_out, s->krange.p + 2 * d, &dual));
// ... 934 lines not shown
```

parasitoids_amd/csrc/rs_launch.h:

```cpp
#pragma once
#include <hip/hip_runtime.h>
#include "fft_kernels.h"

struct ColFullArgs;

struct RsInfo {
  int np, nthr;
  size_t lds_rows, lds_col1, lds_colc;
  bool chain;
  bool rsp;
};
bool rs_lookup(int L, int* r2, int* r3);
int rs_next_size(int n);
bool rs_info(int r2, int r3, RsInfo* out);
int rs_rows_set_attrs();
int rs_colfull_set_attrs();
int rs_launch_row_fwd(int r2, int r3, const RowFwdArgs& a, int npairs, int batch, hipStream_t st);
int rs_launch_row_inv(int r2, int r3, const RowInvArgs& a, int npairs, int batch, hipStream_t st);
int rs_launch_colfull(int r2, int r3, const ColFullArgs& a, int lines8, int batch, hipStream_t st);
struct RowFoldArgs;
int rs_launch_row_fold(int r2, int r3, const RowFoldArgs& a, int units, hipStream_t st);
bool rs_colfull_alt_ok(int r2, int r3);
bool rs_dual_ok(int r2, int r3);
int rs_coldual_set_attrs();
int rs_launch_coldual(int r2, int r3, const ColFullArgs& a, int lines8, int batch, hipStream_t st);
```

Measured before the change: 4323 grid-days/s.

## Launch row-forward FFT only over live row pairs and zero kernel boxes

```diff
diff --git a/include/parasitoid_hip.h b/include/parasitoid_hip.h
--- a/include/parasitoid_hip.h
+++ b/include/parasitoid_hip.h
@@ -44,6 +44,7 @@
 
 int ps_solver_create(ps_solver** out, int device, int dom_len, int max_shape, int mode);
 int ps_fast_size(int dom_len, int max_shape);
+int ps_live_pairs(int P, int n1, int off1, int lo2, int off2, int nd, const int32_t* range, int32_t* out);
 int ps_solver_retarget(ps_solver* s, int max_shape);
 int ps_solver_destroy(ps_solver* s);
 int ps_solver_info(ps_solver* s, int* dom_len, int* P, int* Pfft, int* H);
diff --git a/parasitoids_amd/_lib.py b/parasitoids_amd/_lib.py
--- a/parasitoids_amd/_lib.py
+++ b/parasitoids_amd/_lib.py
@@ -49,6 +49,7 @@
     'ps_last_error': (C.c_char_p, []),
     'ps_device_info': (C.c_int, [C.c_int, C.c_char_p, C.c_int, _I32P, _I64P]),
     'ps_solver_create': (C.c_int, [C.POINTER(_VP), C.c_int, C.c_int, C.c_int, C.c_int]),
+    'ps_live_pairs': (C.c_int, [C.c_int, C.c_int, C.c_int, C.c_int, C.c_int, C.c_int, _I32P, _I32P]),
     'ps_solver_destroy': (C.c_int, [_VP]),
     'ps_solver_info': (C.c_int, [_VP, _I32P, _I32P, _I32P, _I32P]),
     'ps_solver_sync': (C.c_int, [_VP]),
diff --git a/parasitoids_amd/csrc/chain_kernels.h b/parasitoids_amd/csrc/chain_kernels.h
--- a/parasitoids_amd/csrc/chain_kernels.h
+++ b/parasitoids_amd/csrc/chain_kernels.h
@@ -15,6 +15,15 @@
   const int64_t n = (int64_t)(r1 - r0 + 1) * K;
   for (int64_t i = blockIdx.x * (int64_t)blockDim.x + threadIdx.x; i < n; i += (int64_t)gridDim.x * blockDim.x)
     base[i] = 0.0;
+}
+
+static __global__ void k_zero_box(double* dst, int K, const int* __restrict__ rr, const int* __restrict__ cr) {
+  const int d = blockIdx.y;
+  const int r0 = max(rr[2 * d], 0), r1 = min(rr[2 * d + 1], K - 1);
+  const int c0 = max(cr[2 * d], 0), c1 = min(cr[2 * d + 1], K - 1);
+  double* base = dst + (int64_t)d * K * K;
+  for (int r = r0 + (int)blockIdx.x; r <= r1; r += (int)gridDim.x)
+    for (int c = c0 + (int)threadIdx.x; c <= c1; c += (int)blockDim.x) base[(int64_t)r * K + c] = 0.0;
 }
 
 static __global__ void k_scatter_coo_batch(const int* __restrict__ row, const int* __restrict__ col,
@@ -280,6 +289,7 @@
   }
 }
 
-static __global__ void k_set_int2(int* dst, int a, int b) {
-  if (threadIdx.x == 0 && blockIdx.x == 0) { dst[0] = a; dst[1] = b; }
-}
+struct Ints16 { int v[16]; };
+static __global__ void k_set_ints(int* dst, Ints16 v, int n) {
+  if (blockIdx.x == 0 && (int)threadIdx.x < n && threadIdx.x < 16) dst[threadIdx.x] = v.v[threadIdx.x];
+}
diff --git a/parasitoids_amd/csrc/fft_kernels.h b/parasitoids_amd/csrc/fft_kernels.h
--- a/parasitoids_amd/csrc/fft_kernels.h
+++ b/parasitoids_amd/csrc/fft_kernels.h
@@ -44,8 +44,13 @@
   const unsigned long long* pred;
   const unsigned long long* trunc_pred;
   int trunc_n;
+  const int* pairs;
+  int pairs_n;
+  const int* colrange;
   FftProg prog;
 };
+
+#define PS_LP_W 4
 
 struct ColArgs {
   const cplx* src;
diff --git a/parasitoids_amd/csrc/fft_rs_kernels.h b/parasitoids_amd/csrc/fft_rs_kernels.h
--- a/parasitoids_amd/csrc/fft_rs_kernels.h
+++ b/parasitoids_amd/csrc/fft_rs_kernels.h
@@ -794,15 +794,31 @@
     const int xcd = unit & 7, q = unit >> 3;
     unit = ((q / KL) * 8 + xcd) * KL + (q % KL);
   }
-  const int pair = ((int)gridDim.x - 1 - unit) * NP + half;
+  int pair, bat = (int)blockIdx.y;
+  if (a.pairs) {
+    const int* lp = a.pairs;
+    const int v = lp[0] + unit * NP + half;
+    if (v >= lp[PS_LP_W * a.pairs_n]) return;
+    int lo = 0, hi = a.pairs_n;
+    while (hi - lo > 1) {
+      const int mid = (lo + hi) >> 1;
+      if (lp[PS_LP_W * mid] <= v) lo = mid; else hi = mid;
+    }
+    bat = lo;
+    const int* e = lp + PS_LP_W * bat;
+    const int w = v - e[0];
+    pair = w < e[2] ? e[1] + w : e[3] + (w - e[2]);
+  } else {
+    pair = ((int)gridDim.x - 1 - unit) * NP + half;
+  }
   const int ra = 2 * pair, rb = ra + 1;
   if (ra >= a.P || pair < 0) return;
   double* ex = reinterpret_cast<double*>(ps_lds_raw) + half * (Y::XW + Y::RED);
   const int j = threadIdx.x - half * S::NTHR;
-  const double* src = a.src + (int64_t)blockIdx.y * a.src_bstride;
-  cplx* dst = a.dst + (int64_t)blockIdx.y * a.dst_bstride;
-  const int rlo = a.rowrange ? a.rowrange[2 * blockIdx.y] : 0;
-  const int rhi = a.rowrange ? a.rowrange[2 * blockIdx.y + 1] : 0x7fffffff;
+  const double* src = a.src + (int64_t)bat * a.src_bstride;
+  cplx* dst = a.dst + (int64_t)bat * a.dst_bstride;
+  const int rlo = a.rowrange ? a.rowrange[2 * bat] : 0;
+  const int rhi = a.rowrange ? a.rowrange[2 * bat + 1] : 0x7fffffff;
   SrcMap rmap = a.rmap, cmap = a.cmap;
   const bool trunc = a.trunc_pred && !pred_skip(a.trunc_pred);
   if (trunc) {
@@ -835,13 +851,28 @@
   if (j < S::T1) {
     const double* pa = src + (int64_t)(sa >= 0 ? sa : 0) * a.src_ld;
     const double* pb = src + (int64_t)(sb >= 0 ? sb : 0) * a.src_ld;
-#pragma unroll
-    for (int q = 0; q < R1; ++q) {
-      const int sc = src_map(cmap, j + q * S::T1);
-      const bool ok = sc >= 0;
-      const int c = ok ? sc : 0;
-      const double va = pa[c], vb = pb[c];
-      x[q] = make_double2((ok && sa >= 0) ? va : 0.0, (ok && sb >= 0) ? vb : 0.0);
+    if (a.colrange) {
+      const int clo = a.colrange[2 * bat], chi = a.colrange[2 * bat + 1];
+#pragma unroll
+      for (int q = 0; q < R1; ++q) {
+        const int sc = src_map(cmap, j + q * S::T1);
+        const bool ok = sc >= 0 && sc >= clo && sc <= chi;
+        double va = 0.0, vb = 0.0;
+        if (ok) {
+          if (sa >= 0) va = pa[sc];
+          if (sb >= 0) vb = pb[sc];
+        }
+        x[q] = make_double2(va, vb);
+      }
+    } else {
+#pragma unroll
+      for (int q = 0; q < R1; ++q) {
+        const int sc = src_map(cmap, j + q * S::T1);
+        const bool ok = sc >= 0;
+        const int c = ok ? sc : 0;
+        const double va = pa[c], vb = pb[c];
+        x[q] = make_double2((ok && sa >= 0) ? va : 0.0, (ok && sb >= 0) ? vb : 0.0);
+      }
     }
     bfly<R1, PS_FWD>(x);
   }
diff --git a/parasitoids_amd/csrc/ps_config.h b/parasitoids_amd/csrc/ps_config.h
--- a/parasitoids_amd/csrc/ps_config.h
+++ b/parasitoids_amd/csrc/ps_config.h
@@ -38,6 +38,7 @@
   X("PS_NO_DUAL", no_dual, 0, FLAG, R)                                                              \
   X("PS_NO_DIRECT", no_direct, 0, FLAG, R)                                                          \
   X("PS_NO_ROW_BATCH", no_row_batch, 0, FLAG, R)                                                    \
+  X("PS_NO_LIVE_PAIRS", no_live_pairs, 0, FLAG, R)                                                  \
   X("PS_NO_PAD_QUIET", no_pad_quiet, 0, FLAG, R)                                                    \
   X("PS_NO_TAIL_SPLIT", no_tail_split, 0, FLAG, R)                                                  \
   X("PS_NO_DEFER_REFFT", no_defer_refft, 0, FLAG, R)                                                \
diff --git a/parasitoids_amd/csrc/ps_rs_rows.hip b/parasitoids_amd/csrc/ps_rs_rows.hip
--- a/parasitoids_amd/csrc/ps_rs_rows.hip
+++ b/parasitoids_amd/csrc/ps_rs_rows.hip
@@ -72,11 +72,13 @@
   return gx;
 }
 
-int rs_launch_row_fwd(int r2, int r3, const RowFwdArgs& a, int npairs, int batch, hipStream_t st) {
+int rs_launch_row_fwd(int r2, int r3, const RowFwdArgs& a, int npairs, int batch, hipStream_t st, int listed) {
 #define X(A, B)                                                                                              \
   if (r2 == A && r3 == B) {                                                                                  \
     using C = RsCfg<A, B>;                                                                                   \
     constexpr int np = C::NP;                                                                                \
+    const int gy = a.pairs ? 1 : batch;                                                                      \
+    const int gp = a.pairs ? listed : npairs;                                                                \
                                                  \
     constexpr int np2 = (np >= 2 && C::S::L <= 2560) ? np / 2 : np;                                          \
     if constexpr (np2 != np) {                                                                               \
@@ -85,12 +87,14 @@
         auto k2 = k_row_fwd_rs<16, A, B, np2>;                                                               \
         using Y2 = RsInvLds<16, A, B>;                                                                       \
         constexpr size_t lds2 = Y2::bytes(np2);                                                              \
-        hipLaunchKernelGGL(k2, dim3(grid_x(npairs, np2, a.tstride), batch), dim3(C::S::NTHR * np2), lds2, st, a); \
+        if (gp > 0)                                                                                          \
+          hipLaunchKernelGGL(k2, dim3(grid_x(gp, np2, a.tstride), gy), dim3(C::S::NTHR * np2), lds2, st, a); \
         return 1;                                                                                            \
       }                                                                                                      \
     }                                                                                                        \
     auto kern = k_row_fwd_rs<16, A, B, np>;                                                                  \
-    hipLaunchKernelGGL(kern, dim3(grid_x(npairs, np, a.tstride), batch), dim3(C::S::NTHR * np), C::LDS, st, a); \
+    if (gp > 0)                                                                                              \
+      hipLaunchKernelGGL(kern, dim3(grid_x(gp, np, a.tstride), gy), dim3(C::S::NTHR * np), C::LDS, st, a);  \
     return 1;                                                                                                \
   }
   PS_RS_SIZES(X)
diff --git a/parasitoids_amd/csrc/ps_solver.hip b/parasitoids_amd/csrc/ps_solver.hip
--- a/parasitoids_amd/csrc/ps_solver.hip
+++ b/parasitoids_amd/csrc/ps_solver.hip
@@ -181,6 +181,7 @@
   int chunk_days = 1;
   DevBuf<int> srange;
   bool srange_valid = false;
+  int srange_listed = 0;
   DevBuf<int> krow, kcol;
   DevBuf<double> kval;
   std::vector<int64_t> koff;
@@ -201,8 +202,15 @@
   int last_renorm = 0;
   RowLive kt_live{0, {0, 0, 0, 0}, nullptr};
   bool kt_direct = false;
-  DevBuf<int> krange;
+  struct IntView { int* p = nullptr; };
+  IntView krange;
   std::vector<int> hkrange;
+  IntView kcrange;
+  std::vector<int> hkcrange;
+  IntView kpairs;
+  std::vector<int> hkpairs;
+  DevBuf<int> kmeta;
+  std::vector<int> hkmeta;
   DevBuf<int> orow, ocol;
   DevBuf<double> oval;
   DevBuf<const double*> wptr;
@@ -319,11 +327,54 @@
   return PS_OK;
 }
 
+static int live_pairs(SrcMap m, int P, int nd, const int* range, int* out) {
+  int pos = 0;
+  for (int d = 0; d < nd; ++d) {
+    const int64_t lo = range ? range[2 * d] : 0, hi = range ? range[2 * d + 1] : INT64_MAX / 4;
+    const int64_t r0[2] = {std::max<int64_t>(0, lo - m.off1),
+                           std::max<int64_t>(std::max(m.lo2, m.n1), lo - m.off2 + m.lo2)};
+    const int64_t r1[2] = {std::min<int64_t>(std::min(m.n1, P) - 1, hi - m.off1),
+                           std::min<int64_t>(P - 1, hi - m.off2 + m.lo2)};
+    int64_t gs[2] = {0, 0}, ge[2] = {0, 0};
+    int n = 0;
+    for (int i = 0; i < 2 && lo <= hi; ++i) {
+      if (r0[i] > r1[i]) continue;
+      const int64_t s0 = r0[i] / 2 / 4 * 4, e0 = r1[i] / 2 / 4 * 4 + 4;
+      if (n == 1 && s0 <= ge[0]) {
+        ge[0] = std::max(ge[0], e0);
+      } else {
+        gs[n] = s0;
+        ge[n] = e0;
+        ++n;
+      }
+    }
+    int* e = out + PS_LP_W * d;
+    e[0] = pos;
+    e[1] = (int)gs[0];
+    e[2] = (int)(ge[0] - gs[0]);
+    e[3] = (int)gs[1];
+    pos += (int)(ge[0] - gs[0] + ge[1] - gs[1]);
+  }
+  int* e = out + PS_LP_W * nd;
+  e[0] = pos;
+  for (int i = 1; i < PS_LP_W; ++i) e[i] = 0;
+  return pos;
+}
+
+extern "C" int ps_live_pairs(int P, int n1, int off1, int lo2, int off2, int nd, const int32_t* range, int32_t* out) {
+  if (P < 1 || nd < 0 || !out) return ps_fail(PS_ERR_BAD_ARG, "live_pairs: bad arguments");
+  return live_pairs(SrcMap{n1, off1, lo2, off2}, P, nd, range, out);
+}
+
 static int launch_row_fwd(ps_solver* s, const double* src, int64_t src_bstride, int src_ld,
                           SrcMap rmap, SrcMap cmap, cplx* dst, int batch,
                           const unsigned long long* pred, int skip_zero = 0, const int* rowrange = nullptr,
-                          const unsigned long long* trunc_pred = nullptr, int trunc_n = 0) {
+                          const unsigned long long* trunc_pred = nullptr, int trunc_n = 0,
+                          const int* pairs = nullptr, int listed = 0, const int* colrange = nullptr) {
   RowFwdArgs a;
+  a.pairs = (pairs && skip_zero && !pred && !trunc_pred && !s->cfg.no_live_pairs) ? pairs : nullptr;
+  a.pairs_n = batch;
+  a.colrange = a.pairs ? colrange : nullptr;
   if (trunc_pred && s->rs_r2 == 0) return ps_fail(PS_ERR_STATE, "row pass: only the register-resident kernels truncate on the fly");
   a.trunc_pred = trunc_pred; a.trunc_n = trunc_n;
   a.src = src; a.src_bstride = src_bstride; a.src_ld = src_ld;
@@ -344,7 +395,7 @@
   if (lds > (size_t)kMaxLds) return ps_fail(PS_ERR_UNSUPPORTED, "row pass needs %zu B LDS", lds);
   ProfScope prof(s, pred ? PS_PROF_REFFT : PS_PROF_ROW_FWD);
   if (s->rs_r2 != 0 && !s->cfg.no_rs_fwd) {
-    if (!rs_launch_row_fwd(s->rs_r2, s->rs_r3, a, npairs, batch, s->stream))
+    if (!rs_launch_row_fwd(s->rs_r2, s->rs_r3, a, npairs, batch, s->stream, listed))
       return ps_fail(PS_ERR_STATE, "no register-resident row kernel for 16 x %d x %d", s->rs_r2, s->rs_r3);
   } else if (s->row_plan.generic)
     hipLaunchKernelGGL((k_row_fwd<true, false>), grid, dim3(thr), lds, s->stream, a);
@@ -537,8 +588,9 @@
 }
 
 static int fwd2d(ps_solver* s, const double* src, int64_t src_bstride, int src_ld, SrcMap rmap,
-                 SrcMap cmap, cplx* out, int batch, const unsigned long long* pred, const int* rowrange = nullptr) {
-  PS_TRY(launch_row_fwd(s, src, src_bstride, src_ld, rmap, cmap, s->T1.p, batch, pred, 1, rowrange));
+                 SrcMap cmap, cplx* out, int batch, const unsigned long long* pred, const int* rowrange = nullptr,
+                 const int* pairs = nullptr, int listed = 0) {
+  PS_TRY(launch_row_fwd(s, src, src_bstride, src_ld, rmap, cmap, s->T1.p, batch, pred, 1, rowrange, nullptr, 0, pairs, listed));
   if (s->tpipe) return launch_colfull(s, 1, s->T1.p, out, 0, nullptr, batch, RowLive{1, rmap, rowrange}, pred);
   if (s->fwd_passes.size() == 1) {
     PS_TRY(launch_col<PS_FWD>(s, s->fwd_passes[0], s->T1.p, nullptr, nullptr, out, batch, 0, pred, RowLive{1, rmap, rowrange}));
@@ -569,19 +621,22 @@
 
 static int fwd2d_partial(ps_solver* s, const double* src, int64_t src_bstride, int src_ld,
                          SrcMap rmap, SrcMap cmap, cplx* out, int batch, const int* rowrange = nullptr,
-                         bool direct = false) {
+                         bool direct = false, const int* pairs = nullptr, int listed = 0,
+                         const int* colrange = nullptr) {
   const RowLive live{1, rmap, rowrange};
   s->kt_live = RowLive{0, {0, 0, 0, 0}, nullptr};
   s->kt_direct = s->split && direct && !s->tpipe;
   if (s->tpipe) {
     s->kt_live = live;
-    return launch_row_fwd(s, src, src_bstride, src_ld, rmap, cmap, out, batch, nullptr, 1, rowrange);
+    return launch_row_fwd(s, src, src_bstride, src_ld, rmap, cmap, out, batch, nullptr, 1, rowrange, nullptr, 0, pairs, listed,
+                          colrange);
   }
   if (!s->split || direct) {
     s->kt_live = live;
-    return launch_row_fwd(s, src, src_bstride, src_ld, rmap, cmap, out, batch, nullptr, 1, rowrange);
-  }
-  PS_TRY(launch_row_fwd(s, src, src_bstride, src_ld, rmap, cmap, s->T1.p, batch, nullptr, 1, rowrange));
+    return launch_row_fwd(s, src, src_bstride, src_ld, rmap, cmap, out, batch, nullptr, 1, rowrange, nullptr, 0, pairs, listed,
+                          colrange);
+  }
+  PS_TRY(launch_row_fwd(s, src, src_bstride, src_ld, rmap, cmap, s->T1.p, batch, nullptr, 1, rowrange, nullptr, 0, pairs, listed, colrange));
   return launch_col<PS_FWD>(s, s->fwd_passes[0], s->T1.p, nullptr, nullptr, out, batch, 0, nullptr, live);
 }
 
@@ -1032,7 +1087,7 @@
   s->Ahat.release(); s->Chat.release(); s->T1.release(); s->T2.release(); s->Bhat.release(); s->Fhat.release();
   s->Trow.release(); s->blk.release(); s->one_flag.release(); s->tail_hat.release(); s->pad_energy.release(); s->pad_quiet.release();
   s->srange.release();
-  s->krow.release(); s->kcol.release(); s->kval.release(); s->kdense.release(); s->krange.release();
+  s->krow.release(); s->kcol.release(); s->kval.release(); s->kdense.release(); s->kmeta.release();
   for (auto& v : s->recs)
     for (double* p : v)
       if (p) ps_dev_free(p);
@@ -1178,7 +1233,7 @@
   if (s->recs[PS_REC_STATE].empty() || !s->recs[PS_REC_STATE][0]) return ps_fail(PS_ERR_STATE, "no state record");
   PS_TRY(ensure_temps(s, 1));
   PS_TRY(fwd2d(s, s->recs[PS_REC_STATE][0], 0, s->N, map_plain(s->N, s->Pf), map_plain(s->N, s->Pf), s->Ahat.p, 1, nullptr,
-               s->srange_valid ? s->srange.p : nullptr));
+               s->srange_valid ? s->srange.p : nullptr, s->srange_valid ? s->srange.p + 2 : nullptr, s->srange_listed));
   s->spec_valid = true;
   return PS_OK;
 }
@@ -1205,8 +1260,13 @@
     range[0] = std::min(range[0], (int)row[i]);
     range[1] = std::max(range[1], (int)row[i]);
   }
-  PS_TRY(s->srange.ensure(2));
-  hipLaunchKernelGGL(k_set_int2, dim3(1), dim3(64), 0, s->stream, s->srange.p, range[0], range[1]);
+  Ints16 v{};
+  v.v[0] = range[0];
+  v.v[1] = range[1];
+  static_assert(2 + 2 * PS_LP_W <= 16, "state range and live-pair list fit one k_set_ints");
+  s->srange_listed = live_pairs(map_plain(s->N, s->Pf), s->Pf, 1, range, v.v + 2);
+  PS_TRY(s->srange.ensure(2 + 2 * PS_LP_W));
+  hipLaunchKernelGGL(k_set_ints, dim3(1), dim3(64), 0, s->stream, s->srange.p, v, 2 + 2 * PS_LP_W);
   PS_HIP(hipGetLastError());
   s->srange_valid = true;
   return PS_OK;
@@ -1234,16 +1294,26 @@
   PS_TRY(s->Bhat.ensure(spec * total));
   PS_TRY(ensure_temps(s, total));
   double* kd = s->kdense.p + (size_t)slot0 * K * K;
-  int blo = K, bhi = -1;
+  const bool listed = s->hkpairs.size() >= (size_t)PS_LP_W * (first + count + 1) &&
+                      s->hkcrange.size() >= 2 * (size_t)(first + count);
+  const bool boxes = listed && s->rs_r2 != 0 && !s->cfg.no_rs_fwd && !s->cfg.no_live_pairs;
+  int blo = K, bhi = -1, wmax = 0;
   int64_t maxn = 0;
   for (int d = first; d < first + count; ++d) {
     if (s->hkrange[2 * d] <= s->hkrange[2 * d + 1]) {
       blo = std::min(blo, s->hkrange[2 * d]);
       bhi = std::max(bhi, s->hkrange[2 * d + 1]);
+      if (boxes) wmax = std::max(wmax, s->hkrange[2 * d + 1] - s->hkrange[2 * d] + 1);
     }
     maxn = std::max<int64_t>(maxn, s->koff[d + 1] - s->koff[d]);
   }
-  if (bhi >= blo) {
+  if (boxes) {
+    if (wmax > 0) {
+      hipLaunchKernelGGL(k_zero_box, dim3(std::min(wmax, 1024), count), dim3(256), 0, s->stream, kd, K,
+                         s->krange.p + 2 * first, s->kcrange.p + 2 * first);
+      PS_HIP(hipGetLastError());
+    }
+  } else if (bhi >= blo) {
     blo = std::max(blo, 0);
     bhi = std::min(bhi, K - 1);
     const int64_t n = (int64_t)(bhi - blo + 1) * K;
@@ -1262,7 +1332,9 @@
   if (direct_chunk >= 0) direct = direct && direct_chunk != 0;
   else for (int d = first; d < first + count && direct; ++d) direct = day_is_compact(s, d);
   PS_TRY(fwd2d_partial(s, kd, (int64_t)K * K, K, map_wrap(M, s->Pf), map_wrap(M, s->Pf), s->Bhat.p + (size_t)slot0 * spec, count,
-                       s->krange.p + 2 * first, direct));
+                       s->krange.p + 2 * first, direct, listed ? s->kpairs.p + PS_LP_W * first : nullptr,
+                       listed ? s->hkpairs[PS_LP_W * (first + count)] - s->hkpairs[PS_LP_W * first] : 0,
+                       boxes ? s->kcrange.p + 2 * first : nullptr));
   s->bhat_first = first - slot0;
   s->bhat_count = slot0 + count;
   return PS_OK;
@@ -1288,8 +1360,23 @@
   return PS_OK;
 }
 
+static int upload_kranges(ps_solver* s) {
+  const int nd = (int)s->hkrange.size() / 2;
+  s->hkpairs.assign((size_t)PS_LP_W * (nd + 1), 0);
+  live_pairs(map_wrap(s->Kmax / 2, s->Pf), s->Pf, nd, s->hkrange.data(), s->hkpairs.data());
+  s->hkmeta.assign(s->hkrange.begin(), s->hkrange.end());
+  s->hkmeta.insert(s->hkmeta.end(), s->hkcrange.begin(), s->hkcrange.end());
+  s->hkmeta.insert(s->hkmeta.end(), s->hkpairs.begin(), s->hkpairs.end());
+  PS_TRY(s->kmeta.ensure(s->hkmeta.size()));
+  s->krange.p = s->kmeta.p;
+  s->kcrange.p = s->kmeta.p + s->hkrange.size();
+  s->kpairs.p = s->kcrange.p + s->hkcrange.size();
+  PS_HIP(hipMemcpyAsync(s->kmeta.p, s->hkmeta.data(), s->hkmeta.size() * sizeof(int), hipMemcpyHostToDevice, s->stream));
+  return PS_OK;
+}
+
 static int set_kernels_common(ps_solver* s, int nk, const int64_t* off, const int32_t* kshape,
-                              const int32_t* rows) {
+                              const int32_t* rows, const int32_t* cols) {
   s->koff.assign(off, off + nk + 1);
   s->kshape.assign(kshape, kshape + nk);
   s->nk = nk;
@@ -1303,25 +1390,29 @@
   }
   if (2 * (s->Kmax / 2) + 1 > s->Pf) return ps_fail(PS_ERR_BAD_SHAPE, "kernel larger than the pad");
   s->hkrange.assign(2 * (size_t)std::max(nk, 1), 0);
+  s->hkcrange.assign(2 * (size_t)std::max(nk, 1), 0);
   const int M = s->Kmax / 2;
   for (int d = 0; d < nk; ++d) {
     const int o = M - kshape[d] / 2;
-    int lo = 0, hi = kshape[d] - 1;
-    if (rows && off[d + 1] > off[d]) {
-      lo = kshape[d];
-      hi = -1;
-      for (int64_t i = off[d]; i < off[d + 1]; ++i) {
-        lo = std::min(lo, (int)rows[i]);
-        hi = std::max(hi, (int)rows[i]);
+    for (int pass = 0; pass < 2; ++pass) {
+      const int32_t* idx = pass == 0 ? rows : cols;
+      int lo = 0, hi = kshape[d] - 1;
+      if (idx && off[d + 1] > off[d]) {
+        lo = kshape[d];
+        hi = -1;
+        for (int64_t i = off[d]; i < off[d + 1]; ++i) {
+          lo = std::min(lo, (int)idx[i]);
+          hi = std::max(hi, (int)idx[i]);
+        }
+      } else if (idx) {
+        lo = 1;
+        hi = 0;
       }
-    } else if (rows) {
-      lo = 1;
-      hi = 0;
-    }
-    s->hkrange[2 * d] = lo + o;
-    s->hkrange[2 * d + 1] = hi + o;
-  }
-  PS_TRY(s->krange.ensure(s->hkrange.size()));
+      std::vector<int>& r = pass == 0 ? s->hkrange : s->hkcrange;
+      r[2 * d] = lo + o;
+      r[2 * d + 1] = hi + o;
+    }
+  }
   PS_TRY(s->dkoff.ensure((size_t)nk + 1));
   PS_TRY(s->dkshape.ensure((size_t)std::max(nk, 1)));
   {
@@ -1329,7 +1420,7 @@
     PS_HIP(hipMemcpy(s->dkoff.p, o64.data(), o64.size() * sizeof(long long), hipMemcpyHostToDevice));
     if (nk > 0) PS_HIP(hipMemcpy(s->dkshape.p, kshape, (size_t)nk * sizeof(int), hipMemcpyHostToDevice));
   }
-  PS_HIP(hipMemcpyAsync(s->krange.p, s->hkrange.data(), s->hkrange.size() * sizeof(int), hipMemcpyHostToDevice, s->stream));
+  PS_TRY(upload_kranges(s));
   PS_HIP(hipStreamSynchronize(s->stream));
   s->bhat_first = -1;
   s->bhat_count = 0;
@@ -1359,7 +1450,7 @@
     PS_HIP(hipMemcpyAsync(s->kval.p, val, tot * 8, hipMemcpyHostToDevice, s->stream));
     PS_HIP(hipStreamSynchronize(s->stream));
   }
-  return set_kernels_common(s, nk, off, kshape, row);
+  return set_kernels_common(s, nk, off, kshape, row, col);
 }
 
 int ps_chain_adopt_device_kernels(ps_solver* s, int nk, const int64_t* off, const int32_t* kshape,
@@ -1374,7 +1465,7 @@
     PS_HIP(hipMemcpyAsync(s->kcol.p, col, tot * 4, hipMemcpyDeviceToDevice, s->stream));
     PS_HIP(hipMemcpyAsync(s->kval.p, val, tot * 8, hipMemcpyDeviceToDevice, s->stream));
   }
-  return set_kernels_common(s, nk, off, kshape, nullptr);
+  return set_kernels_common(s, nk, off, kshape, nullptr, nullptr);
 }
 
 static int auto_attach(ps_solver* s, ps_solver** slot, int mode, int max_shape, bool* kernels_ok, int end) {
@@ -1396,7 +1487,8 @@
   if (!*kernels_ok) {
     PS_TRY(ps_chain_adopt_device_kernels(c, s->nk, s->koff.data(), s->kshape.data(), s->krow.p, s->kcol.p, s->kval.p));
     c->hkrange = s->hkrange;
-    PS_HIP(hipMemcpyAsync(c->krange.p, c->hkrange.data(), c->hkrange.size() * sizeof(int), hipMemcpyHostToDevice, c->stream));
+    c->hkcrange = s->hkcrange;
+    PS_TRY(upload_kranges(c));
     PS_HIP(hipStreamSynchronize(c->stream));
     *kernels_ok = true;
   }
diff --git a/parasitoids_amd/csrc/rs_launch.h b/parasitoids_amd/csrc/rs_launch.h
--- a/parasitoids_amd/csrc/rs_launch.h
+++ b/parasitoids_amd/csrc/rs_launch.h
@@ -15,7 +15,7 @@
 bool rs_info(int r2, int r3, RsInfo* out);
 int rs_rows_set_attrs();
 int rs_colfull_set_attrs();
-int rs_launch_row_fwd(int r2, int r3, const RowFwdArgs& a, int npairs, int batch, hipStream_t st);
+int rs_launch_row_fwd(int r2, int r3, const RowFwdArgs& a, int npairs, int batch, hipStream_t st, int listed = 0);
 int rs_launch_row_inv(int r2, int r3, const RowInvArgs& a, int npairs, int batch, hipStream_t st);
 int rs_launch_colfull(int r2, int r3, const ColFullArgs& a, int lines8, int batch, hipStream_t st);
 struct RowFoldArgs;
```

Result: faster. 4425 grid-days/s, median of 4 (+2.4%).
